# AdeeshKolluru/AdsorbDiff

Measured on AMD Instinct MI355X. Metric: sampled adsorbate sites/sec (50 denoise steps, ~200-atom slabs), higher is better.
Workload: dtype f32 (f16x3-split MFMA, fp32 accumulate; ADF_GEMM=f32 selects exact f32)

## Files before the change

adsorbdiff_amd/csrc/api.hip:

```cpp
#include <stdarg.h>
#include <stdlib.h>
#include <string.h>

#include <new>

#include "common.h"

static thread_local char g_err[512] = "";

void adf_set_error(const char* fmt, ...) {
    va_list ap;
    va_start(ap, fmt);
    vsnprintf(g_err, sizeof(g_err), fmt, ap);
    va_end(ap);
}

extern "C" const char* adf_last_error(void) { return g_err; }
extern "C" const char* adf_version(void) { return "adsorbdiff_hip 0.5.0 (gfx950)"; }

adf_tune adf_tune_from_env() {
    auto off_is_0 = [](const char* name) { const char* e = getenv(name); return (e && atoi(e) == 0) ? 0 : 1; };
    auto is_f32 = [](const char* name) { const char* e = getenv(name); return e && strcmp(e, "f32") == 0; };
    adf_tune t = {};
    t.gemm_stream = off_is_0("ADF_GEMM_STREAM");
    t.head_gate_fused = off_is_0("ADF_HEAD_GATE_FUSED");
    t.lift_emit = off_is_0("ADF_LIFT_EMIT");
    t.graph_sys_csr = off_is_0("ADF_GRAPH_SYS_CSR");
    t.train_gemm16 = is_f32("ADF_TRAIN_GEMM") ? 0 : 1;
    t.wgrad_f32 = is_f32("ADF_WGRAD") ? 1 : 0;
    const char* gt = getenv("ADF_EQV2_GEMM_TILE");
    t.eqv2_gemm_tile256 = (gt && atoi(gt) == 128) ? 0 : 1;
    t.eqv2_rotin_generic = getenv("ADF_EQV2_ROTIN_GENERIC") != nullptr;
    t.eqv2_rotout_generic = getenv("ADF_EQV2_ROTOUT_GENERIC") != nullptr;
    t.sample_split = off_is_0("ADF_SAMPLE_SPLIT");
    return t;
}
const adf_tune& adf_tune_process() {
    static const adf_tune t = adf_tune_from_env();
    return t;
}
int adf_current_num_cus() {
    int dev = 0, n = 0;
    if (hipGetDevice(&dev) != hipSuccess || hipDeviceGetAttribute(&n, hipDeviceAttributeMultiprocessorCount, dev) != hipSuccess) return 0;
    return n;
}

extern "C" int32_t adf_profile_enable(adf_painn_t h, int32_t on) {
    if (!h) { adf_set_error("null handle"); return ADF_EINVAL; }
    h->prof.enable(on != 0);
    ADF_HIP_CHECK(hipMemset(h->kcount, 0, 8 * sizeof(unsigned long long)));
    if (h->twin) return adf_profile_enable(h->twin, on);
    return ADF_OK;
}

extern "C" int32_t adf_profile_read(adf_painn_t h, float* ms, int64_t* count, int64_t* message_ksteps, void* stream) {
    if (!h || !ms || !count) { adf_set_error("null argument"); return ADF_EINVAL; }
    ADF_HIP_CHECK(hipStreamSynchronize((hipStream_t)stream));
    if (message_ksteps) {
        unsigned long long k[8];
        ADF_HIP_CHECK(hipMemcpy(k, h->kcount, sizeof(k), hipMemcpyDeviceToHost));
        ADF_HIP_CHECK(hipMemset(h->kcount, 0, sizeof(k)));
        *message_ksteps = (int64_t)k[0];
    }
    ADF_TRY(h->prof.read(ms, count, ADF_PROF_NCAT));
    if (h->twin) {
        float ms2[ADF_PROF_NCAT];
        int64_t count2[ADF_PROF_NCAT], k2 = 0;
        ADF_TRY(adf_profile_read(h->twin, ms2, count2, message_ksteps ? &k2 : nullptr, h->twin->split_stream));
        for (int c = 0; c < ADF_PROF_NCAT; ++c) { ms[c] += ms2[c]; count[c] += count2[c]; }
        if (message_ksteps) *message_ksteps += k2;
    }
    return ADF_OK;
}

extern "C" int32_t adf_painn_create(const adf_painn_hparams* hp, adf_painn_t* out) {
    if (!hp || !out) { adf_set_error("null argument"); return ADF_EINVAL; }
    if (hp->hidden_channels % ADF_SLICE_CH != 0 || hp->hidden_channels < 128 || hp->hidden_channels > 1024) {
        adf_set_error("hidden_channels=%d must be a multiple of %d in [128,1024]", hp->hidden_channels, ADF_SLICE_CH);
        return ADF_EINVAL;
    }
    if (hp->num_rbf % 2 != 0 || hp->num_rbf > 128 || hp->num_rbf < 2) {
        adf_set_error("num_rbf=%d must be even and <= 128", hp->num_rbf);
        return ADF_EINVAL;
    }
    if (hp->max_neighbors < 1 || hp->max_neighbors > ADF_MAX_K) {
        adf_set_error("max_neighbors=%d must be in [1,%d]", hp->max_neighbors, ADF_MAX_K);
        return ADF_EINVAL;
    }
    if (hp->num_layers < 1 || hp->num_layers > 16 || hp->num_heads < 0 || hp->num_heads > 2) {
        adf_set_error("num_layers must be in [1,16], num_heads in [0,2]");
        return ADF_EINVAL;
    }
    adf_painn* h = new (std::nothrow) adf_painn();
    if (!h) { adf_set_error("host allocation failed"); return ADF_EOOM; }
    h->hp = *hp;
    hipDeviceProp_t prop;
    if (hipGetDevice(&h->device) != hipSuccess || hipGetDeviceProperties(&prop, h->device) != hipSuccess) {
        adf_set_error("no usable HIP device: %s", hipGetErrorString(hipGetLastError()));
        adf_painn_destroy(h);
        return ADF_EHIP;
    }
    h->num_cus = prop.multiProcessorCount;
    h->dist_floor = 1.0e-3f;
    {
        const char* e = getenv("ADF_INCREMENTAL");
        h->inc_on = !(e && e[0] == '0');
        const char* e2 = getenv("ADF_INC_SYNC");
        h->inc_sync = e2 && e2[0] == '1';
    }
    const int H = hp->hidden_channels, R = hp->num_rbf, L = hp->num_layers;
    adf_pool& m = h->m_life;
    int32_t st = m.alloc(&h->rbf_pack, (size_t)L * (H / ADF_SLICE_CH) * R * 192);
    if (st == ADF_OK) st = m.alloc(&h->rbf_bias_pack, (size_t)L * (H / ADF_SLICE_CH) * 192);
    if (st == ADF_OK) st = m.alloc(&h->rbf_pack16, (size_t)L * (H / ADF_SLICE_CH) * R * 192 * 2 * sizeof(uint16_t));
    if (st == ADF_OK) st = m.alloc(&h->rbf_bias_pack16, (size_t)L * (H / ADF_SLICE_CH) * 192);
    if (st == ADF_OK) st = m.alloc(&h->rbf_scales, 16);
    if (st == ADF_OK) st = m.alloc(&h->flags, ADF_NFLAGS);
    if (st == ADF_OK && hipMemset(h->flags, 0, sizeof(int32_t) * ADF_NFLAGS) != hipSuccess) st = ADF_EHIP;
    {
        const size_t HH = (size_t)H * H;
        const size_t per_layer = HH + 3 * HH + 2 * HH + 2 * HH + 3 * HH;
        const size_t per_head = HH + HH / 2 + 2 * HH + HH + HH / 4 + HH / 2;
        const size_t elems = (size_t)L * per_layer + (size_t)hp->num_heads * per_head;
        h->w16_bytes = elems * 2 * sizeof(uint16_t) + 4096;
        if (st == ADF_OK) st = m.alloc(&h->w16_arena, h->w16_bytes);
        if (st == ADF_OK) st = m.alloc(&h->w16_scales, 256);
        if (st == ADF_OK) st = m.alloc(&h->w16_bias_perm, (size_t)L * 2 * 3 * H);
        if (st == ADF_OK) st = m.alloc(&h->w16_scratch, 1);
        if (st == ADF_OK) st = m.alloc(&h->wfrag_arena, h->w16_bytes);
        const char* e = getenv("ADF_GEMM");
        h->gemm_f32 = e && strcmp(e, "f32") == 0;
        const char* el = getenv("ADF_LIFT");
        h->lift_on = !(el && strcmp(el, "0") == 0);
        const char* e2 = getenv("ADF_MSG");
        h->msg_f32 = e2 ? strcmp(e2, "f32") == 0 : h->gemm_f32;
        h->msg_f32_only = hp->num_rbf % 8 != 0;
        h->msg_f32 = h->msg_f32 || h->msg_f32_only;
        const char* er = getenv("ADF_ROW_MAXIMA");
        h->rmx = (er && atoi(er) == 0) ? 0 : 1;
        h->tune = adf_tune_from_env();
    }
    if (st == ADF_OK) st = m.alloc(&h->kcount, 8);
    if (st == ADF_OK && hipMemset(h->kcount, 0, 8 * sizeof(unsigned long long)) != hipSuccess) st = ADF_EHIP;
    if (st != ADF_OK) { adf_painn_destroy(h); return st; }
    *out = h;
    return ADF_OK;
}

static void inc_free(adf_painn* h) {
    h->m_inc.release();
    h->inc_tmp_bytes = 0;
    h->inc_capN = 0; h->inc_valid = false;
}

static void free_workspaces(adf_painn* h) {
    h->m_ws.release();
    h->inc_valid = false;
    h->scan_tmp_bytes = 0;
    h->lift.cap = 0; h->mag_v3_valid = false;
    h->xpart = h->catpart = h->vpart = nullptr; h->part_stride = 0;
    h->part_x = h->part_vec = nullptr; h->dbg_msg_rows = h->dbg_cat_rows = h->dbg_comb_rows = 0; h->dbg_mag = nullptr;
    h->cache_valid = false;
    h->capN = h->capB = h->capE = 0;
}

extern "C" int32_t adf_painn_destroy(adf_painn_t h) {
    if (!h) return ADF_OK;
    if (h->twin) { adf_set_error("destroy: the handle has a live twin that reads its weight images; destroy the twin first"); return ADF_EINVAL; }
    if (h->parent) {
        h->parent->twin = nullptr;
        h->parent->split_last = false;
        if (h->split_stream) { (void)hipStreamSynchronize((hipStream_t)h->split_stream); (void)hipStreamDestroy((hipStream_t)h->split_stream); }
        for (void* e : h->split_ev)
            if (e) (void)hipEventDestroy((hipEvent_t)e);
    }
    if (h->inc_cnt_host) (void)hipHostFree(h->inc_cnt_host);
    for (int i = 0; i < 2; ++i)
        if (h->inc_ev[i]) (void)hipEventDestroy((hipEvent_t)h->inc_ev[i]);
    adf_grad_free(h);
    delete h;
    return ADF_OK;
}

static void borrow_weights(adf_painn* t, const adf_painn* p, bool bound) {
    t->emb = p->emb; t->rbf_offset = p->rbf_offset;
    memcpy(t->layer, p->layer, sizeof(t->layer));
    memcpy(t->head, p->head, sizeof(t->head));
    memcpy(t->scale, p->scale, sizeof(t->scale));
    t->rbf_pack = p->rbf_pack; t->rbf_bias_pack = p->rbf_bias_pack; t->rbf_pack16 = p->rbf_pack16;
    t->rbf_bias_pack16 = p->rbf_bias_pack16; t->rbf_scales = p->rbf_scales; t->rbf_uniform = p->rbf_uniform;
    t->w16_arena = p->w16_arena; t->w16_bytes = p->w16_bytes; t->w16_scales = p->w16_scales;
    t->w16_bias_perm = p->w16_bias_perm; t->w16_scratch = p->w16_scratch; t->wfrag_arena = p->wfrag_arena;
    t->weights_set = bound && p->weights_set;
    t->rec0_valid = false;
    t->inc_valid = false;
}
static void follow_settings(adf_painn* t, const adf_painn* p) {
    if (t->gemm_f32 != p->gemm_f32 || t->msg_f32 != p->msg_f32 || t->dist_floor != p->dist_floor || t->lift_on != p->lift_on) {
        t->cache_valid = false; t->rec0_valid = false; t->inc_valid = false;
    }
    t->gemm_f32 = p->gemm_f32; t->msg_f32 = p->msg_f32; t->msg_f32_only = p->msg_f32_only; t->dist_floor = p->dist_floor;
    t->lift_on = p->lift_on; t->tune = p->tune; t->inc_sync = p->inc_sync;
}

extern "C" int32_t adf_painn_create_twin(adf_painn_t parent, adf_painn_t* out) {
    if (!parent || !out) { adf_set_error("create_twin: null argument"); return ADF_EINVAL; }
    if (parent->parent) { adf_set_error("create_twin: the handle is a twin itself"); return ADF_EINVAL; }
    if (parent->twin) { adf_set_error("create_twin: the handle already has a twin"); return ADF_EINVAL; }
    int dev = -1;
    if (hipGetDevice(&dev) != hipSuccess || dev != parent->device) {
        adf_set_error("create_twin: the parent lives on device %d, the current device is %d", parent->device, dev);
        return ADF_EINVAL;
    }
    adf_painn* t = new (std::nothrow) adf_painn();
    if (!t) { adf_set_error("host allocation failed"); return ADF_EOOM; }
    t->hp = parent->hp; t->device = parent->device; t->num_cus = parent->num_cus;
    t->rmx = parent->rmx; t->inc_on = parent->inc_on;
    follow_settings(t, parent);
    int32_t st = t->m_life.alloc(&t->flags, ADF_NFLAGS);
    if (st == ADF_OK && hipMemset(t->flags, 0, sizeof(int32_t) * ADF_NFLAGS) != hipSuccess) st = ADF_EHIP;
    if (st == ADF_OK) st = t->m_life.alloc(&t->kcount, 8);
    if (st == ADF_OK && hipMemset(t->kcount, 0, 8 * sizeof(unsigned long long)) != hipSuccess) st = ADF_EHIP;
    if (st == ADF_OK) st = t->m_life.alloc(&t->split_state, 16);
    if (st == ADF_OK && hipStreamCreateWithFlags(reinterpret_cast<hipStream_t*>(&t->split_stream), hipStreamNonBlocking) != hipSuccess) st = ADF_EHIP;
    for (int i = 0; i < 2 && st == ADF_OK; ++i)
        if (hipEventCreateWithFlags(reinterpret_cast<hipEvent_t*>(&t->split_ev[i]), hipEventDisableTiming) != hipSuccess) st = ADF_EHIP;
    if (st != ADF_OK) {
        if (st == ADF_EHIP) adf_set_error("create_twin: %s", hipGetErrorString(hipGetLastError()));
        t->parent = parent;
        parent->twin = t;
        adf_painn_destroy(t);
        return st;
    }
    borrow_weights(t, parent, true);
    t->prof.enable(parent->prof.on);
    t->parent = parent;
    parent->twin = t;
    *out = t;
    return ADF_OK;
}

extern "C" int32_t adf_painn_set_split(adf_painn_t h, int32_t on) {
    if (!h) { adf_set_error("null handle"); return ADF_EINVAL; }
    h->tune.sample_split = on != 0;
    return ADF_OK;
}

extern "C" int32_t adf_split_stats(adf_painn_t h, int64_t* split_runs, int64_t* fallback_runs) {
    if (!h) { adf_set_error("null handle"); return ADF_EINVAL; }
    if (split_runs) *split_runs = (int64_t)h->split_runs;
    if (fallback_runs) *fallback_runs = (int64_t)h->split_fallbacks;
    return ADF_OK;
}

static void leave_split(adf_painn* h) {
    if (!h || !h->split_last) return;
    h->split_last = false;
    h->cache_valid = false; h->rec0_valid = false; h->inc_valid = false;
}

extern "C" int32_t adf_painn_set_weights(adf_painn_t h, int32_t n_weights, const void* const* w,
                                         const float* scale_factors, void* stream) {
    if (!h || !w || !scale_factors) { adf_set_error("null argument"); return ADF_EINVAL; }
    if (h->parent) { adf_set_error("set_weights: a twin reads its parent's weights; bind them there"); return ADF_EINVAL; }
    if (h->twin) borrow_weights(h->twin, h, false);
    const int L = h->hp.num_layers;
    const int expect = 2 + ADF_WEIGHTS_PER_LAYER * L + ADF_WEIGHTS_PER_HEAD * h->hp.num_heads;
    if (n_weights != expect) {
        adf_set_error("expected %d weight tensors, got %d", expect, n_weights);
        return ADF_EINVAL;
    }
    for (int i = 0; i < n_weights; ++i)
        if (!w[i]) { adf_set_error("weight %d is null", i); return ADF_EINVAL; }
    auto f = [&](int i) { return reinterpret_cast<const float*>(w[i]); };
    h->emb = f(0);
    h->rbf_offset = f(1);
    int k = 2;
    for (int l = 0; l < L; ++l) {
        adf_layer_weights& lw = h->layer[l];
        lw.ln_w = f(k++); lw.ln_b = f(k++); lw.xp0_w = f(k++); lw.xp0_b = f(k++); lw.xp2_w = f(k++); lw.xp2_b = f(k++);
        lw.rbf_w = f(k++); lw.rbf_b = f(k++); lw.vp_w = f(k++); lw.xv0_w = f(k++); lw.xv0_b = f(k++);
        lw.xv2_w = f(k++); lw.xv2_b = f(k++);
        h->scale[l] = scale_factors[l];
    }
    for (int hd = 0; hd < h->hp.num_heads; ++hd)
        for (int b = 0; b < 2; ++b) {
            adf_block_weights& bw = h->head[hd][b];
            bw.vec1_w = f(k++); bw.vec2_w = f(k++); bw.un0_w = f(k++); bw.un0_b = f(k++); bw.un2_w = f(k++);
            bw.un2_b = f(k++);
        }
    ADF_TRY(adf_pack_rbf(h, (hipStream_t)stream));
    {
        hipStream_t s = (hipStream_t)stream;
        const long long H = h->hp.hidden_channels, HH = H * H;
        unsigned char* cur = h->w16_arena;
        unsigned char* fcur = h->wfrag_arena;
        int nscale = 0;
        float* bperm = h->w16_bias_perm;
        auto split = [&](const float* w, long long rows, long long K, adf_w16* out, const float* fused_bias = nullptr,
                         bool pair_perm = false) -> int32_t {
            const long long n = rows * K;
            out->hi = cur; cur += n * 2;
            out->lo = cur; cur += n * 2;
            out->inv_scale = h->w16_scales + nscale++;
            out->bias_perm = nullptr;
            out->frag = nullptr;
            if (fused_bias) {
                out->bias_perm = bperm; bperm += 3 * H;
                ADF_TRY(adf_split_weight(w, n, out, h->w16_scratch, s, (int)H, (int)H, fused_bias));
            } else if (pair_perm) {
                ADF_TRY(adf_split_weight(w, n, out, h->w16_scratch, s, (int)H, (int)H, nullptr, 2));
            } else {
                ADF_TRY(adf_split_weight(w, n, out, h->w16_scratch, s));
            }
            if (rows % 32 == 0 && K % 16 == 0) {
                out->frag = fcur; fcur += n * 4;
                ADF_TRY(adf_pack_frag(out, (int)rows, (int)K, out->frag, s));
            }
            return ADF_OK;
        };
        for (int l = 0; l < L; ++l) {
            adf_layer_weights& lw = h->layer[l];
            ADF_TRY(split(lw.xp0_w, H, H, &lw.xp0_16));
            ADF_TRY(split(lw.xp2_w, 3 * H, H, &lw.xp2_16, lw.xp2_b));
            ADF_TRY(split(lw.vp_w, 2 * H, H, &lw.vp_16, nullptr, true));
            ADF_TRY(split(lw.xv0_w, H, 2 * H, &lw.xv0_16));
            ADF_TRY(split(lw.xv2_w, 3 * H, H, &lw.xv2_16, lw.xv2_b));
        }
        for (int hd = 0; hd < h->hp.num_heads; ++hd) {
            adf_block_weights& b0 = h->head[hd][0];
            adf_block_weights& b1 = h->head[hd][1];
            ADF_TRY(split(b0.vec1_w, H, H, &b0.vec1_16));
            ADF_TRY(split(b0.vec2_w, H / 2, H, &b0.vec2_16));
            ADF_TRY(split(b0.un0_w, H, 2 * H, &b0.un0_16));
            ADF_TRY(split(b0.un2_w, H, H, &b0.un2_16));
            ADF_TRY(split(b1.vec1_w, H / 2, H / 2, &b1.vec1_16));
            ADF_TRY(split(b1.un0_w, H / 2, H, &b1.un0_16));
        }
        if ((size_t)(cur - h->w16_arena) > h->w16_bytes || (size_t)(fcur - h->wfrag_arena) > h->w16_bytes || nscale > 256) {
            adf_set_error("internal: fp16 weight arena overflow");
            return ADF_EINVAL;
        }
    }
    h->weights_set = true;
    h->rec0_valid = false;
    h->inc_valid = false;
    adf_grad_invalidate(h);
    if (h->twin) borrow_weights(h->twin, h, true);
    return ADF_OK;
}

static int32_t ensure_capacity(adf_painn* h, int64_t N, int64_t B) {
    if (N <= h->capN && B <= h->capB) return ADF_OK;
    const int64_t capN = N > h->capN ? N : h->capN;
    const int64_t capB = B > h->capB ? B : h->capB;
    ADF_HIP_CHECK(hipDeviceSynchronize());
    free_workspaces(h);
    const int64_t H = h->hp.hidden_channels, K = h->hp.max_neighbors;
    const int64_t capE = 2 * capN * K;
    int32_t st = ADF_OK;
#define ALLOC(field, count) if (st == ADF_OK) st = h->m_ws.alloc(&h->field, (size_t)(count))
    ALLOC(nbr_cnt, capN);
    ALLOC(nbr_src, capN * K);
    ALLOC(nbr_shift, capN * K);
    ALLOC(cache_d2, capN * K);
    ALLOC(cache_cid, capN * K);
    ALLOC(cache_cnt, capN);
    ALLOC(deg, capN + 1);
    ALLOC(nptr, capN + 1);
    ALLOC(cursor, capN);
    ALLOC(img_cnt, capB);
    ALLOC(sys_slow, capB);
    ALLOC(e_src, capE);
    ALLOC(e_geom, capE);
    if (h->inc_on) {
        ALLOC(prev_nptr, capN + 1);
        ALLOC(prev_src, capE);
        ALLOC(prev_geom, capE);
    }
    if (st == ADF_OK) {
        h->scan_tmp_bytes = adf_scan_temp_bytes(capN + 1);
        st = h->m_ws.alloc(&h->scan_tmp, h->scan_tmp_bytes + 16);
    }
    ALLOC(x, capN * H);
    ALLOC(vecA, capN * 3 * H);
    ALLOC(vecB, capN * 3 * H);
    ALLOC(rec, (capN + 1) * 5 * H);
    ALLOC(y, capN * H);
    ALLOC(xh, capN * 3 * H);
    ALLOC(vv, capN * 6 * H);
    ALLOC(cat, capN * 2 * H);
    ALLOC(dot, capN * H);
    ALLOC(sys, capB * 16);
    ALLOC(lift.buf, capN * 3);
    ALLOC(mag_a, capN);
    ALLOC(mag_b, capN);
    ALLOC(mag_v3, capN * 3);
    const int64_t ps = (capN + 31) / 32 * 32, ns = H / ADF_SLICE_CH;
    if (h->rmx) ALLOC(rmx_part, (4 * ns + H / 32 + 4) * ps);
#undef ALLOC
    h->lift.cap = st == ADF_OK ? capN * 3 : 0;
    if (st != ADF_OK) { free_workspaces(h); return st; }
    if (h->rmx) {
        h->part_stride = ps;
        h->xpart = h->rmx_part; h->catpart = h->xpart + ns * ps; h->vpart = h->catpart + (H / 32) * ps;
        h->dbg_mag = h->vpart + 3 * ns * ps;
    }
    h->capN = capN; h->capB = capB; h->capE = capE;
    return ADF_OK;
}

static int32_t check_batch(const adf_painn* h, const adf_batch* b) {
    if (!h || !b) { adf_set_error("null argument"); return ADF_EINVAL; }
    if (b->num_atoms <= 0 || b->num_systems <= 0) { adf_set_error("empty batch"); return ADF_EINVAL; }
    if (!b->pos || !b->cell || !b->batch || !b->atom_offset) { adf_set_error("null batch array"); return ADF_EINVAL; }
    for (int k = 0; k < 3; ++k)
        if (b->reps[k] < 0 || b->reps[k] > 16) { adf_set_error("reps[%d]=%d out of range", k, b->reps[k]); return ADF_EINVAL; }
    return ADF_OK;
}

static int32_t read_flags(adf_painn* h, hipStream_t s) {
    int32_t f[ADF_NFLAGS];
    ADF_HIP_CHECK(hipMemcpyAsync(f, h->flags, sizeof(f), hipMemcpyDeviceToHost, s));
    ADF_HIP_CHECK(hipMemsetAsync(h->flags, 0, sizeof(f), s));
    int32_t f2[ADF_NFLAGS] = {};
    if (h->twin) {
        ADF_HIP_CHECK(hipMemcpyAsync(f2, h->twin->flags, sizeof(f2), hipMemcpyDeviceToHost, s));
        ADF_HIP_CHECK(hipMemsetAsync(h->twin->flags, 0, sizeof(f2), s));
    }
    ADF_HIP_CHECK(hipStreamSynchronize(s));
    for (int i = 0; i < ADF_NFLAGS; ++i) f[i] |= f2[i];
    if (f[4]) { adf_set_error("atomic number outside [1, %d] (rows of the embedding table)", h->hp.num_elements); return ADF_EINVAL; }
    if (f[0]) { adf_set_error("a centre atom has more than %d in-cutoff candidates", ADF_MAX_CAND); return ADF_EOVERFLOW; }
    if (f[2]) { adf_set_error("edge buffer overflow"); return ADF_EOVERFLOW; }
    if (f[3]) { adf_set_error("an atom has more than %d incoming edges", ADF_MAX_INDEG); return ADF_EOVERFLOW; }
    if (f[1]) { adf_set_error("An image has no neighbors"); return ADF_ENONEIGHBOR; }
    if (f[6]) { adf_set_error("energy gradient: an edge row has no reverse row in its partner's segment (asymmetric graph)"); return ADF_EINVAL; }
    if (f[5]) {
        adf_set_error("non-finite model output%s", h->gemm_f32 ? " (exact-f32 arithmetic: the inputs or weights are not finite)"
                      : " in f16x3 arithmetic: an activation left the fp16 range or the inputs are not finite; "
                        "adf_painn_set_arithmetic(h, 1) selects exact f32");
        return ADF_ENUMERIC;
    }
    return ADF_OK;
}

extern "C" int32_t adf_graph_set_moving(adf_painn_t h, const int32_t* moving, const int32_t* mov_idx,
                                        const int32_t* mov_off) {
    if (!h) { adf_set_error("null handle"); return ADF_EINVAL; }
    if (moving && (!mov_idx || !mov_off)) { adf_set_error("moving mask needs mov_idx and mov_off"); return ADF_EINVAL; }
    h->moving = moving; h->mov_idx = mov_idx; h->mov_off = mov_off;
    ++h->moving_serial;
    ADF_HIP_CHECK(hipMemset(h->flags, 0, sizeof(int32_t) * ADF_NFLAGS));
    h->cache_valid = false;
    h->rec0_valid = false;
    h->inc_valid = false;
    return ADF_OK;
}

extern "C" int32_t adf_graph_build(adf_painn_t h, const adf_batch* b, void* stream, int64_t* num_edges) {
    ADF_TRY(check_batch(h, b));
    leave_split(h);
    ADF_TRY(ensure_capacity(h, b->num_atoms, b->num_systems));
    hipStream_t s = (hipStream_t)stream;
    ADF_TRY(adf_graph_build_impl(h, b, s));
    if (num_edges) {
        int32_t e = 0;
        ADF_HIP_CHECK(hipMemcpyAsync(&e, h->nptr + b->num_atoms, sizeof(int32_t), hipMemcpyDeviceToHost, s));
        ADF_TRY(read_flags(h, s));
        *num_edges = e;
    }
    return ADF_OK;
}

__global__ void adf_export_edges_kernel(const int32_t* nptr, const int32_t* e_src, const float4* eg, int N,
                                        int32_t* src, int32_t* dst, float* dist, float* vec, long long cap) {
    const int n = blockIdx.x * 4 + (threadIdx.x >> 6);
    if (n >= N) return;
    for (int e = nptr[n] + (threadIdx.x & 63); e < nptr[n + 1]; e += 64) {
        if (e >= cap) continue;
        if (src) src[e] = e_src[e];
        if (dst) dst[e] = n;
        const float4 q = eg[e];
        if (dist) dist[e] = q.w;
        if (vec) { vec[3 * (size_t)e] = q.x; vec[3 * (size_t)e + 1] = q.y; vec[3 * (size_t)e + 2] = q.z; }
    }
}

__global__ void adf_export_shift_kernel(const int32_t* nbr_shift, int32_t* out, long long n, int r0, int r1, int r2) {
    const long long i = (long long)blockIdx.x * blockDim.x + threadIdx.x;
    if (i >= n) return;
    const int c = nbr_shift[i];
    const int n2 = 2 * r2 + 1, n1 = 2 * r1 + 1;
    const int ia = c / (n1 * n2), rem = c - ia * (n1 * n2);
    out[3 * i] = ia - r0;
    out[3 * i + 1] = rem / n2 - r1;
    out[3 * i + 2] = rem % n2 - r2;
}

extern "C" int32_t adf_graph_export(adf_painn_t h, int32_t* nbr_count, int32_t* nbr_src, int32_t* nbr_shift,
                                    int64_t edge_capacity, int32_t* edge_src, int32_t* edge_dst, float* edge_dist,
                                    float* edge_vec, int64_t* num_edges, void* stream) {
    if (!h || h->lastN <= 0) { adf_set_error("no graph built"); return ADF_EINVAL; }
    hipStream_t s = (hipStream_t)stream;
    const int64_t N = h->lastN, K = h->hp.max_neighbors;
    if (nbr_count) ADF_HIP_CHECK(hipMemcpyAsync(nbr_count, h->nbr_cnt, sizeof(int32_t) * N, hipMemcpyDeviceToDevice, s));
    if (nbr_src) ADF_HIP_CHECK(hipMemcpyAsync(nbr_src, h->nbr_src, sizeof(int32_t) * N * K, hipMemcpyDeviceToDevice, s));
    if (nbr_shift)
        hipLaunchKernelGGL(adf_export_shift_kernel, dim3((unsigned)((N * K + 255) / 256)), dim3(256), 0, s, h->nbr_shift,
                           nbr_shift, (long long)(N * K), h->last_reps[0], h->last_reps[1], h->last_reps[2]);
    if (edge_src || edge_dst || edge_dist || edge_vec)
        hipLaunchKernelGGL(adf_export_edges_kernel, dim3((unsigned)((N + 3) / 4)), dim3(256), 0, s, h->nptr, h->e_src,
                           h->e_geom, (int)N, edge_src, edge_dst, edge_dist, edge_vec, (long long)edge_capacity);
    ADF_HIP_CHECK(hipGetLastError());
    int32_t e = 0;
    ADF_HIP_CHECK(hipMemcpyAsync(&e, h->nptr + N, sizeof(int32_t), hipMemcpyDeviceToHost, s));
    ADF_HIP_CHECK(hipStreamSynchronize(s));
    if (num_edges) *num_edges = e;
    return ADF_OK;
}

static int32_t zero_pad_rows(adf_painn* h, int N, hipStream_t s) {
    const size_t row = (size_t)5 * h->hp.hidden_channels;
    ADF_HIP_CHECK(hipMemsetAsync(h->rec + (size_t)N * row, 0, sizeof(float) * row, s));
    return ADF_OK;
}

static int32_t make_records(adf_painn* h, int l, int n, const float* x, const float* vec, bool vec_is_zero, float* rec,
                            const int32_t* row_map, hipStream_t s) {
    const int H = h->hp.hidden_channels;
    const adf_layer_weights& w = h->layer[l];
    if (n <= 0) return ADF_OK;
    adf_prof_begin(h, ADF_PROF_NODE, s);
    const bool lift = h->lift_on && !h->gemm_f32;
    const bool em = lift && h->tune.lift_emit;
    ADF_TRY(adf_nodewise_layernorm(x, w.ln_w, w.ln_b, h->y, n, H, s, em ? h->mag_a : nullptr, h->rows_dev));
    ADF_TRY(adf_linear(h, h->y, H, w.xp0_w, &w.xp0_16, w.xp0_b, h->cat, H, n, H, H, 1, s, em ? h->mag_a : nullptr,
                       em ? h->mag_b : nullptr));
    if (h->gemm_f32) {
        if (row_map) { adf_set_error("internal: mapped records need the f16x3 path"); return ADF_EINVAL; }
        ADF_TRY(adf_launch_gemm(h->cat, H, w.xp2_w, H, w.xp2_b, h->xh, 3 * H, n, 3 * H, H, 0, s));
        ADF_TRY(adf_pack_records(h, n, h->xh, vec, vec_is_zero, s, rec));
    } else {
        adf_epi ep = {};
        ep.vec_in = vec; ep.rec = rec ? rec : h->rec; ep.H = H; ep.vec_is_zero = vec_is_zero ? 1 : 0;
        ep.row_map = row_map;
        ep.rmag = em ? h->mag_b : nullptr;
        ep.m_dev = h->rows_dev;
        ADF_TRY(adf_launch_gemm16_fused(h->cat, H, &w.xp2_16, n, H, H, 1, &ep, s, h->tune, lift ? &h->lift : nullptr));
    }
    adf_prof_end(h, s);
    return ADF_OK;
}

static int32_t message_layer(adf_painn* h, int l, int N, const float* x, const float* vec, float* x_out,
                             float* vec_out, bool vec_is_zero, hipStream_t s, const int32_t* tlist = nullptr,
                             int n_targets = 0, float* rec = nullptr, bool records_ready = false) {
    if (!records_ready) ADF_TRY(make_records(h, l, N, x, vec, vec_is_zero, rec, nullptr, s));
    adf_prof_begin(h, ADF_PROF_MESSAGE, s);
    const int items = tlist ? n_targets : N;
    const bool emit = h->rmx && h->lift_on && !h->gemm_f32 && !h->msg_f32 && items > 0 && items <= h->part_stride;
    h->part_x = h->part_vec = nullptr;
    const int32_t st = adf_message_impl(h, l, N, x, h->xh, vec, x_out, vec_out, vec_is_zero, s, tlist, n_targets, rec,
                                        tlist ? h->rows_dev : nullptr, emit ? h->xpart : nullptr, h->vpart, h->part_stride);
    if (st == ADF_OK && emit) {
        h->part_x = x_out; h->part_vec = vec_out; h->part_n = items; h->part_dev = tlist ? h->rows_dev : nullptr;
        h->dbg_msg_rows = items;
    }
    adf_prof_end(h, s);
    return st;
}

static int32_t update_layer(adf_painn* h, int l, int N, float* x, float* vec, hipStream_t s, bool from_message = true) {
    const int H = h->hp.hidden_channels;
    const adf_layer_weights& w = h->layer[l];
    adf_prof_begin(h, ADF_PROF_NODE, s);
    const bool parts = from_message && h->rmx && h->lift_on && !h->gemm_f32 && N > 0 && h->part_x == x && h->part_vec == vec &&
                       h->part_n == N && h->part_dev == h->rows_dev;
    h->part_x = h->part_vec = nullptr;
    if (h->gemm_f32) {
        ADF_TRY(adf_launch_gemm(vec, H, w.vp_w, H, nullptr, h->vv, 2 * H, 3 * N, 2 * H, H, 0, s));
        ADF_TRY(adf_nodewise_update_prep(h->vv, x, h->cat, h->dot, N, H, s));
        ADF_TRY(adf_linear(h, h->cat, 2 * H, w.xv0_w, &w.xv0_16, w.xv0_b, h->y, H, N, H, 2 * H, 1, s));
    } else {
        adf_epi ep = {};
        ep.v1 = h->vv; ep.dotw = h->dot; ep.cat = h->cat; ep.H = H; ep.m_dev = h->rows_dev;
        const adf_lift* lf = h->lift_on ? &h->lift : nullptr;
        if (parts) {
            ADF_TRY(adf_launch_rowmax_combine(h->vpart, 3 * h->part_stride, H / ADF_SLICE_CH, 3ll * N, h->lift.buf, s, h->rows_dev, 3));
            ep.rmag = h->lift.buf;
            if (h->dbg_capture) ADF_HIP_CHECK(hipMemcpyAsync(h->dbg_mag, h->lift.buf, sizeof(float) * 3 * (size_t)N, hipMemcpyDeviceToDevice, s));
        }
        if (parts || (h->dbg_capture && h->rmx && lf && N <= h->part_stride)) {
            ep.catpart = h->catpart; ep.part_stride = h->part_stride; h->dbg_cat_rows = N;
        }
        ADF_TRY(adf_launch_gemm16_fused(vec, H, &w.vp_16, N, H, H, 3, &ep, s, h->tune, lf));
        if (parts) {
            ADF_TRY(adf_launch_rowmax_combine(h->xpart, h->part_stride, H / ADF_SLICE_CH + H / 32, N, h->lift.buf, s, h->rows_dev, 1));
            if (h->dbg_capture) {
                ADF_HIP_CHECK(hipMemcpyAsync(h->dbg_mag + 3 * h->part_stride, h->lift.buf, sizeof(float) * (size_t)N, hipMemcpyDeviceToDevice, s));
                h->dbg_comb_rows = N;
            }
        }
        adf_epi e0 = {};
        e0.A2 = h->cat; e0.K1 = H; e0.m_dev = h->rows_dev;
        e0.rmag = parts ? h->lift.buf : nullptr;
        e0.out_mag = h->lift_on ? reinterpret_cast<unsigned int*>(h->mag_b) : nullptr;
        ADF_TRY(adf_launch_gemm16(x, H, &w.xv0_16, w.xv0_b, h->y, H, N, H, 2 * H, 1, &e0, s, lf, h->tune, h->num_cus));
    }
    int32_t st;
    if (h->gemm_f32) {
        ADF_TRY(adf_launch_gemm(h->y, H, w.xv2_w, H, w.xv2_b, h->xh, 3 * H, N, 3 * H, H, 0, s));
        st = adf_nodewise_update_apply(h->xh, h->dot, h->vv, x, vec, h->scale[l], N, H, s);
    } else {
        adf_epi ep = {};
        ep.x = x; ep.vec = vec; ep.dot = h->dot; ep.vv = h->vv; ep.scale = h->scale[l]; ep.H = H;
        ep.rmag = h->lift_on ? h->mag_b : nullptr;
        ep.m_dev = h->rows_dev;
        st = adf_launch_gemm16_fused(h->y, H, &w.xv2_16, N, H, H, 2, &ep, s, h->tune);
    }
// ... 701 lines not shown
```

adsorbdiff_amd/csrc/common.h:

```cpp
#pragma once
#include "base.h"
#include "arith.h"
#include "lanes.h"

#define ADF_GROUP_NODES 32
#define ADF_SLICE_CH 64
#define ADF_MAX_CAND 1024
#define ADF_MAX_K 128
#define ADF_NFLAGS 8
#define ADF_MAX_INDEG 1024
#define ADF_MAX_LAYERS 16

struct adf_w16 {
    void* hi;
    void* lo;
    float* inv_scale;
    float* bias_perm;
    void* frag;
};
struct adf_epi {
    const float* vec_in;
    float* rec;
    float* x;
    float* vec;
    const float* dot;
    const float* vv;
    float* v1;
    float* dotw;
    float* cat;
    float scale;
    int H;
    int vec_is_zero;
    const float* A2;
    int K1;
    const int32_t* row_map;
    const float* rmag;
    unsigned int* out_mag;
    const int32_t* m_dev;
    int accumulate;
    const float* gate;
    int gate_ld;
    float* catpart;
    long long part_stride;
};
struct adf_lift {
    float* buf;
    long long cap;
};
struct adf_layer_weights {
    const float *ln_w, *ln_b, *xp0_w, *xp0_b, *xp2_w, *xp2_b, *rbf_w, *rbf_b;
    const float *vp_w, *xv0_w, *xv0_b, *xv2_w, *xv2_b;
    adf_w16 xp0_16, xp2_16, vp_16, xv0_16, xv2_16;
};
struct adf_block_weights {
    const float *vec1_w, *vec2_w, *un0_w, *un0_b, *un2_w, *un2_b;
    adf_w16 vec1_16, vec2_16, un0_16, un2_16;
};

struct adf_painn {
    adf_painn_hparams hp;
    int device;
    bool weights_set;
    const float* emb;
    const float* rbf_offset;
    adf_layer_weights layer[16];
    adf_block_weights head[2][2];
    float scale[16];
    float* rbf_pack;
    float* rbf_bias_pack;
    void* rbf_pack16;
    float* rbf_bias_pack16;
    float* rbf_scales;
    unsigned char* w16_arena;
    size_t w16_bytes;
    float* w16_scales;
    float* w16_bias_perm;
    unsigned int* w16_scratch;
    unsigned char* wfrag_arena;
    bool gemm_f32;
    bool msg_f32;
    bool msg_f32_only;
    adf_tune tune;
    bool lift_on;
    adf_lift lift;
    float *mag_a, *mag_b;
    float* mag_v3;
    bool mag_v3_valid;
    int rmx;
    float* rmx_part;
    float *xpart, *catpart, *vpart;
    int64_t part_stride;
    const float *part_x, *part_vec;
    int part_n;
    const int32_t* part_dev;
    int dbg_msg_rows, dbg_cat_rows;
    bool dbg_capture;
    float* dbg_mag;
    int dbg_comb_rows;

    int64_t capN, capB, capE;
    int32_t* nbr_cnt;
    int32_t* nbr_src;
    int32_t* nbr_shift;
    int32_t* deg;
    int32_t* nptr;
    int32_t* cursor;
    int32_t* img_cnt;
    int32_t* sys_slow;
    void* scan_tmp;
    size_t scan_tmp_bytes;
    const int32_t* moving;
    const int32_t* mov_idx;
    const int32_t* mov_off;
    float* cache_d2;
    int32_t* cache_cid;
    int32_t* cache_cnt;
    bool cache_valid;
    int32_t* e_src;
    float4* e_geom;
    int32_t* flags;
    float *x, *vecA, *vecB, *y, *xh, *vv, *cat, *dot;
    float* rec;
    bool rbf_uniform;
    float* rec0;
    int64_t rec0_cap, rec0_N;
    bool rec0_valid;
    bool inc_on;
    bool inc_valid;
    int64_t inc_capN, inc_N;
    int inc_layers;
    float* incX[ADF_MAX_LAYERS + 1];
    float* incV[ADF_MAX_LAYERS + 1];
    float* incR[ADF_MAX_LAYERS];
    int32_t *prev_nptr, *prev_src;
    float4* prev_geom;
    unsigned char *inc_c0, *inc_chg;
    unsigned char *inc_pend, *inc_need, *inc_tf;
    int32_t* inc_list;
    int32_t* inc_cnt;
    int32_t* inc_cnt_host;
    void* inc_ev[2];
    bool inc_ev_live[2];
    int inc_slot;
    bool inc_sync;
    int32_t inc_seen[2 * ADF_MAX_LAYERS + 1];
    bool inc_seen_valid;
    unsigned char inc_pend_whole[2][ADF_MAX_LAYERS];
    int32_t inc_pend_N[2];
    int32_t inc_pend_Nseen;
    const int32_t* rows_dev;
    void* inc_tmp; size_t inc_tmp_bytes;
    unsigned long long inc_rows, inc_rows_full, inc_edges, inc_launches;
    unsigned long long build_serial, inc_serial;
    float *sub_x, *sub_vec, *sub_f;
    int64_t capS;
    float* sys;
    int32_t* ps_state = nullptr; int32_t ps_B = 0;
    const float *oe0_w, *oe0_b, *oe2_w, *oe2_b;
    adf_w16 oe0_16;
    unsigned char* oe0_buf;
    bool energy_set;
    const float* x_last;
    float dist_floor;
    void* grad;
    int64_t lastN, lastB;
    int32_t last_reps[3];
    int num_cus;
    adf_prof prof;
    unsigned long long* kcount;
    adf_painn* twin;
    adf_painn* parent;
    bool split_last;
    int32_t split_cut; int64_t split_N;
    unsigned long long split_runs, split_fallbacks;
    unsigned long long moving_serial, inc_set_serial;
    unsigned long long seen_moving_serial, seen_inc_serial;
    void* split_stream;
    void* split_ev[2];
    int32_t* split_state;
    int32_t* split_hist; int64_t split_hist_cap;
    adf_pool m_life;
    adf_pool m_ws;
    adf_pool m_inc;
    adf_pool m_sub;
    adf_pool m_rec0;
    void* obs_scratch = nullptr;
    int64_t obs_bytes = 0;
    adf_pool m_obs;
};

enum { ADF_PROF_GRAPH = 0, ADF_PROF_MESSAGE = 1, ADF_PROF_NODE = 2, ADF_PROF_HEADS = 3, ADF_PROF_STEPPER = 4 };
static inline void adf_prof_begin(adf_painn* h, int cat, hipStream_t s) { h->prof.begin(cat, s); }
static inline void adf_prof_end(adf_painn* h, hipStream_t s) { h->prof.end(s); }

int32_t adf_launch_gemm(const float* A, int lda, const float* W, int ldw, const float* bias, float* C, int ldc,
                        int M, int N, int K, int act_ssilu, hipStream_t s);
adf_tune adf_tune_from_env();
const adf_tune& adf_tune_process();
int adf_current_num_cus();
int32_t adf_launch_gemm16(const float* A, int lda, const adf_w16* W, const float* bias, float* C, int ldc, int M,
                          int N, int K, int act_ssilu, const adf_epi* ep, hipStream_t s, const adf_lift* lf,
                          const adf_tune& tune, int num_cus);
int32_t adf_launch_rowmag(const float* A, int lda, int K1, const float* A2, int K2, long long M, float* mag, hipStream_t s,
                          const int32_t* m_dev = nullptr, int m_mul = 1);
int32_t adf_launch_rowmax_combine(const float* part, long long stride, int nparts, long long M, float* mag, hipStream_t s,
                                  const int32_t* m_dev = nullptr, int m_mul = 1);
int32_t adf_split_weight(const float* w, long long n, adf_w16* out, unsigned int* scratch_bits, hipStream_t s,
                         int perm_H = 0, int K = 0, const float* bias = nullptr, int parts = 3);
int32_t adf_launch_gemm16_vecnorm(const float* A, int lda, const adf_w16* W, float* nrm, int M, int N, int K,
                                  hipStream_t s, const adf_tune& tune, const adf_lift* lf = nullptr,
                                  const float* premag = nullptr);
int32_t adf_launch_gemm16_fused(const float* A, int lda, const adf_w16* W, int M, int H, int K, int epi,
                                const adf_epi* ep, hipStream_t s, const adf_tune& tune, const adf_lift* lf = nullptr);
static inline int32_t adf_linear(const adf_painn* h, const float* A, int lda, const float* W, const adf_w16* W16,
                                 const float* bias, float* C, int ldc, int M, int N, int K, int act, hipStream_t s,
                                 const float* premag = nullptr, float* out_mag = nullptr) {
    if (h->gemm_f32) return adf_launch_gemm(A, lda, W, K, bias, C, ldc, M, N, K, act, s);
    adf_epi ep = {};
    ep.m_dev = h->rows_dev;
    if (h->lift_on) { ep.rmag = premag; ep.out_mag = reinterpret_cast<unsigned int*>(out_mag); }
    return adf_launch_gemm16(A, lda, W16, bias, C, ldc, M, N, K, act, &ep, s, h->lift_on ? &h->lift : nullptr, h->tune,
                             h->num_cus);
}
int32_t adf_pack_frag(const adf_w16* w, int N, int K, void* out, hipStream_t s);
int32_t adf_graph_build_impl(adf_painn* h, const adf_batch* b, hipStream_t s);
int32_t adf_energy_sum(const float* y, int H2, const float* w, const float* bias, const int32_t* atom_offset, float* energy,
                       int num_systems, hipStream_t s);
void adf_grad_invalidate(adf_painn* h);
void adf_grad_free(adf_painn* h);
bool adf_message_geo_supported(const adf_painn* h);
int32_t adf_message_geo(adf_painn* h, int layer, const float* xh, const float* vec, bool vec_is_zero, float4* part,
                        long long ecap, bool accumulate, hipStream_t s);
size_t adf_inc_temp_bytes(int64_t n);
int32_t adf_inc_compare(adf_painn* h, int N, hipStream_t s);
int32_t adf_inc_need_from_list(adf_painn* h, int N, int L, const int32_t* out_idx, int n_out, hipStream_t s);
int32_t adf_inc_plan_layer(adf_painn* h, int l, int N, bool first, bool have_need, hipStream_t s);
int32_t adf_inc_scatter_rows(const float* src, const int32_t* idx, int n, int width, float* dst, hipStream_t s,
                             const int32_t* n_dev = nullptr);
int32_t adf_inc_gather_rows(const float* src, const int32_t* idx, int n, int width, float* dst, hipStream_t s);
size_t adf_scan_temp_bytes(int64_t n);
int32_t adf_message_impl(adf_painn* h, int layer, int N, const float* x, const float* xh, const float* vec,
                         float* x_out, float* vec_out, bool vec_is_zero, hipStream_t s,
                         const int32_t* tlist = nullptr, int n_targets = 0, const float* rec = nullptr,
                         const int32_t* n_targets_dev = nullptr,
                         float* xpart = nullptr, float* vpart = nullptr, long long part_stride = 0);
int32_t adf_pack_rbf(adf_painn* h, hipStream_t s);
int32_t adf_pack_rbf_layer(adf_painn* h, int l, hipStream_t s);
int32_t adf_pack_records(adf_painn* h, int N, const float* xh, const float* vec, bool vec_is_zero, hipStream_t s,
                         float* rec = nullptr);
int32_t adf_nodewise_embed(adf_painn* h, const int32_t* Z, int N, float* x, hipStream_t s);
int32_t adf_nodewise_layernorm(const float* x, const float* w, const float* b, float* y, int N, int H, hipStream_t s,
                               float* out_mag = nullptr, const int32_t* n_dev = nullptr);
int32_t adf_nodewise_update_prep(const float* vv, const float* x, float* cat, float* dot, int N, int H, hipStream_t s);
int32_t adf_nodewise_update_apply(const float* h3, const float* dot, const float* vv, float* x, float* vec,
                                  float scale, int N, int H, hipStream_t s);
int32_t adf_head_forward(adf_painn* h, int head, int N, const float* x, const float* vec, float* out, hipStream_t s);
int32_t adf_stepper_init(const adf_batch* b, float* pos, const int32_t* tags, const float* noise,
                         hipStream_t s);
int32_t adf_stepper_step(float* sys, const adf_batch* b, float* pos, const int32_t* tags, const int32_t* fixed,
                         const float* f1, const float* f2, const adf_step_coef* coef, const adf_step_coef* coefs_dev,
                         int num_steps, const float* z_tr, const float* z_rot, int32_t early_stop_count,
                         int32_t* state, float* dcom, float* drot, hipStream_t s, int32_t* sys_state = nullptr,
                         int32_t* hist_t = nullptr);
int32_t adf_stepper_tr_step(float* sys, const adf_batch* b, float* pos, const int32_t* tags, const float* f1,
                            const adf_tr_coef* coef, const adf_tr_coef* coefs_dev, int num_steps, const float* z,
                            int32_t early_stop_count, int32_t* state, float* dcom, hipStream_t s,
                            int32_t* sys_state = nullptr);

struct adf_model {
    void* h;
    int32_t (*check)(void* h, const adf_batch* b);
    int32_t (*grow)(void* h, const adf_batch* b, float** sys);
    int32_t (*forward)(void* h, const adf_batch* b, const int32_t* out_idx, int32_t n_out, float* f1, float* f2,
                       hipStream_t s);
    void (*prof)(void* h, bool begin, hipStream_t s);
    int32_t* sys_state;
    int32_t sys_B;
};
int32_t adf_model_set_per_system_stop(int32_t** slot, int32_t* slot_B, int32_t* sys_state, int32_t B);
int32_t adf_frames_push_impl(adf_frames* f, const float* src, hipStream_t s);
int32_t adf_model_init_placement(const adf_model& m, const adf_batch* b, float* pos, const int32_t* tags,
                                 const float* noise, hipStream_t s);
int32_t adf_model_sde_step(const adf_model& m, const adf_batch* b, float* pos, const int32_t* tags, const int32_t* fixed,
                           const float* f1, const float* f2, const adf_step_coef* coef, const adf_step_coef* coefs_dev,
                           int32_t num_steps, const float* z_tr, const float* z_rot, int32_t early_stop_count,
                           int32_t* state, float* dcom, float* drot, hipStream_t s, int32_t* hist_t = nullptr);
int32_t adf_model_tr_step(const adf_model& m, const adf_batch* b, float* pos, const int32_t* tags, const float* f1,
                          const adf_tr_coef* coef, const adf_tr_coef* coefs_dev, int32_t num_steps, const float* z,
                          int32_t early_stop_count, int32_t* state, float* dcom, hipStream_t s);
int32_t adf_model_sample(const adf_model& m, const adf_batch* b, float* pos, const int32_t* tags, const int32_t* fixed,
                         const adf_step_coef* coefs_dev, int32_t num_steps, const float* z_tr_all, const float* z_rot_all,
                         int32_t early_stop_count, int32_t poll_every, int32_t* state, const int32_t* out_idx,
                         int32_t n_out, float* f1, float* f2, adf_frames* sink, int32_t frame_every, hipStream_t s);
int32_t adf_model_tr_sample(const adf_model& m, const adf_batch* b, float* pos, const int32_t* tags,
                            const adf_tr_coef* coefs_dev, int32_t num_steps, const float* z_all, int32_t early_stop_count,
                            int32_t poll_every, int32_t* state, const int32_t* out_idx, int32_t n_out, float* f1,
                            adf_frames* sink, int32_t frame_every, hipStream_t s);

struct adf_split_side {
    const adf_batch* b;
    float* pos;
    const int32_t* tags;
    const int32_t* fixed;
    const int32_t* out_idx;
    int32_t n_out;
    float* f1;
    float* f2;
    int32_t* state;
    int32_t* hist;
    int32_t sys0;
    hipStream_t s;
};
int32_t adf_model_sample_split(const adf_model& mA, const adf_model& mB, adf_split_side A, adf_split_side B,
                               const adf_step_coef* coefs_dev, int32_t num_steps, const float* z_tr_all,
                               const float* z_rot_all, int32_t total_systems, int32_t early_stop_count, int32_t poll_every,
                               int32_t* state_init, hipEvent_t fork, hipEvent_t join);
```

adsorbdiff_amd/csrc/energy_grad.hip:

```cpp
#include <stdlib.h>
#include <string.h>

#include "message.h"

struct EgW {
    const float* f32;
    adf_w16 w16;
};
enum { EG_XP0 = 0, EG_XP2, EG_VP, EG_XV0, EG_XV2, EG_NW };

struct adf_grad {
    unsigned char* warena;
    float* wscales;
    bool wvalid;
    EgW fw[ADF_MAX_LAYERS][EG_NW];
    EgW bw[ADF_MAX_LAYERS][EG_NW];
    EgW oe_bw;
    float* rbf_wt[ADF_MAX_LAYERS];
    float* act;
    size_t act_floats;
    float4* part;
    int32_t* rev;
    long long ecap;
    int part_slices;
    adf_pool m_w;
    adf_pool m_ws;
};

static adf_grad* eg_state(adf_painn* h) {
    if (!h->grad) {
        adf_grad* g = new (std::nothrow) adf_grad();
        if (!g) return nullptr;
        h->grad = g;
    }
    return reinterpret_cast<adf_grad*>(h->grad);
}

void adf_grad_invalidate(adf_painn* h) {
    if (h && h->grad) reinterpret_cast<adf_grad*>(h->grad)->wvalid = false;
}

void adf_grad_free(adf_painn* h) {
    if (!h) return;
    delete reinterpret_cast<adf_grad*>(h->grad);
    h->grad = nullptr;
}

__global__ void eg_transpose_kernel(const float* __restrict__ src, float* __restrict__ dst, int R, int C) {
    __shared__ float t[32][33];
    const int bx = blockIdx.x * 32, by = blockIdx.y * 32;
    for (int r = threadIdx.y; r < 32; r += 8) {
        const int rr = by + r, cc = bx + threadIdx.x;
        t[r][threadIdx.x] = (rr < R && cc < C) ? src[(size_t)rr * C + cc] : 0.f;
    }
    __syncthreads();
    for (int r = threadIdx.y; r < 32; r += 8) {
        const int cc = bx + r, rr = by + threadIdx.x;
        if (cc < C && rr < R) dst[(size_t)cc * R + rr] = t[threadIdx.x][r];
    }
}

static inline unsigned eg_grid(long long total) {
    long long b = (total + 255) / 256;
    if (b > 256 * 16) b = 256 * 16;
    if (b < 1) b = 1;
    return (unsigned)b;
}

__global__ void eg_seed_kernel(const float* __restrict__ he0, const float* __restrict__ w2, float* __restrict__ dhe,
                               long long N, int H2) {
    for (long long t = (long long)blockIdx.x * blockDim.x + threadIdx.x; t < N * H2; t += (long long)gridDim.x * blockDim.x) {
        const int c = (int)(t % H2);
        dhe[t] = adf_dssilu_times(he0[t], w2[c]);
    }
}

__global__ void eg_add_kernel(const float* __restrict__ src, float* __restrict__ dst, long long n) {
    for (long long i = (long long)blockIdx.x * blockDim.x + threadIdx.x; i < n; i += (long long)gridDim.x * blockDim.x)
        dst[i] += src[i];
}

__global__ __launch_bounds__(256) void eg_msg_bwd_plain_kernel(
    const int32_t* __restrict__ nptr, const int32_t* __restrict__ e_src, const float4* __restrict__ e_geom,
    const float* __restrict__ xh, const float* __restrict__ vec, const float* __restrict__ wt, const float* __restrict__ bias,
    const float* __restrict__ mu, int R, float inv_cutoff, float coeff, float env_a, float env_b, float env_c, int env_pi,
    const float* __restrict__ gx1, const float* __restrict__ gv1, float* __restrict__ dxh, float* __restrict__ dvec,
    float* __restrict__ dx, float4* __restrict__ part, int H, int vec_is_zero, int accumulate) {
    __shared__ float rbv[128], rbd[128], red[4][4];
    const int j = blockIdx.x, tid = threadIdx.x, lane = tid & 63, wave = tid >> 6;
    const int e0 = nptr[j], e1 = nptr[j + 1];
    const float is3 = 0.57735026918962576f, ish = 1.0f / sqrtf((float)H), is2 = 0.70710678118654752f;
    const int H3 = 3 * H;
    for (int cb = 0; cb < H; cb += 256) {
        const int c = cb + tid;
        const bool on = c < H;
        float xa = 0.f, xb = 0.f, xc = 0.f, w0 = 0.f, w1 = 0.f, w2 = 0.f, ba = 0.f, bb = 0.f, bc = 0.f;
        if (on) {
            const float* xr = xh + (size_t)j * H3;
            xa = xr[c]; xb = xr[H + c]; xc = xr[2 * H + c];
            ba = bias[c]; bb = bias[H + c]; bc = bias[2 * H + c];
            if (!vec_is_zero) { const float* vr = vec + (size_t)j * H3; w0 = vr[c]; w1 = vr[H + c]; w2 = vr[2 * H + c]; }
        }
        float dxa = 0.f, dxb = 0.f, dxc = 0.f, dv0 = 0.f, dv1 = 0.f, dv2 = 0.f;
        for (int e = e0; e < e1; ++e) {
            const int i = e_src[e];
            const float4 g = e_geom[e];
            __syncthreads();
            if (tid < R) {
                const float xs = g.w * inv_cutoff;
                float xq = 1.0f;
                for (int k = 1; k < env_pi; ++k) xq *= xs;
                const float xp = xq * xs, pe = (float)env_pi;
                float env = 1.0f + env_a * xp + env_b * (xp * xs) + env_c * (xp * xs * xs);
                float envd = env_a * pe * xq + env_b * (pe + 1.0f) * xp + env_c * (pe + 2.0f) * (xp * xs);
                if (!(xs < 1.0f)) { env = 0.f; envd = 0.f; }
                const float dm = xs - mu[tid];
                const float ga = expf(coeff * dm * dm);
                rbv[tid] = env * ga;
                rbd[tid] = (envd + env * 2.0f * coeff * dm) * ga * inv_cutoff;
            }
            __syncthreads();
            float al = 0.f, b0 = 0.f, b1 = 0.f, b2 = 0.f;
            if (on) {
                float ra = ba, rb = bb, rc = bc, pa = 0.f, pb = 0.f, pc = 0.f;
                for (int k = 0; k < R; ++k) {
                    const float* wr = wt + (size_t)k * H3;
                    const float wa = wr[c], wb = wr[H + c], wc = wr[2 * H + c];
                    const float v = rbv[k], d = rbd[k];
                    ra = fmaf(wa, v, ra); rb = fmaf(wb, v, rb); rc = fmaf(wc, v, rc);
                    pa = fmaf(wa, d, pa); pb = fmaf(wb, d, pb); pc = fmaf(wc, d, pc);
                }
                const float gx = gx1[(size_t)i * H + c] * is2;
                const size_t vo = (size_t)i * H3 + c;
                const float g0 = gv1[vo] * ish, g1 = gv1[vo + H] * ish, g2 = gv1[vo + 2 * H] * ish;
                const float S = (g0 * w0 + g1 * w1 + g2 * w2) * is3;
                const float T = -(g0 * g.x + g1 * g.y + g2 * g.z);
                dxa += gx * ra; dxb += S * rb; dxc += T * rc;
                const float f = xb * rb * is3;
                dv0 += g0 * f; dv1 += g1 * f; dv2 += g2 * f;
                al = gx * xa * pa + S * xb * pb + T * xc * pc;
                const float fc = xc * rc;
                b0 = g0 * fc; b1 = g1 * fc; b2 = g2 * fc;
            }
            al = adf_wave_sum(al); b0 = adf_wave_sum(b0); b1 = adf_wave_sum(b1); b2 = adf_wave_sum(b2);
            if (lane == 0) { red[wave][0] = al; red[wave][1] = b0; red[wave][2] = b1; red[wave][3] = b2; }
            __syncthreads();
            if (tid < 4) {
                const float sum = (red[0][tid] + red[1][tid]) + (red[2][tid] + red[3][tid]);
                float* o = reinterpret_cast<float*>(part + e) + tid;
                *o = (cb == 0 && !accumulate) ? sum : *o + sum;
            }
        }
        if (on) {
            float* dh = dxh + (size_t)j * H3;
            dh[c] = dxa; dh[H + c] = dxb; dh[2 * H + c] = dxc;
            dx[(size_t)j * H + c] = gx1[(size_t)j * H + c] * is2;
            if (!vec_is_zero) {
                const size_t vo = (size_t)j * H3 + c;
                dvec[vo] = gv1[vo] + dv0; dvec[vo + H] = gv1[vo + H] + dv1; dvec[vo + 2 * H] = gv1[vo + 2 * H] + dv2;
            }
        }
    }
}

__global__ __launch_bounds__(256) void eg_reverse_index_kernel(const int32_t* __restrict__ nptr, const int32_t* __restrict__ e_src,
                                                                const float4* __restrict__ e_geom, int N, int32_t* __restrict__ rev,
                                                                int32_t* __restrict__ flags) {
    const int n = blockIdx.x * 4 + (threadIdx.x >> 6);
    if (n >= N) return;
    for (int e = nptr[n] + (threadIdx.x & 63); e < nptr[n + 1]; e += 64) {
        const int i = e_src[e];
        const float4 g = e_geom[e];
        int found = -1;
        for (int f = nptr[i]; f < nptr[i + 1]; ++f) {
            if (e_src[f] != n) continue;
            const float4 o = e_geom[f];
            if (o.w == g.w && o.x == -g.x && o.y == -g.y && o.z == -g.z) { found = f; break; }
        }
        rev[e] = found;
        if (found < 0) flags[6] = 1;
    }
}

__device__ __forceinline__ void eg_row_gradient(const float4* __restrict__ part, long long ecap, int nslices,
                                                const float4 g, int e, float& gx, float& gy, float& gz) {
    float al = 0.f, bx = 0.f, by = 0.f, bz = 0.f;
    for (int sl = 0; sl < nslices; ++sl) {
        const float4 v = part[(size_t)sl * ecap + e];
        al = __fadd_rn(al, v.x); bx = __fadd_rn(bx, v.y); by = __fadd_rn(by, v.z); bz = __fadd_rn(bz, v.w);
    }
    const float bu = fmaf(bz, g.z, fmaf(by, g.y, __fmul_rn(bx, g.x)));
    const float inv = __fdiv_rn(1.0f, g.w);
    gx = __fsub_rn(__fmul_rn(al, g.x), __fmul_rn(fmaf(-bu, g.x, bx), inv));
    gy = __fsub_rn(__fmul_rn(al, g.y), __fmul_rn(fmaf(-bu, g.y, by), inv));
    gz = __fsub_rn(__fmul_rn(al, g.z), __fmul_rn(fmaf(-bu, g.z, bz), inv));
}

__global__ __launch_bounds__(256) void eg_position_kernel(const int32_t* __restrict__ nptr, const float4* __restrict__ e_geom,
                                                           const int32_t* __restrict__ rev, const float4* __restrict__ part,
                                                           long long ecap, int nslices, int N,
                                                           float* __restrict__ forces) {
    const int n = blockIdx.x * 4 + (threadIdx.x >> 6), lane = threadIdx.x & 63;
    if (n >= N) return;
    float fx = 0.f, fy = 0.f, fz = 0.f;
    for (int e = nptr[n] + lane; e < nptr[n + 1]; e += 64) {
        float ax, ay, az, bx = 0.f, by = 0.f, bz = 0.f;
        eg_row_gradient(part, ecap, nslices, e_geom[e], e, ax, ay, az);
        const int f = rev[e];
        if (f >= 0) eg_row_gradient(part, ecap, nslices, e_geom[f], f, bx, by, bz);
        fx = __fadd_rn(fx, __fsub_rn(ax, bx)); fy = __fadd_rn(fy, __fsub_rn(ay, by)); fz = __fadd_rn(fz, __fsub_rn(az, bz));
    }
#pragma unroll
    for (int o = 32; o > 0; o >>= 1) {
        fx = __fadd_rn(fx, __shfl_xor(fx, o)); fy = __fadd_rn(fy, __shfl_xor(fy, o)); fz = __fadd_rn(fz, __shfl_xor(fz, o));
    }
    if (lane == 0) { forces[3 * (size_t)n] = fx; forces[3 * (size_t)n + 1] = fy; forces[3 * (size_t)n + 2] = fz; }
}

static size_t eg_al(size_t b) { return (b + 255) & ~(size_t)255; }
static size_t eg_weight_bytes(const adf_painn* h) {
    const size_t H = h->hp.hidden_channels, L = h->hp.num_layers, R = h->hp.num_rbf;
    const size_t per_layer = eg_al(H * H * 20) + 2 * eg_al(2 * H * H * 20) + 2 * eg_al(3 * H * H * 20) + eg_al(3 * H * R * 4);
    return per_layer * L + eg_al(H / 2 * H * 12);
}

static int32_t eg_build_weights(adf_painn* h, adf_grad* g, hipStream_t s) {
    const long long H = h->hp.hidden_channels, L = h->hp.num_layers, R = h->hp.num_rbf, H2 = H / 2;
    struct Shape { long long n, k; };
    const Shape shp[EG_NW] = {{H, H}, {3 * H, H}, {2 * H, H}, {H, 2 * H}, {3 * H, H}};
    auto al = eg_al;
    const size_t bytes = eg_weight_bytes(h);
    if (!g->wscales) ADF_TRY(g->m_w.alloc(&g->wscales, (size_t)2 * EG_NW * ADF_MAX_LAYERS + 8));
    ADF_TRY(g->m_w.alloc(&g->warena, bytes));
    unsigned char* cur = g->warena;
    int nscale = 0;
    auto image = [&](const float* w, long long n, long long k, EgW* out) -> int32_t {
        const long long e = n * k;
        out->f32 = w;
        out->w16 = adf_w16{};
        out->w16.hi = cur; out->w16.lo = cur + e * 2; out->w16.frag = cur + e * 4;
        cur += e * 8;
        out->w16.inv_scale = g->wscales + nscale++;
        ADF_TRY(adf_split_weight(w, e, &out->w16, h->w16_scratch, s));
        return adf_pack_frag(&out->w16, (int)n, (int)k, out->w16.frag, s);
    };
    auto transposed = [&](const float* w, long long n, long long k, EgW* out) -> int32_t {
        float* t = reinterpret_cast<float*>(cur);
        cur += n * k * 4;
        hipLaunchKernelGGL(eg_transpose_kernel, dim3((unsigned)((k + 31) / 32), (unsigned)((n + 31) / 32)), dim3(32, 8), 0, s,
                           w, t, (int)n, (int)k);
        return image(t, k, n, out);
    };
    for (int l = 0; l < L; ++l) {
        const adf_layer_weights& lw = h->layer[l];
        const float* src[EG_NW] = {lw.xp0_w, lw.xp2_w, lw.vp_w, lw.xv0_w, lw.xv2_w};
        for (int i = 0; i < EG_NW; ++i) {
            unsigned char* start = cur;
            ADF_TRY(image(src[i], shp[i].n, shp[i].k, &g->fw[l][i]));
            ADF_TRY(transposed(src[i], shp[i].n, shp[i].k, &g->bw[l][i]));
            cur = start + al((size_t)shp[i].n * shp[i].k * 20);
        }
        g->rbf_wt[l] = reinterpret_cast<float*>(cur);
        hipLaunchKernelGGL(eg_transpose_kernel, dim3((unsigned)((R + 31) / 32), (unsigned)((3 * H + 31) / 32)), dim3(32, 8), 0, s,
                           lw.rbf_w, g->rbf_wt[l], (int)(3 * H), (int)R);
        cur += al((size_t)3 * H * R * 4);
    }
    ADF_TRY(transposed(h->oe0_w, H2, H, &g->oe_bw));
    ADF_HIP_CHECK(hipGetLastError());
    if ((size_t)(cur - g->warena) > bytes) { adf_set_error("internal: gradient weight arena overflow"); return ADF_EINVAL; }
    g->wvalid = true;
    return ADF_OK;
}

static int32_t eg_lin(adf_painn* h, const float* A, int lda, const EgW& w, const float* bias, float* C, int ldc, long long M,
                      int N, int K, hipStream_t s, int accumulate = 0, float* tmp = nullptr) {
    if (M * (long long)lda * 4 >= (1ll << 32) || M * (long long)ldc * 4 >= (1ll << 32)) {
        adf_set_error("energy gradient: %lld rows exceed the 32-bit offsets of the products, split the batch", M);
        return ADF_EOOM;
    }
    if (h->gemm_f32) {
        if (!accumulate) return adf_launch_gemm(A, lda, w.f32, K, bias, C, ldc, (int)M, N, K, 0, s);
        if (!tmp || ldc != N) { adf_set_error("internal: accumulating exact product needs contiguous scratch"); return ADF_EINVAL; }
        ADF_TRY(adf_launch_gemm(A, lda, w.f32, K, bias, tmp, N, (int)M, N, K, 0, s));
        hipLaunchKernelGGL(eg_add_kernel, dim3(eg_grid(M * N)), dim3(256), 0, s, tmp, C, M * N);
        ADF_HIP_CHECK(hipGetLastError());
        return ADF_OK;
    }
    adf_epi ep = {};
    ep.accumulate = accumulate;
    return adf_launch_gemm16(A, lda, &w.w16, bias, C, ldc, (int)M, N, K, 0, &ep, s, h->lift_on ? &h->lift : nullptr, h->tune,
                             h->num_cus);
}

struct EgLayer { float *x, *vec, *stats, *h0, *xh, *vv, *cat, *u0, *a, *dot; };
struct EgBufs {
    EgLayer layer[ADF_MAX_LAYERS];
    float *x_last, *he0;
    float *t1, *t2, *dx1, *dvec1, *dy;
    float *dxA, *dxB, *dvecA, *dvecB, *da, *ddot, *dv1, *dcat, *dvv, *dxh, *lnw, *lnscratch;
    size_t total;
};
static void eg_layout(long long N, int H, int L, float* base, EgBufs* b) {
    size_t off = 0;
    auto take = [&](long long floats) { float* p = base ? base + off : nullptr; off += ((size_t)floats + 63) & ~(size_t)63; return p; };
    const long long NH = N * H;
    for (int l = 0; l < L; ++l) {
        EgLayer& a = b->layer[l];
        a.x = take(NH); a.vec = l ? take(3 * NH) : nullptr; a.stats = take(2 * N); a.h0 = take(NH); a.xh = take(3 * NH);
        a.vv = take(6 * NH); a.cat = take(2 * NH); a.u0 = take(NH); a.a = take(3 * NH); a.dot = take(NH);
    }
    b->x_last = take(NH); b->he0 = take(NH / 2);
    b->t1 = take(NH); b->t2 = take(NH); b->dx1 = take(NH); b->dvec1 = take(3 * NH); b->dy = take(NH);
    b->dxA = take(NH); b->dxB = take(NH); b->dvecA = take(3 * NH); b->dvecB = take(3 * NH); b->da = take(3 * NH);
    b->ddot = take(NH); b->dv1 = take(3 * NH); b->dcat = take(2 * NH); b->dvv = take(6 * NH); b->dxh = take(3 * NH);
    b->lnw = take(2 * H); b->lnscratch = take((long long)512 * 2 * H + 64);
    b->total = off;
}

static long long eg_ecap(const adf_painn* h, long long N) { return 2 * N * h->hp.max_neighbors; }
static bool eg_fused(adf_painn* h) { return adf_message_geo_supported(h) && adf_op_message_bwd_fused_supported(h); }

extern "C" int32_t adf_painn_energy_gradient_workspace(adf_painn_t h, int64_t num_atoms, int64_t* bytes) {
    if (!h || !bytes || num_atoms <= 0) { adf_set_error("energy_gradient_workspace: bad argument"); return ADF_EINVAL; }
    EgBufs b;
    eg_layout(num_atoms, h->hp.hidden_channels, h->hp.num_layers, nullptr, &b);
    const long long ecap = eg_ecap(h, num_atoms);
    *bytes = (int64_t)(b.total * sizeof(float) +
                       (size_t)ecap * ((h->hp.hidden_channels / ADF_SLICE_CH) * sizeof(float4) + sizeof(int32_t)) +
                       eg_weight_bytes(h));
    return ADF_OK;
}

extern "C" int32_t adf_painn_forward_energy_gradient(adf_painn_t h, const adf_batch* b, float* energy, float* forces,
                                                     void* stream) {
    if (!h || !b || !energy || !forces) { adf_set_error("forward_energy_gradient: null argument"); return ADF_EINVAL; }
    if (!h->weights_set || !h->energy_set) {
        adf_set_error("forward_energy_gradient: weights / energy head not set (adf_painn_set_weights, adf_painn_set_energy_head)");
        return ADF_EINVAL;
    }
    if (!b->atomic_numbers) { adf_set_error("forward_energy_gradient: null atomic numbers"); return ADF_EINVAL; }
    hipStream_t s = (hipStream_t)stream;
    ADF_TRY(adf_graph_build(h, b, stream, nullptr));
    const int N = b->num_atoms, H = h->hp.hidden_channels, L = h->hp.num_layers, R = h->hp.num_rbf, H2 = H / 2;
    adf_grad* g = eg_state(h);
    if (!g) { adf_set_error("host allocation failed"); return ADF_EOOM; }
    if (!g->wvalid) ADF_TRY(eg_build_weights(h, g, s));
    const bool fused = eg_fused(h);
    const int nslices = fused ? H / ADF_SLICE_CH : 1;
    const long long ecap = eg_ecap(h, N);
    EgBufs w;
    eg_layout(N, H, L, nullptr, &w);
    if (w.total > g->act_floats || ecap > g->ecap || nslices > g->part_slices) {
        ADF_HIP_CHECK(hipDeviceSynchronize());
        g->m_ws.release();
        g->act_floats = 0; g->ecap = 0; g->part_slices = 0;
        const int sl = H / ADF_SLICE_CH;
        ADF_TRY(g->m_ws.alloc(&g->act, w.total));
        ADF_TRY(g->m_ws.alloc(&g->part, (size_t)ecap * sl));
        ADF_TRY(g->m_ws.alloc(&g->rev, (size_t)ecap));
        g->act_floats = w.total; g->ecap = ecap; g->part_slices = sl;
    }
    eg_layout(N, H, L, g->act, &w);
    const long long pstride = g->ecap;
    const size_t recrow = (size_t)(H / 32) * 160;

    ADF_TRY(adf_nodewise_embed(h, b->atomic_numbers, N, w.layer[0].x, s));
    for (int l = 0; l < L; ++l) {
        const adf_layer_weights& lw = h->layer[l];
        EgLayer& a = w.layer[l];
        const bool vz = l == 0;
        float* xn = l + 1 < L ? w.layer[l + 1].x : w.x_last;
        float* vn = l + 1 < L ? w.layer[l + 1].vec : w.dvecA;
        float *y = w.t1, *c = w.t2, *x1 = w.dx1, *vec1 = w.dvec1, *ua = w.dy;
        ADF_TRY(adf_op_layernorm_fwd(a.x, lw.ln_w, lw.ln_b, y, a.stats, N, H, stream));
        ADF_TRY(eg_lin(h, y, H, g->fw[l][EG_XP0], lw.xp0_b, a.h0, H, N, H, H, s));
        ADF_TRY(adf_op_ssilu_fwd(a.h0, c, (int64_t)N * H, stream));
        ADF_TRY(eg_lin(h, c, H, g->fw[l][EG_XP2], lw.xp2_b, a.xh, 3 * H, N, 3 * H, H, s));
        ADF_HIP_CHECK(hipMemsetAsync(h->rec + (size_t)N * recrow, 0, sizeof(float) * recrow, s));
        ADF_TRY(adf_pack_records(h, N, a.xh, a.vec, vz, s));
        {
            const bool prof = h->prof.on;
            h->prof.on = false;
            const int32_t st = adf_message_impl(h, l, N, a.x, a.xh, a.vec, x1, vec1, vz, s);
            h->prof.on = prof;
            ADF_TRY(st);
        }
        ADF_TRY(eg_lin(h, vec1, H, g->fw[l][EG_VP], nullptr, a.vv, 2 * H, 3ll * N, 2 * H, H, s));
        ADF_TRY(adf_op_copy_rows(x1, H, a.cat, 2 * H, N, H, 0, stream));
        ADF_TRY(adf_op_vdot_fwd(a.vv, a.dot, a.cat + H, 2 * H, N, H, 1e-8f, stream));
        ADF_TRY(eg_lin(h, a.cat, 2 * H, g->fw[l][EG_XV0], lw.xv0_b, a.u0, H, N, H, 2 * H, s));
        ADF_TRY(adf_op_ssilu_fwd(a.u0, ua, (int64_t)N * H, stream));
        ADF_TRY(eg_lin(h, ua, H, g->fw[l][EG_XV2], lw.xv2_b, a.a, 3 * H, N, 3 * H, H, s));
        ADF_TRY(adf_op_update_out_fwd(x1, vec1, a.a, a.dot, a.vv, h->scale[l], xn, vn, N, H, stream));
    }
    ADF_TRY(adf_linear(h, w.x_last, H, h->oe0_w, &h->oe0_16, h->oe0_b, w.he0, H2, N, H2, H, 0, s));
    ADF_TRY(adf_op_ssilu_fwd(w.he0, w.t1, (int64_t)N * H2, stream));
    ADF_TRY(adf_energy_sum(w.t1, H2, h->oe2_w, h->oe2_b, b->atom_offset, energy, b->num_systems, s));

    float *dx = w.dxA, *dx_in = w.dxB, *dvec = w.dvecA, *dvec_in = w.dvecB;
    hipLaunchKernelGGL(eg_seed_kernel, dim3(eg_grid((long long)N * H2)), dim3(256), 0, s, w.he0, h->oe2_w, w.ddot, (long long)N, H2);
    ADF_HIP_CHECK(hipGetLastError());
    ADF_TRY(eg_lin(h, w.ddot, H2, g->oe_bw, nullptr, dx, H, N, H, H2, s));
    ADF_HIP_CHECK(hipMemsetAsync(dvec, 0, sizeof(float) * 3 * (size_t)N * H, s));
    const double step = 1.0 / (R - 1), pe = (double)h->hp.envelope_exponent;
    for (int l = L - 1; l >= 0; --l) {
        const adf_layer_weights& lw = h->layer[l];
        EgLayer& a = w.layer[l];
        const bool vz = l == 0;
        ADF_TRY(adf_op_update_out_bwd(a.a, a.dot, a.vv, h->scale[l], dx, dvec, w.da, w.ddot, w.dv1, w.dx1, w.dvec1, N, H, stream));
        ADF_TRY(eg_lin(h, w.da, 3 * H, g->bw[l][EG_XV2], nullptr, w.t1, H, N, H, 3 * H, s));
        ADF_TRY(adf_op_ssilu_bwd(a.u0, w.t1, w.t2, (int64_t)N * H, stream));
        ADF_TRY(eg_lin(h, w.t2, H, g->bw[l][EG_XV0], nullptr, w.dcat, 2 * H, N, 2 * H, H, s));
        ADF_TRY(adf_op_copy_rows(w.dcat, 2 * H, w.dx1, H, N, H, 1, stream));
        ADF_TRY(adf_op_vdot_bwd(a.vv, a.cat + H, 2 * H, w.ddot, w.dcat + H, 2 * H, w.dv1, w.dvv, N, H, stream));
        ADF_TRY(eg_lin(h, w.dvv, 2 * H, g->bw[l][EG_VP], nullptr, w.dvec1, H, 3ll * N, H, 2 * H, s, 1, w.dv1));
        if (fused) {
            if (!vz) {
                ADF_TRY(adf_op_message_bwd_fused(h, l, a.xh, a.vec, w.dx1, w.dvec1, w.dxh, nullptr, ecap, dvec_in, dx_in, 0,
                                                 w.da, stream));
            } else {
                ADF_TRY(adf_pack_grad_records(h, w.dx1, w.dvec1, nullptr, s));
            }
            ADF_TRY(adf_message_geo(h, l, a.xh, a.vec, vz, g->part, pstride, l != L - 1, s));
        } else {
            hipLaunchKernelGGL(eg_msg_bwd_plain_kernel, dim3((unsigned)N), dim3(256), 0, s, h->nptr, h->e_src, h->e_geom, a.xh,
                               a.vec, g->rbf_wt[l], lw.rbf_b, h->rbf_offset, R, 1.0f / h->hp.cutoff,
                               (float)(-0.5 / (step * step)), (float)(-(pe + 1) * (pe + 2) / 2), (float)(pe * (pe + 2)),
                               (float)(-pe * (pe + 1) / 2), h->hp.envelope_exponent, w.dx1, w.dvec1, w.dxh, dvec_in, dx_in,
                               g->part, H, vz ? 1 : 0, l != L - 1 ? 1 : 0);
            ADF_HIP_CHECK(hipGetLastError());
        }
        if (vz) break;
        ADF_TRY(eg_lin(h, w.dxh, 3 * H, g->bw[l][EG_XP2], nullptr, w.t1, H, N, H, 3 * H, s));
        ADF_TRY(adf_op_ssilu_bwd(a.h0, w.t1, w.t2, (int64_t)N * H, stream));
        ADF_TRY(eg_lin(h, w.t2, H, g->bw[l][EG_XP0], nullptr, w.dy, H, N, H, H, s));
        ADF_TRY(adf_op_layernorm_bwd(a.x, lw.ln_w, a.stats, w.dy, dx_in, w.lnw, w.lnw + H, N, H, w.lnscratch, stream));
        float* t = dx; dx = dx_in; dx_in = t;
        t = dvec; dvec = dvec_in; dvec_in = t;
    }
    hipLaunchKernelGGL(eg_reverse_index_kernel, dim3((unsigned)((N + 3) / 4)), dim3(256), 0, s, h->nptr, h->e_src, h->e_geom, N,
                       g->rev, h->flags);
    hipLaunchKernelGGL(eg_position_kernel, dim3((unsigned)((N + 3) / 4)), dim3(256), 0, s, h->nptr, h->e_geom, g->rev, g->part,
                       pstride, nslices, N, forces);
    ADF_HIP_CHECK(hipGetLastError());
    return ADF_OK;
}
```

adsorbdiff_amd/csrc/gemm16.hip:

```cpp
#include <stdlib.h>

#include "common.h"

typedef float f32x16 __attribute__((ext_vector_type(16)));
typedef _Float16 half8 __attribute__((ext_vector_type(8)));
typedef _Float16 half4 __attribute__((ext_vector_type(4)));

#ifndef EPI_ABL
#define EPI_ABL 0
#endif
#ifndef G16_ABL
#define G16_ABL 0
#endif
#define HK 32
#define TLD3 96
#define TLD2 64
#define HLD 40

struct g16_tile {
    int NWN;
    int MI, NJ;
    int NT;
    int TM, TN;
    int ROWS;
};
constexpr g16_tile g16_tile_of(int epi, bool stream) {
    const int nwm = stream ? 1 : 2, nwn = stream ? 4 : 2;
    const int mi = epi >= 3 ? 3 : (epi ? 2 : (stream ? 3 : 2));
    const int nj = epi >= 3 ? 2 : (epi ? 3 : (stream ? 2 : 4));
    const int tm = 32 * mi * nwm;
    return {nwn, mi, nj, 64 * nwm * nwn, tm, 32 * nj * nwn, epi >= 3 ? tm / 3 : tm};
}

template <int ACT, int EPI, bool STREAM>
__global__ __launch_bounds__(g16_tile_of(EPI, STREAM).NT, 2) void adf_gemm_f16x3_kernel(
    const float* __restrict__ A, int lda, const _Float16* __restrict__ Whi, const _Float16* __restrict__ Wlo,
    const float* __restrict__ inv_scale, const float* __restrict__ bias, float* __restrict__ C, int ldc, int Mh, int N,
    int K, int tiles_n, adf_epi ep) {
    constexpr g16_tile geo = g16_tile_of(EPI, STREAM);
    constexpr int MI = geo.MI, NJ = geo.NJ, NWN = geo.NWN, NT = geo.NT, TM = geo.TM, TN = geo.TN;
    const int M = ep.m_dev ? min(Mh, (int)*ep.m_dev) : Mh;
    constexpr int NA = TM * 8 / NT;
    static_assert(TM * 8 % NT == 0, "A staging: whole float4s per thread");
    constexpr int LDS_STREAM = 4 * TM * HLD > NT / 64 * 6400 ? 4 * TM * HLD : NT / 64 * 6400;
    constexpr int LDS_MAIN = STREAM ? LDS_STREAM : (2 * TM + 2 * TN) * HLD;
    constexpr int LDS_REC = EPI == 1 ? NT / 64 * 2048 : 0;
    __shared__ __attribute__((aligned(16))) _Float16 lds[LDS_MAIN + LDS_REC];
    __shared__ float rinv[TM];
    _Float16* Ahi = lds;
    _Float16* Alo = Ahi + TM * HLD;
    _Float16* Bhi = Alo + TM * HLD;
    _Float16* Blo = Bhi + TN * HLD;
    const int tid = threadIdx.x;
    const int lane = tid & 63;
    const int wave = tid >> 6;
    const int wm = (wave / NWN) * (32 * MI);
    const int wn = (wave % NWN) * (32 * NJ);

    const int id = blockIdx.x;
    const int xcd = id & 7;
    const int qd = id >> 3;
    const int tile_m = (qd / tiles_n) * 8 + xcd;
    const int tile_n = qd % tiles_n;
    const int m0 = tile_m * geo.ROWS;
    const int n0 = tile_n * TN;
    if (m0 >= M) return;

    unsigned int a_goff[NA];
    int a_off[NA];
    float a_rs[NA];
    auto global_row = [&](int row) -> unsigned int {
        if constexpr (EPI >= 3) {
            const int atom = m0 + (row / 96) * 32 + (row & 31), ax = (row % 96) >> 5;
            return (unsigned int)min(atom, M - 1) * 3u + ax;
        } else {
            return (unsigned int)min(m0 + row, M - 1);
        }
    };
#pragma unroll
    for (int i = 0; i < NA; ++i) {
        const int f = tid + NT * i;
        const int row = f >> 3, kq = f & 7;
        const unsigned int grow = global_row(row);
        a_goff[i] = (grow * (unsigned int)lda + kq * 4) * 4u;
        a_off[i] = row * HLD + kq * 4;
        a_rs[i] = ep.rmag ? adf_pow2_lift(ep.rmag[grow]) : 1.0f;
    }
    if (tid < TM) rinv[tid] = ep.rmag ? 1.0f / adf_pow2_lift(ep.rmag[global_row(tid)]) : 1.0f;
    const char* const A1b = reinterpret_cast<const char*>(A);
    const char* const A2b = reinterpret_cast<const char*>(ep.A2) - (size_t)ep.K1 * 4;
    int w_src[NJ];
    int w_off[NJ];
#pragma unroll
    for (int i = 0; i < NJ; ++i) {
        const int f = tid + 256 * i;
        const int row = f >> 2, part = f & 3;
        w_src[i] = min(n0 + row, N - 1) * K + part * 8;
        w_off[i] = row * HLD + part * 8;
    }

    float4 ra[NA];
    half8 rwh[NJ], rwl[NJ];
#pragma unroll
    for (int i = 0; i < NA; ++i) ra[i] = *reinterpret_cast<const float4*>(A1b + a_goff[i]);
    if constexpr (!STREAM) {
#pragma unroll
        for (int i = 0; i < NJ; ++i) {
            rwh[i] = *reinterpret_cast<const half8*>(Whi + w_src[i]);
            rwl[i] = *reinterpret_cast<const half8*>(Wlo + w_src[i]);
        }
    }
    half8 wfa[NJ][2], wfb[NJ][2];
    const half8* const wfr = reinterpret_cast<const half8*>(Whi) + (size_t)((n0 + wn) / 32) * (K / 16) * 128 + lane;
    auto load_wf = [&](int s_, half8 (&wf)[NJ][2]) {
#pragma unroll
        for (int j = 0; j < NJ; ++j) {
            const size_t base = ((size_t)j * (K / 16) + s_) * 128;
            wf[j][0] = wfr[base];
            wf[j][1] = wfr[base + 64];
        }
    };
    if constexpr (STREAM) load_wf(0, wfa);

    f32x16 acc[MI][NJ];
#pragma unroll
    for (int i = 0; i < MI; ++i)
#pragma unroll
        for (int j = 0; j < NJ; ++j)
#pragma unroll
            for (int r = 0; r < 16; ++r) acc[i][j][r] = 0.f;

    const int nk = K / HK;
    const int fa = (wm + (lane & 31)) * HLD + (lane >> 5) * 8;
    const int fb = (wn + (lane & 31)) * HLD + (lane >> 5) * 8;
    auto stage_a = [&](int boff = 0) {
#pragma unroll
        for (int i = 0; i < NA; ++i) {
            if (G16_ABL & 2) {
                *reinterpret_cast<float2*>(Ahi + boff + a_off[i]) = make_float2(ra[i].x, ra[i].y);
                *reinterpret_cast<float2*>(Alo + boff + a_off[i]) = make_float2(ra[i].z, ra[i].w);
                continue;
            }
            const float sx = ra[i].x * a_rs[i], sy = ra[i].y * a_rs[i], sz = ra[i].z * a_rs[i], sw = ra[i].w * a_rs[i];
            half4 h, l;
            h[0] = (_Float16)sx; h[1] = (_Float16)sy; h[2] = (_Float16)sz; h[3] = (_Float16)sw;
            l[0] = (_Float16)(sx - (float)h[0]); l[1] = (_Float16)(sy - (float)h[1]);
            l[2] = (_Float16)(sz - (float)h[2]); l[3] = (_Float16)(sw - (float)h[3]);
            *reinterpret_cast<half4*>(Ahi + boff + a_off[i]) = h;
            *reinterpret_cast<half4*>(Alo + boff + a_off[i]) = l;
        }
    };
    auto request_a = [&](int kt1) {
        const int k1 = kt1 * HK;
        const char* ab = ((ep.K1 > 0 && k1 >= ep.K1) ? A2b : A1b) + (size_t)k1 * 4;
#pragma unroll
        for (int i = 0; i < NA; ++i) ra[i] = *reinterpret_cast<const float4*>(ab + ((G16_ABL & 4) ? (a_goff[i] & 127u) : a_goff[i]));
    };
    if constexpr (STREAM) {
        auto kstep = [&](int boff, int ks, const half8 (&cur)[NJ][2]) {
            if (G16_ABL & 8) { asm volatile("" :: "v"(cur[0][0]), "v"(cur[0][1]), "v"(cur[NJ - 1][0]), "v"(cur[NJ - 1][1])); return; }
#pragma unroll
            for (int i = 0; i < MI; ++i) {
                const half8 ah = *reinterpret_cast<const half8*>(Ahi + boff + fa + i * 32 * HLD + ks * 16);
                const half8 al = *reinterpret_cast<const half8*>(Alo + boff + fa + i * 32 * HLD + ks * 16);
#pragma unroll
                for (int j = 0; j < NJ; ++j) {
                    acc[i][j] = __builtin_amdgcn_mfma_f32_32x32x16_f16(al, cur[j][0], acc[i][j], 0, 0, 0);
                    acc[i][j] = __builtin_amdgcn_mfma_f32_32x32x16_f16(ah, cur[j][1], acc[i][j], 0, 0, 0);
                    acc[i][j] = __builtin_amdgcn_mfma_f32_32x32x16_f16(ah, cur[j][0], acc[i][j], 0, 0, 0);
                }
            }
        };
        {
            constexpr int BUF = 2 * TM * HLD;
            float4 rb[NA];
            auto request_b = [&](int kt1) {
                const int k1 = kt1 * HK;
                const char* ab = ((ep.K1 > 0 && k1 >= ep.K1) ? A2b : A1b) + (size_t)k1 * 4;
#pragma unroll
                for (int i = 0; i < NA; ++i) rb[i] = *reinterpret_cast<const float4*>(ab + ((G16_ABL & 4) ? (a_goff[i] & 127u) : a_goff[i]));
            };
            auto stage_from = [&](const float4 (&src)[NA], int boff) {
#pragma unroll
                for (int i = 0; i < NA; ++i) {
                    if (G16_ABL & 2) {
                        *reinterpret_cast<float2*>(Ahi + boff + a_off[i]) = make_float2(src[i].x, src[i].y);
                        *reinterpret_cast<float2*>(Alo + boff + a_off[i]) = make_float2(src[i].z, src[i].w);
                        continue;
                    }
                    const float sx = src[i].x * a_rs[i], sy = src[i].y * a_rs[i], sz = src[i].z * a_rs[i], sw = src[i].w * a_rs[i];
                    half4 h, l;
                    h[0] = (_Float16)sx; h[1] = (_Float16)sy; h[2] = (_Float16)sz; h[3] = (_Float16)sw;
                    l[0] = (_Float16)(sx - (float)h[0]); l[1] = (_Float16)(sy - (float)h[1]);
                    l[2] = (_Float16)(sz - (float)h[2]); l[3] = (_Float16)(sw - (float)h[3]);
                    *reinterpret_cast<half4*>(Ahi + boff + a_off[i]) = h;
                    *reinterpret_cast<half4*>(Alo + boff + a_off[i]) = l;
                }
            };
            half8 wfc[NJ][2], wfd[NJ][2];
            load_wf(1, wfb);
            auto tile = [&](int kt, int cur, const float4 (&nxt_regs)[NA], const half8 (&w0)[NJ][2], const half8 (&w1)[NJ][2],
                            half8 (&w2)[NJ][2], half8 (&w3)[NJ][2]) {
                load_wf(min(2 * kt + 2, 2 * nk - 1), w2);
                __builtin_amdgcn_sched_barrier(0);
                kstep(cur, 0, w0);
                __builtin_amdgcn_sched_barrier(0);
                load_wf(min(2 * kt + 3, 2 * nk - 1), w3);
                __builtin_amdgcn_sched_barrier(0);
                kstep(cur, 1, w1);
                stage_from(nxt_regs, BUF - cur);
                __builtin_amdgcn_sched_group_barrier(0x100, 2 * MI, 0);
#pragma unroll
                for (int u = 0; u < 3 * MI * NJ; ++u) {
                    __builtin_amdgcn_sched_group_barrier(0x8, 1, 0);
                    __builtin_amdgcn_sched_group_barrier(0x2, 4, 0);
                    if (u % 3 == 2) __builtin_amdgcn_sched_group_barrier(0x200, 1, 0);
                }
                __builtin_amdgcn_sched_barrier(0);
            };
            __syncthreads();
            stage_a(0);
            request_a(min(1, nk - 1));
            request_b(min(2, nk - 1));
            __syncthreads();
            for (int kt = 0; kt < nk; kt += 2) {
                tile(kt, 0, ra, wfa, wfb, wfc, wfd);
                request_a(min(kt + 3, nk - 1));
                __syncthreads();
                tile(kt + 1, BUF, rb, wfc, wfd, wfa, wfb);
                request_b(min(kt + 4, nk - 1));
                __syncthreads();
            }
        }
    } else {
    for (int kt = 0; kt < nk; ++kt) {
        __syncthreads();
        stage_a();
#pragma unroll
        for (int i = 0; i < NJ; ++i) {
            *reinterpret_cast<half8*>(Bhi + w_off[i]) = rwh[i];
            *reinterpret_cast<half8*>(Blo + w_off[i]) = rwl[i];
        }
        __syncthreads();
        if (kt + 1 < nk) {
            const int k1 = (kt + 1) * HK;
            request_a(kt + 1);
#pragma unroll
            for (int i = 0; i < NJ; ++i) {
                rwh[i] = *reinterpret_cast<const half8*>(Whi + w_src[i] + k1);
                rwl[i] = *reinterpret_cast<const half8*>(Wlo + w_src[i] + k1);
            }
        }
#pragma unroll
        for (int ks = 0; ks < 2; ++ks) {
            half8 bh[NJ], bl[NJ];
#pragma unroll
            for (int j = 0; j < NJ; ++j) {
                bh[j] = *reinterpret_cast<const half8*>(Bhi + fb + j * 32 * HLD + ks * 16);
                bl[j] = *reinterpret_cast<const half8*>(Blo + fb + j * 32 * HLD + ks * 16);
            }
#pragma unroll
            for (int i = 0; i < MI; ++i) {
                const half8 ah = *reinterpret_cast<const half8*>(Ahi + fa + i * 32 * HLD + ks * 16);
                const half8 al = *reinterpret_cast<const half8*>(Alo + fa + i * 32 * HLD + ks * 16);
#pragma unroll
                for (int j = 0; j < NJ; ++j) {
                    acc[i][j] = __builtin_amdgcn_mfma_f32_32x32x16_f16(al, bh[j], acc[i][j], 0, 0, 0);
                    acc[i][j] = __builtin_amdgcn_mfma_f32_32x32x16_f16(ah, bl[j], acc[i][j], 0, 0, 0);
                    acc[i][j] = __builtin_amdgcn_mfma_f32_32x32x16_f16(ah, bh[j], acc[i][j], 0, 0, 0);
                }
            }
        }
    }
    }

    const float isc = *inv_scale;
    if constexpr (EPI == 0) {
        if (((N | ldc) & 3) == 0 && (reinterpret_cast<uintptr_t>(C) & 15) == 0 && NJ % 2 == 0) {
            const int q = lane & 31;
            __syncthreads();
            float* T = reinterpret_cast<float*>(lds) + wave * (32 * TLD2);
#pragma unroll
            for (int jj = 0; jj < NJ / 2; ++jj) {
                const int cb = n0 + wn + 64 * jj;
                const float bv0 = (bias && cb + q < N) ? bias[cb + q] : 0.f;
                const float bv1 = (bias && cb + 32 + q < N) ? bias[cb + 32 + q] : 0.f;
#pragma unroll
                for (int i = 0; i < MI; ++i) {
#pragma unroll
                    for (int r = 0; r < 16; ++r) {
                        const int lr = (r & 3) + 8 * (r >> 2) + 4 * (lane >> 5);
                        const float sc = isc * rinv[wm + 32 * i + lr];
                        float v0 = acc[i][2 * jj][r] * sc + bv0, v1 = acc[i][2 * jj + 1][r] * sc + bv1;
                        if (ACT) { v0 = adf_ssilu(v0); v1 = adf_ssilu(v1); }
                        T[lr * TLD2 + q] = v0;
                        T[lr * TLD2 + 32 + q] = v1;
                    }
                    __builtin_amdgcn_fence(__ATOMIC_RELEASE, "wavefront");
                    __builtin_amdgcn_wave_barrier();
#pragma unroll
                    for (int it = 0; it < 8; ++it) {
                        const int item = lane + 64 * it;
                        const int lr = item >> 4, c4 = item & 15;
                        const int row = m0 + wm + 32 * i + lr, col = cb + 4 * c4;
                        float4 v = *reinterpret_cast<const float4*>(T + lr * TLD2 + 4 * c4);
                        if (row < M && col < N) {
                            if (ep.gate) {
                                const float4 g4 = *reinterpret_cast<const float4*>(ep.gate + (size_t)(row / 3) * ep.gate_ld + col);
                                v.x = g4.x * v.x; v.y = g4.y * v.y; v.z = g4.z * v.z; v.w = g4.w * v.w;
                            }
                            if (ep.accumulate) {
                                const float4 o = *reinterpret_cast<const float4*>(C + (size_t)row * ldc + col);
                                v.x += o.x; v.y += o.y; v.z += o.z; v.w += o.w;
                            }
                            *reinterpret_cast<float4*>(C + (size_t)row * ldc + col) = v;
                        }
                        if (ep.out_mag) {
                            float mg = col < N ? fmaxf(fmaxf(fabsf(v.x), fabsf(v.y)), fmaxf(fabsf(v.z), fabsf(v.w))) : 0.f;
                            mg = adf_row16_max(mg);
                            if (c4 == 0 && row < M) atomicMax(ep.out_mag + row, __float_as_uint(mg));
                        }
                    }
                    __builtin_amdgcn_wave_barrier();
                }
            }
            return;
        }
#pragma unroll
        for (int j = 0; j < NJ; ++j) {
            const int col = n0 + wn + 32 * j + (lane & 31);
            if (col >= N) continue;
            const float bv = bias ? bias[col] : 0.f;
#pragma unroll
            for (int i = 0; i < MI; ++i) {
#pragma unroll
                for (int r = 0; r < 16; ++r) {
                    const int row = m0 + wm + 32 * i + (r & 3) + 8 * (r >> 2) + 4 * (lane >> 5);
                    if (row < M) {
                        float v = acc[i][j][r] * (isc * rinv[row - m0]) + bv;
                        if (ACT) v = adf_ssilu(v);
                        if (ep.accumulate) v += C[(size_t)row * ldc + col];
                        C[(size_t)row * ldc + col] = v;
                        if (ep.out_mag) atomicMax(ep.out_mag + row, __float_as_uint(fabsf(v)));
                    }
                }
            }
        }
    } else if constexpr (EPI == 3) {
        static_assert(EPI != 3 || (NJ == 2 && MI == 3), "vec_proj epilogue: 3 components x (v1, v2)");
        const int q = lane & 31;
        const int g = (n0 + wn) / 64;
        const int H = ep.H;
        const float inv_sqrt_h = 1.0f / sqrtf((float)H);
        __syncthreads();
        float* T = reinterpret_cast<float*>(lds) + wave * 3200;
        const int a0 = m0 + (wave / NWN) * 32;
        float dv[16], nv[16];
#pragma unroll
        for (int r = 0; r < 16; ++r) {
            const int lr = (r & 3) + 8 * (r >> 2) + 4 * (lane >> 5);
            float d = 0.f, qq = 0.f;
#pragma unroll
            for (int i = 0; i < 3; ++i) {
                const float sc = isc * rinv[wm + 32 * i + lr];
                const float v1 = acc[i][0][r] * sc, v2 = acc[i][1][r] * sc;
                d += v1 * v2;
                qq += v2 * v2;
                T[lr * TLD3 + i * 32 + q] = v1;
            }
            dv[r] = d * inv_sqrt_h;
            nv[r] = sqrtf(qq + 1e-8f);
        }
        __builtin_amdgcn_fence(__ATOMIC_RELEASE, "wavefront");
        __builtin_amdgcn_wave_barrier();
#pragma unroll
        for (int it = 0; it < 4; ++it) {
            const int item = lane + 64 * it;
            const int lr = item >> 3, c4 = item & 7;
            const int n = a0 + lr;
            if (n < M) {
                float* vo = ep.v1 + (size_t)n * 3 * H + 32 * g + 4 * c4;
#pragma unroll
                for (int ax = 0; ax < 3; ++ax) {
                    const float4 tv_ = *reinterpret_cast<const float4*>(T + lr * TLD3 + ax * 32 + 4 * c4);
                    if (G16_ABL & 1) asm volatile("" :: "v"(tv_.x), "v"(tv_.w)); else
                    *reinterpret_cast<float4*>(vo + ax * H) = tv_;
                }
            }
        }
        __builtin_amdgcn_wave_barrier();
#pragma unroll
        for (int r = 0; r < 16; ++r) {
            const int lr = (r & 3) + 8 * (r >> 2) + 4 * (lane >> 5);
            T[lr * TLD3 + q] = dv[r];
            T[lr * TLD3 + 32 + q] = nv[r];
        }
        __builtin_amdgcn_fence(__ATOMIC_RELEASE, "wavefront");
        __builtin_amdgcn_wave_barrier();
#pragma unroll
        for (int it = 0; it < 4; ++it) {
            const int lr = it * 8 + (lane >> 3), c4 = lane & 7;
            const int n = a0 + lr, c = 32 * g + 4 * c4;
            const float4 dv_ = *reinterpret_cast<const float4*>(T + lr * TLD3 + 4 * c4);
            const float4 nv_ = *reinterpret_cast<const float4*>(T + lr * TLD3 + 32 + 4 * c4);
            if (n < M) {
                if (G16_ABL & 1) { asm volatile("" :: "v"(dv_.x), "v"(nv_.w)); } else {
                *reinterpret_cast<float4*>(ep.dotw + (size_t)n * H + c) = dv_;
                *reinterpret_cast<float4*>(ep.cat + (size_t)n * H + c) = nv_;
                }
            }
            if (ep.catpart) {
                const float mg = adf_lane8_max(fmaxf(fmaxf(fmaxf(0.f, fabsf(nv_.x)), fabsf(nv_.y)), fmaxf(fabsf(nv_.z), fabsf(nv_.w))));
                if (c4 == 0 && n < M) ep.catpart[(size_t)g * ep.part_stride + n] = mg;
            }
        }
    } else if constexpr (EPI == 4) {
        static_assert(EPI != 4 || (NJ == 2 && MI == 3), "norm epilogue: 3 components x 64 columns per wave");
        const int q = lane & 31;
        const int cb = n0 + wn;
        __syncthreads();
        float* T = reinterpret_cast<float*>(lds) + wave * 3200;
        const int a0 = m0 + (wave / NWN) * 32;
#pragma unroll
        for (int r = 0; r < 16; ++r) {
            const int lr = (r & 3) + 8 * (r >> 2) + 4 * (lane >> 5);
#pragma unroll
            for (int j = 0; j < 2; ++j) {
                const float a = acc[0][j][r] * (isc * rinv[wm + lr]), b = acc[1][j][r] * (isc * rinv[wm + 32 + lr]),
                            d = acc[2][j][r] * (isc * rinv[wm + 64 + lr]);
                T[lr * TLD2 + j * 32 + q] = sqrtf(a * a + b * b + d * d);
            }
        }
        __builtin_amdgcn_fence(__ATOMIC_RELEASE, "wavefront");
        __builtin_amdgcn_wave_barrier();
#pragma unroll
        for (int it = 0; it < 8; ++it) {
            const int lr = it * 4 + (lane >> 4), c4 = lane & 15;
            const int n = a0 + lr, c = cb + 4 * c4;
            if (n < M && c < N)
                *reinterpret_cast<float4*>(ep.cat + (size_t)n * N + c) = *reinterpret_cast<const float4*>(T + lr * TLD2 + 4 * c4);
        }
    } else {
        static_assert(EPI >= 3 || (NJ == 3 && MI == 2), "fused epilogues are written for the 64 x 96 wave tile");
        if (((EPI_ABL & 1) && EPI == 1) || ((EPI_ABL & 2) && EPI == 2)) {
            float sacc = 0.f;
            for (int i = 0; i < MI; ++i) for (int j = 0; j < NJ; ++j) for (int r = 0; r < 16; ++r) sacc += acc[i][j][r];
            if (ep.H < 0) ep.x[0] = sacc;
            return;
        }
        const int q = lane & 31;
        const int g = (n0 + wn) / 96;
        const int H = ep.H;
        const float b0 = bias[n0 + wn + q], b1 = bias[n0 + wn + 32 + q], b2 = bias[n0 + wn + 64 + q];
        __syncthreads();
        float* T = reinterpret_cast<float*>(lds) + wave * 3200;
#pragma unroll
        for (int i = 0; i < MI; ++i) {
#pragma unroll
            for (int r = 0; r < 16; ++r) {
                const int lr = (r & 3) + 8 * (r >> 2) + 4 * (lane >> 5);
                const float sc = isc * rinv[wm + 32 * i + lr];
                T[lr * TLD3 + q] = acc[i][0][r] * sc + b0;
                T[lr * TLD3 + 32 + q] = acc[i][1][r] * sc + b1;
                T[lr * TLD3 + 64 + q] = acc[i][2][r] * sc + b2;
            }
            __builtin_amdgcn_fence(__ATOMIC_RELEASE, "wavefront");
            __builtin_amdgcn_wave_barrier();
            const int c4 = lane & 7;
            const int c = 32 * g + 4 * c4;
            if constexpr (EPI == 1) {
                float4 v0[4], v1[4], v2[4];
                if (EPI_ABL & 4) { for (int it = 0; it < 4; ++it) { v0[it] = make_float4(1.f, 2.f, 3.f, 4.f); v1[it] = v0[it]; v2[it] = v0[it]; } }
                else if (!ep.vec_is_zero) {
#pragma unroll
                    for (int it = 0; it < 4; ++it) {
                        const int n = min(m0 + wm + 32 * i + it * 8 + (lane >> 3), M - 1);
                        const float* vr = ep.vec_in + (size_t)n * 3 * H + c;
                        v0[it] = *reinterpret_cast<const float4*>(vr);
                        v1[it] = *reinterpret_cast<const float4*>(vr + H);
                        v2[it] = *reinterpret_cast<const float4*>(vr + 2 * H);
                    }
                }
#pragma unroll
                for (int it = 0; it < 4; ++it) {
                    const int lr = it * 8 + (lane >> 3);
                    const int n = m0 + wm + 32 * i + lr;
                    const float4 p0 = *reinterpret_cast<const float4*>(T + lr * TLD3 + 4 * c4);
                    const float4 p1 = *reinterpret_cast<const float4*>(T + lr * TLD3 + 32 + 4 * c4);
                    const float4 p2 = *reinterpret_cast<const float4*>(T + lr * TLD3 + 64 + 4 * c4);
                    float4 o[4];
                    if (!ep.vec_is_zero) {
                        o[0] = make_float4(v0[it].x * p1.x, v1[it].x * p1.x, v2[it].x * p1.x, p0.x);
                        o[1] = make_float4(v0[it].y * p1.y, v1[it].y * p1.y, v2[it].y * p1.y, p0.y);
                        o[2] = make_float4(v0[it].z * p1.z, v1[it].z * p1.z, v2[it].z * p1.z, p0.z);
                        o[3] = make_float4(v0[it].w * p1.w, v1[it].w * p1.w, v2[it].w * p1.w, p0.w);
                    } else {
                        o[0] = make_float4(0.f, 0.f, 0.f, p0.x);
                        o[1] = make_float4(0.f, 0.f, 0.f, p0.y);
                        o[2] = make_float4(0.f, 0.f, 0.f, p0.z);
                        o[3] = make_float4(0.f, 0.f, 0.f, p0.w);
                    }
                    float4* X = reinterpret_cast<float4*>(lds + LDS_MAIN) + wave * 256;
#pragma unroll
                    for (int k = 0; k < 4; ++k) X[lane * 4 + k] = o[k];
                    __builtin_amdgcn_fence(__ATOMIC_RELEASE, "wavefront");
                    __builtin_amdgcn_wave_barrier();
#pragma unroll
                    for (int k = 0; k < 4; ++k) o[k] = X[(lane >> 3) * 32 + 8 * k + c4];
                    __builtin_amdgcn_wave_barrier();
                    if ((EPI_ABL & 8) && n >= 0) { if (ep.H < 0) ep.rec[0] = p2.x + o[0].x + o[1].y + o[2].z + o[3].w; }
                    else if (n < M) {
                        float* rec = ep.rec + ((size_t)(ep.row_map ? ep.row_map[n] : n) * (H / 32) + g) * 160;
#pragma unroll
                        for (int k = 0; k < 4; ++k) *reinterpret_cast<float4*>(rec + 32 * k + 4 * c4) = o[k];
                        *reinterpret_cast<float4*>(rec + 128 + 4 * c4) = p2;
                    }
                }
            } else {
                float4 d[4], xv[4], w1[4][3], tv[4][3];
#pragma unroll
                for (int it = 0; it < 4; ++it) {
                    const int n = min(m0 + wm + 32 * i + it * 8 + (lane >> 3), M - 1);
                    const size_t xo = (size_t)n * H + c;
                    d[it] = *reinterpret_cast<const float4*>(ep.dot + xo);
                    xv[it] = *reinterpret_cast<const float4*>(ep.x + xo);
                    const float* vr = ep.vec + (size_t)n * 3 * H + c;
                    const float* v1p = ep.vv + (size_t)n * 3 * H + c;
#pragma unroll
                    for (int ax = 0; ax < 3; ++ax) {
                        w1[it][ax] = *reinterpret_cast<const float4*>(v1p + ax * H);
                        tv[it][ax] = *reinterpret_cast<const float4*>(vr + ax * H);
                    }
                }
#pragma unroll
                for (int it = 0; it < 4; ++it) {
                    const int lr = it * 8 + (lane >> 3);
                    const int n = m0 + wm + 32 * i + lr;
                    const float4 p0 = *reinterpret_cast<const float4*>(T + lr * TLD3 + 4 * c4);
                    const float4 p1 = *reinterpret_cast<const float4*>(T + lr * TLD3 + 32 + 4 * c4);
                    const float4 p2 = *reinterpret_cast<const float4*>(T + lr * TLD3 + 64 + 4 * c4);
                    const float k2 = 0.70710678118654752f, sc = ep.scale;
                    float4 xo4 = xv[it];
                    xo4.x = (xo4.x + (p0.x + p1.x * d[it].x) * k2) * sc;
                    xo4.y = (xo4.y + (p0.y + p1.y * d[it].y) * k2) * sc;
                    xo4.z = (xo4.z + (p0.z + p1.z * d[it].z) * k2) * sc;
                    xo4.w = (xo4.w + (p0.w + p1.w * d[it].w) * k2) * sc;
                    if (n < M) {
                        *reinterpret_cast<float4*>(ep.x + (size_t)n * H + c) = xo4;
                        float* vr = ep.vec + (size_t)n * 3 * H + c;
#pragma unroll
                        for (int ax = 0; ax < 3; ++ax) {
                            float4 t = tv[it][ax];
                            const float4 v1 = w1[it][ax];
                            t.x += p2.x * v1.x; t.y += p2.y * v1.y; t.z += p2.z * v1.z; t.w += p2.w * v1.w;
                            *reinterpret_cast<float4*>(vr + ax * H) = t;
                        }
                    }
                }
            }
            __builtin_amdgcn_wave_barrier();
        }
    }
}

__global__ __launch_bounds__(256) void adf_rowmag_kernel(const float* __restrict__ A, int lda, int K1,
                                                         const float* __restrict__ A2, int K2, long long M,
                                                         float* __restrict__ mag, const int32_t* __restrict__ m_dev,
                                                         int m_mul) {
    const long long r = (long long)blockIdx.x * 4 + (threadIdx.x >> 6);
    const int lane = threadIdx.x & 63;
    if (r >= M || (m_dev && r >= (long long)*m_dev * m_mul)) return;
    float mx = 0.f;
    const float* a = A + (size_t)r * lda;
    for (int k = lane * 4; k < K1; k += 256) {
        const float4 v = *reinterpret_cast<const float4*>(a + k);
        mx = fmaxf(fmaxf(fmaxf(mx, fabsf(v.x)), fabsf(v.y)), fmaxf(fabsf(v.z), fabsf(v.w)));
    }
    if (A2) {
        const float* b = A2 + (size_t)r * lda;
        for (int k = lane * 4; k < K2; k += 256) {
            const float4 v = *reinterpret_cast<const float4*>(b + k);
            mx = fmaxf(fmaxf(fmaxf(mx, fabsf(v.x)), fabsf(v.y)), fmaxf(fabsf(v.z), fabsf(v.w)));
        }
    }
#pragma unroll
    for (int o = 32; o > 0; o >>= 1) mx = fmaxf(mx, __shfl_xor(mx, o));
    if (lane == 0) mag[r] = mx;
}

__global__ __launch_bounds__(256) void adf_rowmax_combine_kernel(const float* __restrict__ part, long long stride, int nparts,
                                                                 long long M, float* __restrict__ mag,
                                                                 const int32_t* __restrict__ m_dev, int m_mul) {
    const long long r = (long long)blockIdx.x * 256 + threadIdx.x;
    if (r >= M || (m_dev && r >= (long long)*m_dev * m_mul)) return;
    float mx = 0.f;
    for (int p = 0; p < nparts; ++p) mx = fmaxf(mx, part[(size_t)p * stride + r]);
    mag[r] = mx;
}

int32_t adf_launch_rowmax_combine(const float* part, long long stride, int nparts, long long M, float* mag, hipStream_t s,
                                  const int32_t* m_dev, int m_mul) {
    if (M <= 0) return ADF_OK;
    hipLaunchKernelGGL(adf_rowmax_combine_kernel, dim3((unsigned)((M + 255) / 256)), dim3(256), 0, s, part, stride, nparts, M,
                       mag, m_dev, m_mul);
    ADF_HIP_CHECK(hipGetLastError());
    return ADF_OK;
}

int32_t adf_launch_rowmag(const float* A, int lda, int K1, const float* A2, int K2, long long M, float* mag, hipStream_t s,
                          const int32_t* m_dev, int m_mul) {
    if (M <= 0) return ADF_OK;
    hipLaunchKernelGGL(adf_rowmag_kernel, dim3((unsigned)((M + 3) / 4)), dim3(256), 0, s, A, lda, K1, A2, K2, M, mag, m_dev,
                       m_mul);
    ADF_HIP_CHECK(hipGetLastError());
    return ADF_OK;
}

static int32_t lift_mags(const float* A, int lda, int K1, const float* A2, int K2, long long rows, const adf_lift* lf,
                         const float* premag, const float** out, hipStream_t s, const int32_t* m_dev = nullptr, int m_mul = 1) {
    *out = premag;
    if (!premag && lf && lf->buf) {
        if (rows > lf->cap) { adf_set_error("gemm16: lift scratch holds %lld rows, need %lld", lf->cap, rows); return ADF_EINVAL; }
        ADF_TRY(adf_launch_rowmag(A, lda, K1, A2, K2, rows, lf->buf, s, m_dev, m_mul));
        *out = lf->buf;
    }
    return ADF_OK;
}

__global__ void adf_absmax_kernel(const float* __restrict__ w, long long n, unsigned int* out_bits) {
    float m = 0.f;
    for (long long i = (long long)blockIdx.x * blockDim.x + threadIdx.x; i < n; i += (long long)gridDim.x * blockDim.x)
        m = fmaxf(m, fabsf(w[i]));
    m = adf_wave_max(m);
    if ((threadIdx.x & 63) == 0) atomicMax(out_bits, __float_as_uint(m));
}

__global__ void adf_split_kernel(const float* __restrict__ w, long long n, const unsigned int* absmax_bits,
                                 _Float16* __restrict__ hi, _Float16* __restrict__ lo, float* inv_scale, int perm_H,
                                 int K, const float* __restrict__ bias, float* __restrict__ bias_perm, int parts) {
    const float amax = __uint_as_float(*absmax_bits);
    int e = 0;
    if (amax > 0.f) (void)frexpf(amax, &e);
    const float scale = ldexpf(1.0f, 10 - e);
    if (blockIdx.x == 0 && threadIdx.x == 0) *inv_scale = 1.0f / scale;
    for (long long i = (long long)blockIdx.x * blockDim.x + threadIdx.x; i < n; i += (long long)gridDim.x * blockDim.x) {
        long long src = i;
        if (perm_H > 0) {
            const long long prow = i / K;
            const int k = (int)(i - prow * K);
            const int gw = 32 * parts;
            const int g = (int)(prow / gw), part = (int)((prow % gw) / 32), qq = (int)(prow % 32);
            const long long orow = (long long)part * perm_H + 32 * g + qq;
            src = orow * K + k;
            if (k == 0 && bias_perm) bias_perm[prow] = bias ? bias[orow] : 0.f;
        }
        const float v = w[src] * scale;
        const _Float16 h = (_Float16)v;
        hi[i] = h;
        lo[i] = (_Float16)(v - (float)h);
    }
}

int32_t adf_split_weight(const float* w, long long n, adf_w16* out, unsigned int* scratch_bits, hipStream_t s,
                         int perm_H, int K, const float* bias, int parts) {
    ADF_HIP_CHECK(hipMemsetAsync(scratch_bits, 0, sizeof(unsigned int), s));
    hipLaunchKernelGGL(adf_absmax_kernel, dim3(64), dim3(256), 0, s, w, n, scratch_bits);
    hipLaunchKernelGGL(adf_split_kernel, dim3(64), dim3(256), 0, s, w, n, scratch_bits, (_Float16*)out->hi,
                       (_Float16*)out->lo, out->inv_scale, perm_H, K, bias, out->bias_perm, parts);
    ADF_HIP_CHECK(hipGetLastError());
    return ADF_OK;
}

__global__ void adf_pack_frag_kernel(const _Float16* __restrict__ hi, const _Float16* __restrict__ lo, half8* __restrict__ out,
                                     int N, int K) {
    const int nks = K / 16;
    const long long total = (long long)(N / 32) * nks * 2 * 64;
    for (long long i = (long long)blockIdx.x * blockDim.x + threadIdx.x; i < total; i += (long long)gridDim.x * blockDim.x) {
        const int lane = (int)(i & 63), plane = (int)((i >> 6) & 1);
        const long long cs = i >> 7;
        const int s = (int)(cs % nks), cb = (int)(cs / nks);
        const _Float16* src = (plane ? lo : hi) + (size_t)(32 * cb + (lane & 31)) * K + 16 * s + 8 * (lane >> 5);
        out[i] = *reinterpret_cast<const half8*>(src);
    }
}

int32_t adf_pack_frag(const adf_w16* w, int N, int K, void* out, hipStream_t s) {
    if (N % 32 || K % 16) { adf_set_error("pack_frag: N %% 32 or K %% 16"); return ADF_EINVAL; }
    hipLaunchKernelGGL(adf_pack_frag_kernel, dim3(256), dim3(256), 0, s, (const _Float16*)w->hi, (const _Float16*)w->lo,
                       (half8*)out, N, K);
    ADF_HIP_CHECK(hipGetLastError());
    return ADF_OK;
}

static int32_t check_a_span(long long rows, int lda) {
    if (rows * (long long)lda * 4 >= (1ll << 32)) {
        adf_set_error("gemm16: A operand of %lld rows x %d exceeds the 32-bit offset range, split the batch", rows, lda);
        return ADF_EOOM;
    }
    return ADF_OK;
}

static bool can_stream(const adf_tune& tune, const adf_w16* W, int epi, int N, int K) {
    return tune.gemm_stream && W->frag && N % g16_tile_of(epi, true).TN == 0 && (K / HK) % 2 == 0;
}

static int32_t launch_f16x3(bool stream, int act, int epi, const float* A, int lda, const adf_w16* W, const float* bias, float* C,
                            int ldc, int M, int N, int K, const adf_epi& ep, hipStream_t s) {
    using kern_t = decltype(&adf_gemm_f16x3_kernel<0, 0, false>);
#define G16_FORM(STREAM_)                                                                                              \
    { adf_gemm_f16x3_kernel<0, 0, STREAM_>, adf_gemm_f16x3_kernel<1, 0, STREAM_>, adf_gemm_f16x3_kernel<0, 1, STREAM_>, \
      adf_gemm_f16x3_kernel<0, 2, STREAM_>, adf_gemm_f16x3_kernel<0, 3, STREAM_>, adf_gemm_f16x3_kernel<0, 4, STREAM_> }
    static const kern_t kernels[2][6] = {G16_FORM(false), G16_FORM(true)};
#undef G16_FORM
    const g16_tile t = g16_tile_of(epi, stream);
    const int tiles_n = (N + t.TN - 1) / t.TN;
    const int tiles_m8 = ((M + t.ROWS - 1) / t.ROWS + 7) / 8 * 8;
    hipLaunchKernelGGL(kernels[stream][epi ? epi + 1 : (act ? 1 : 0)], dim3((unsigned)(tiles_m8 * tiles_n)), dim3(t.NT), 0, s, A, lda,
                       (const _Float16*)(stream ? W->frag : W->hi), (const _Float16*)(stream ? nullptr : W->lo), W->inv_scale,
                       bias, C, ldc, M, N, K, tiles_n, ep);
    ADF_HIP_CHECK(hipGetLastError());
    return ADF_OK;
}

int32_t adf_launch_gemm16(const float* A, int lda, const adf_w16* W, const float* bias, float* C, int ldc, int M,
                          int N, int K, int act_ssilu, const adf_epi* ep_in, hipStream_t s, const adf_lift* lf,
                          const adf_tune& tune, int num_cus) {
    if (M <= 0) return ADF_OK;
    adf_epi ep = {};
    if (ep_in) ep = *ep_in;
    if (!ep.A2) ep.K1 = 0;
    if (K % HK != 0 || (lda & 3) || (ep.A2 && (ep.K1 <= 0 || ep.K1 % HK != 0 || ep.K1 >= K))) {
        adf_set_error("gemm16: K=%d (K1=%d) must be multiples of %d and lda a multiple of 4", K, ep.K1, HK);
        return ADF_EINVAL;
    }
    ADF_TRY(check_a_span(M, lda));
    if (ep.gate && (((N | ldc | ep.gate_ld) & 3) || (((uintptr_t)C | (uintptr_t)ep.gate) & 15))) {
        adf_set_error("gemm16: the gate epilogue needs N, ldc and gate_ld multiples of 4 and 16-byte aligned C and gate");
        return ADF_EINVAL;
    }
    ADF_TRY(lift_mags(A, lda, ep.A2 ? ep.K1 : K, ep.A2, ep.A2 ? K - ep.K1 : 0, M, lf, ep.rmag, &ep.rmag, s, ep.m_dev, 1));
    if (ep.out_mag) ADF_HIP_CHECK(hipMemsetAsync(ep.out_mag, 0, sizeof(float) * (size_t)M, s));
    const g16_tile ts = g16_tile_of(0, true);
    const long long wg = (long long)((M + ts.ROWS - 1) / ts.ROWS) * (N / ts.TN > 0 ? N / ts.TN : 1);
    const long long slots = 2ll * (num_cus > 0 ? num_cus : 256);
    const bool ragged4 = wg < 4 * slots && wg % slots != 0 && wg % slots < (3 * slots) / 10 && wg > slots;
    return launch_f16x3(can_stream(tune, W, 0, N, K) && !ragged4, act_ssilu, 0, A, lda, W, bias, C, ldc, M, N, K, ep, s);
}

int32_t adf_launch_gemm16_vecnorm(const float* A, int lda, const adf_w16* W, float* nrm, int M, int N, int K,
                                  hipStream_t s, const adf_tune& tune, const adf_lift* lf, const float* premag) {
    if (M <= 0) return ADF_OK;
    if (K % HK != 0 || (lda & 3) || (N & 3)) { adf_set_error("gemm16_vecnorm: bad shape"); return ADF_EINVAL; }
    ADF_TRY(check_a_span(3ll * M, lda));
    adf_epi ep = {};
    ep.cat = nrm;
    ADF_TRY(lift_mags(A, lda, K, nullptr, 0, 3ll * M, lf, premag, &ep.rmag, s));
    return launch_f16x3(can_stream(tune, W, 4, N, K), 0, 4, A, lda, W, nullptr, nullptr, 0, M, N, K, ep, s);
}

int32_t adf_launch_gemm16_fused(const float* A, int lda, const adf_w16* W, int M, int H, int K, int epi,
                                const adf_epi* ep_in, hipStream_t s, const adf_tune& tune, const adf_lift* lf) {
    adf_epi ep = *ep_in;
    if (M <= 0) return ADF_OK;
    if (K % HK != 0 || (lda & 3) || H % 64 != 0 || (epi != 3 && !W->bias_perm)) {
        adf_set_error("gemm16_fused: bad shape");
        return ADF_EINVAL;
    }
    const int rows_per = epi == 3 ? 3 : 1;
    ADF_TRY(check_a_span((long long)rows_per * M, lda));
    ADF_TRY(lift_mags(A, lda, K, nullptr, 0, (long long)rows_per * M, lf, ep_in->rmag, &ep.rmag, s, ep_in->m_dev, rows_per));
    const int N = (epi == 3 ? 2 : 3) * H;
    return launch_f16x3(can_stream(tune, W, epi, N, K), 0, epi, A, lda, W, epi == 3 ? nullptr : W->bias_perm, nullptr, 0, M, N, K, ep, s);
}
```

adsorbdiff_amd/csrc/peaks.hip:

```cpp
#include "common.h"

typedef float f32x16 __attribute__((ext_vector_type(16)));
typedef _Float16 half8 __attribute__((ext_vector_type(8)));

__global__ void adf_peak_copy_kernel(const float4* __restrict__ src, float4* __restrict__ dst, long long n4) {
    const long long i = (long long)blockIdx.x * blockDim.x + threadIdx.x;
    if (i < n4) dst[i] = src[i];
}

template <bool F16>
__global__ __launch_bounds__(256, 2) void adf_peak_mfma_kernel(float* out, int iters) {
    const int lane = threadIdx.x & 63;
    f32x16 acc[4];
#pragma unroll
    for (int b = 0; b < 4; ++b)
#pragma unroll
        for (int r = 0; r < 16; ++r) acc[b][r] = 0.f;
    half8 a, bb;
#pragma unroll
    for (int j = 0; j < 8; ++j) {
        a[j] = (_Float16)(0.37f * (float)(((lane * 7 + j * 13) % 31) - 15));
        bb[j] = (_Float16)(0.011f * (float)(((lane * 11 + j * 5) % 29) - 14));
    }
    const float af = (float)a[0], bf = (float)bb[1];
    for (int it = 0; it < iters; ++it) {
#pragma unroll
        for (int b = 0; b < 4; ++b) {
            if (F16) acc[b] = __builtin_amdgcn_mfma_f32_32x32x16_f16(a, bb, acc[b], 0, 0, 0);
            else acc[b] = __builtin_amdgcn_mfma_f32_32x32x2f32(af, bf, acc[b], 0, 0, 0);
        }
    }
    float sum = 0.f;
#pragma unroll
    for (int b = 0; b < 4; ++b)
#pragma unroll
        for (int r = 0; r < 16; ++r) sum += acc[b][r];
    if (sum == 123.456f) out[0] = sum;
}

extern "C" int32_t adf_measure_peaks(float* out_host3, void* stream) {
    hipStream_t s = (hipStream_t)stream;
    if (!out_host3) { adf_set_error("null argument"); return ADF_EINVAL; }
    int dev = 0, cus = 0;
    ADF_HIP_CHECK(hipGetDevice(&dev));
    ADF_HIP_CHECK(hipDeviceGetAttribute(&cus, hipDeviceAttributeMultiprocessorCount, dev));
    hipEvent_t e0, e1;
    ADF_HIP_CHECK(hipEventCreate(&e0));
    ADF_HIP_CHECK(hipEventCreate(&e1));
    float ms = 0.f;
    {
        const long long n4 = (1ll << 30) / 16;
        float4 *a = nullptr, *b = nullptr;
        ADF_HIP_CHECK(hipMalloc(&a, n4 * 16));
        ADF_HIP_CHECK(hipMalloc(&b, n4 * 16));
        ADF_HIP_CHECK(hipMemsetAsync(a, 1, n4 * 16, s));
        const dim3 grid((unsigned)((n4 + 255) / 256));
        hipLaunchKernelGGL(adf_peak_copy_kernel, grid, dim3(256), 0, s, a, b, n4);
        ADF_HIP_CHECK(hipEventRecord(e0, s));
        for (int i = 0; i < 5; ++i) hipLaunchKernelGGL(adf_peak_copy_kernel, grid, dim3(256), 0, s, a, b, n4);
        ADF_HIP_CHECK(hipEventRecord(e1, s));
        ADF_HIP_CHECK(hipEventSynchronize(e1));
        ADF_HIP_CHECK(hipEventElapsedTime(&ms, e0, e1));
        out_host3[0] = (float)(5.0 * 2.0 * (double)n4 * 16.0 / (ms * 1e-3) * 1e-9);
        (void)hipFree(a); (void)hipFree(b);
    }
    float* d = nullptr;
    ADF_HIP_CHECK(hipMalloc(&d, 64));
    const int iters = 4096;
    const double waves = (double)cus * 2 * 4;
    for (int f16 = 1; f16 >= 0; --f16) {
        for (int rep = 0; rep < 2; ++rep) {
            ADF_HIP_CHECK(hipEventRecord(e0, s));
            if (f16) hipLaunchKernelGGL(adf_peak_mfma_kernel<true>, dim3(cus * 2), dim3(256), 0, s, d, iters);
            else hipLaunchKernelGGL(adf_peak_mfma_kernel<false>, dim3(cus * 2), dim3(256), 0, s, d, iters);
            ADF_HIP_CHECK(hipEventRecord(e1, s));
            ADF_HIP_CHECK(hipEventSynchronize(e1));
            ADF_HIP_CHECK(hipEventElapsedTime(&ms, e0, e1));
        }
        const double flop = waves * iters * 4.0 * 2.0 * 32 * 32 * (f16 ? 16 : 2);
        out_host3[f16 ? 1 : 2] = (float)(flop / (ms * 1e-3) * 1e-12);
    }
    (void)hipFree(d);
    (void)hipEventDestroy(e0); (void)hipEventDestroy(e1);
    ADF_HIP_CHECK(hipGetLastError());
    return ADF_OK;
}
```

adsorbdiff_amd/engine.py:

```python
from __future__ import annotations

import ctypes as C
import logging
import os
from dataclasses import dataclass
from typing import List, Optional, Sequence

import torch

from . import lib as _lib


def cell_repeats(cell: torch.Tensor, radius: float, pbc: Sequence[bool] = (True, True, True)) -> List[int]:
    cell = cell.detach().to("cpu", torch.float32).reshape(-1, 3, 3)
    a1, a2, a3 = cell[:, 0], cell[:, 1], cell[:, 2]
    c23 = torch.cross(a2, a3, dim=-1)
    vol = torch.sum(a1 * c23, dim=-1, keepdim=True)
    crosses = (c23, torch.cross(a3, a1, dim=-1), torch.cross(a1, a2, dim=-1))
    reps = []
    for k in range(3):
        if pbc[k]:
            inv_min_dist = torch.norm(crosses[k] / vol, p=2, dim=-1)
            reps.append(int(torch.ceil(radius * inv_min_dist).max().item()))
        else:
# ... 277 lines not shown
        hp = _lib.Hparams(
            hidden_channels=model.hidden_channels, num_layers=model.num_layers, num_rbf=model.num_rbf,
            num_elements=model.num_elements, max_neighbors=model.max_neighbors,
            envelope_exponent=int(model.radial_basis.envelope.p),
            num_heads=getattr(model, "num_force_heads", 2 if model.so3_denoising else 1),
            cutoff=float(model.cutoff),
        )
        self.num_heads = hp.num_heads
        self.handle = C.c_void_p()
        with torch.cuda.device(self.device):
            _lib.check(self.lib.adf_painn_create(C.byref(hp), C.byref(self.handle)))
        self._last_graph_N = 0
        self._twin = None
        self._split_keepalive = None
        self._moving_gen = 0
        self._split_moving = None
        self._split_default = bool(self.get_tune()["sample_split"])
        floor = getattr(model, "distance_floor", None)
        if floor is not None:
            _lib.check(self.lib.adf_painn_set_distance_floor(self.handle, float(floor)))
        self.bind_weights()

    def _weight_list(self) -> List[torch.Tensor]:
        m = self.model
        sd = dict(m.named_parameters())
        sd.update(dict(m.named_buffers()))
        names = ["atom_emb.embeddings.weight", "radial_basis.rbf.offset"]
        for i in range(m.num_layers):
            p, u = f"message_layers.{i}.", f"update_layers.{i}."
            names += [
                p + "x_layernorm.weight", p + "x_layernorm.bias", p + "x_proj.0.weight", p + "x_proj.0.bias",
                p + "x_proj.2.weight", p + "x_proj.2.bias", p + "rbf_proj.weight", p + "rbf_proj.bias",
                u + "vec_proj.weight", u + "xvec_proj.0.weight", u + "xvec_proj.0.bias",
                u + "xvec_proj.2.weight", u + "xvec_proj.2.bias",
            ]
        heads = ["out_forces", "out_forces2"][:self.num_heads]
        for hname in heads:
            for b in range(2):
                q = f"{hname}.output_network.{b}."
                names += [q + "vec1_proj.weight", q + "vec2_proj.weight", q + "update_net.0.weight",
                          q + "update_net.0.bias", q + "update_net.2.weight", q + "update_net.2.bias"]
        out = []
        for n in names:
            t = sd[n].detach()
            _require_gpu(t, f"parameter {n}")
            if t.dtype != torch.float32 or not t.is_contiguous():
                t = t.to(torch.float32).contiguous()
            out.append(t)
        return out

    def bind_weights(self) -> None:
        ws = self._weight_list()
        self._weights_keepalive = ws
        ptrs = (C.c_void_p * len(ws))(*[w.data_ptr() for w in ws])
        scales = self.model.scale_factors()
        sf = (C.c_float * len(scales))(*scales)
        with torch.cuda.device(self.device):
            _lib.check(self.lib.adf_painn_set_weights(self.handle, len(ws), ptrs, sf, self._stream()))
        if getattr(self.model, "energy_head", False):
            oe = self.model.out_energy
            es = [t.detach().to(torch.float32).contiguous() for t in (oe[0].weight, oe[0].bias, oe[2].weight, oe[2].bias)]
            for t in es:
                _require_gpu(t, "out_energy parameter")
            self._weights_keepalive = ws + es
            eptrs = (C.c_void_p * 4)(*[t.data_ptr() for t in es])
            with torch.cuda.device(self.device):
                _lib.check(self.lib.adf_painn_set_energy_head(self.handle, 4, eptrs, self._stream()))

    def set_moving_atoms(self, prep, moving_mask) -> None:
        self._moving_gen += 1
        super().set_moving_atoms(prep, moving_mask)

    def split_view(self, prep: PreparedBatch, out_idx: Optional[torch.Tensor]):
        cached = getattr(prep, "_split_cut", None)
        if cached is None:
            off = prep.atom_offset.cpu()
            cut = split_cut((off[1:] - off[:-1]).tolist(), prep.edge_counts)
            na = int(off[cut])
            cached = prep._split_cut = (cut, na, (prep.atom_offset[cut:] - na).contiguous(), (prep.batch[na:] - cut).contiguous())
        cut, na, off_b, batch_b = cached
        v = _lib.SplitView()
        v.cut, v.atoms_a, v.atom_offset, v.batch = cut, na, off_b.data_ptr(), batch_b.data_ptr()
        keep = [off_b, batch_b]
        if out_idx is not None:
            n_a = int((out_idx < na).sum().item())
            keep.append((out_idx[n_a:] - na).contiguous())
            v.n_out_a, v.n_out_b, v.out_idx = n_a, int(out_idx.numel()) - n_a, keep[-1].data_ptr()
        if self._moving_keepalive is not None:
            if self._split_moving is None or self._split_moving[0] != (self._moving_gen, cut, na):
                _, idx, moff = self._moving_keepalive
                m0 = int(moff[cut].item())
                self._split_moving = ((self._moving_gen, cut, na), (idx[m0:] - na).contiguous(), (moff[cut:] - m0).contiguous())
            v.mov_idx, v.mov_off = self._split_moving[1].data_ptr(), self._split_moving[2].data_ptr()
        return v, keep

    def split_stats(self):
        a, b = C.c_int64(0), C.c_int64(0)
        _lib.check(self.lib.adf_split_stats(self.handle, C.byref(a), C.byref(b)))
        return int(a.value), int(b.value)

    def sample(self, prep: PreparedBatch, pos, f1, f2, coefs_dev: torch.Tensor, num_steps: int, state,
               z_tr_all=None, z_rot_all=None, early_stop_count: int = 10, poll_every: int = 0,
               out_idx: Optional[torch.Tensor] = None, sink=None, frame_every: int = 1,
               split_streams: Optional[bool] = None) -> None:
        want = self._split_default if split_streams is None else bool(split_streams)
        if not want or sink is not None or prep.num_systems < 2:
            return super().sample(prep, pos, f1, f2, coefs_dev, num_steps, state, z_tr_all, z_rot_all, early_stop_count,
                                  poll_every, out_idx, sink, frame_every)
        with torch.cuda.device(self.device):
            if self._twin is None:
                twin = C.c_void_p()
                _lib.check(self.lib.adf_painn_create_twin(self.handle, C.byref(twin)))
                self._twin = twin
            _lib.check(self.lib.adf_painn_set_split(self.handle, 1))
            view, keep = self.split_view(prep, out_idx)
            self._split_keepalive = keep
            desc = prep.desc(pos)
            _lib.check(self.lib.adf_sample_split(
                self.handle, self._twin, C.byref(desc), C.byref(view), pos.data_ptr(), prep.tags.data_ptr(), _ptr(prep.fixed),
                coefs_dev.data_ptr(), num_steps, _ptr(z_tr_all), _ptr(z_rot_all), early_stop_count, poll_every,
                state.data_ptr(), _ptr(out_idx), _numel(out_idx), f1.data_ptr(), f2.data_ptr(), self._stream()))

    def forward_prepared(self, prep: PreparedBatch, pos: torch.Tensor, f1: torch.Tensor, f2: Optional[torch.Tensor],
                         out_idx: Optional[torch.Tensor] = None) -> None:
        desc = prep.desc(pos)
        with torch.cuda.device(self.device):
            if out_idx is None:
                _lib.check(self.lib.adf_painn_forward(
                    self.handle, C.byref(desc), f1.data_ptr(), f2.data_ptr() if f2 is not None else None, self._stream()))
            else:
                assert out_idx.dtype == torch.int32 and out_idx.is_contiguous() and out_idx.device == pos.device
                _lib.check(self.lib.adf_painn_forward_subset(
                    self.handle, C.byref(desc), out_idx.data_ptr(), int(out_idx.numel()), f1.data_ptr(),
                    f2.data_ptr() if f2 is not None else None, self._stream()))

    def forward(self, data):
        prep = self.prepare(data)
        pos = data.pos.to(torch.float32).contiguous()
        f1 = torch.empty(prep.num_atoms, 3, dtype=torch.float32, device=self.device)
        f2 = torch.empty_like(f1) if self.model.so3_denoising else None
        self.forward_prepared(prep, pos, f1, f2)
        try:
            self.check_flags()
        except _lib.NumericRangeError:
            if not self.use_exact_f32():
                raise
            self.forward_prepared(prep, pos, f1, f2)
            self.check_flags()
        return f1, f2

    def forward_observe(self, data, upto: Optional[int] = None, with_heads: bool = False):
        L = int(self.model.num_layers)
        upto = L - 1 if upto is None else int(upto)
        prep = self.prepare(data)
        pos = data.pos.to(torch.float32).contiguous()
        layer_var = torch.full((L,), float("nan"), dtype=torch.float64, device=self.device)
        f1 = f2 = None
        if with_heads:
            f1 = torch.empty(prep.num_atoms, 3, dtype=torch.float32, device=self.device)
            f2 = torch.empty_like(f1) if self.num_heads == 2 else None
        self._moving_keepalive = None
        self._moving_gen += 1
        desc = prep.desc(pos)

        def run():
            with torch.cuda.device(self.device):
                _lib.check(self.lib.adf_painn_forward_observe(self.handle, C.byref(desc), upto, layer_var.data_ptr(),
                                                              _ptr(f1), _ptr(f2), self._stream()))
        run()
        try:
            self.check_flags()
        except _lib.NumericRangeError:
            if not self.use_exact_f32():
                raise
            run()
            self.check_flags()
        return (layer_var, f1, f2) if with_heads else layer_var

    def forward_energy_prepared(self, prep: PreparedBatch, pos: torch.Tensor, energy: torch.Tensor,
                                forces: Optional[torch.Tensor]) -> None:
        desc = prep.desc(pos)
        with torch.cuda.device(self.device):
            _lib.check(self.lib.adf_painn_forward_energy(
                self.handle, C.byref(desc), energy.data_ptr(), forces.data_ptr() if forces is not None else None,
                self._stream()))

    def forward_energy(self, data):
        prep = self.prepare(data)
        pos = data.pos.to(torch.float32).contiguous()
        energy = torch.empty(prep.num_systems, dtype=torch.float32, device=self.device)
        forces = torch.empty(prep.num_atoms, 3, dtype=torch.float32, device=self.device) if self.num_heads else None
        self.forward_energy_prepared(prep, pos, energy, forces)
        try:
            self.check_flags()
        except _lib.NumericRangeError:
            if not self.use_exact_f32():
                raise
            self.forward_energy_prepared(prep, pos, energy, forces)
            self.check_flags()
        return energy, forces

    def forward_energy_gradient_prepared(self, prep: PreparedBatch, pos: torch.Tensor, energy: torch.Tensor,
                                         forces: torch.Tensor) -> None:
        desc = prep.desc(pos)
        with torch.cuda.device(self.device):
            _lib.check(self.lib.adf_painn_forward_energy_gradient(
                self.handle, C.byref(desc), energy.data_ptr(), forces.data_ptr(), self._stream()))

    def forward_energy_gradient(self, data):
        prep = self.prepare(data)
        pos = data.pos.to(torch.float32).contiguous()
        energy = torch.empty(prep.num_systems, dtype=torch.float32, device=self.device)
        forces = torch.empty(prep.num_atoms, 3, dtype=torch.float32, device=self.device)
        self.forward_energy_gradient_prepared(prep, pos, energy, forces)
        try:
            self.check_flags()
        except _lib.NumericRangeError:
            if not self.use_exact_f32():
                raise
            self.forward_energy_gradient_prepared(prep, pos, energy, forces)
            self.check_flags()
        return energy, forces

    def energy_gradient_workspace_bytes(self, num_atoms: int) -> int:
        n = C.c_int64(0)
        _lib.check(self.lib.adf_painn_energy_gradient_workspace(self.handle, int(num_atoms), C.byref(n)))
        return int(n.value)

    def get_tune(self) -> dict:
        t = _lib.Tune()
        _lib.check(self.lib.adf_painn_get_tune(self.handle, C.byref(t)))
        return {name: int(getattr(t, name)) for name, _ in _lib.Tune._fields_}

    def build_graph(self, data, prep=None):
        if prep is None:
            prep = self.prepare(data)
        pos = data.pos.to(torch.float32).contiguous()
        desc = prep.desc(pos)
        n = C.c_int64(0)
        with torch.cuda.device(self.device):
            _lib.check(self.lib.adf_graph_build(self.handle, C.byref(desc), self._stream(), C.byref(n)))
        self._last_graph_N = prep.num_atoms
        return int(n.value)

    def export_graph(self):
        N, K = self._last_graph_N, self.model.max_neighbors
        if N <= 0:
            raise RuntimeError("export_graph: call build_graph first")
        dev = self.device
        cnt = torch.empty(N, dtype=torch.int32, device=dev)
        src = torch.empty(N, K, dtype=torch.int32, device=dev)
        sh = torch.empty(N, K, 3, dtype=torch.int32, device=dev)
        cap = 2 * N * K
        es = torch.empty(cap, dtype=torch.int32, device=dev)
        ed = torch.empty(cap, dtype=torch.int32, device=dev)
        dist = torch.empty(cap, dtype=torch.float32, device=dev)
        vec = torch.empty(cap, 3, dtype=torch.float32, device=dev)
        n = C.c_int64(0)
        with torch.cuda.device(dev):
            _lib.check(self.lib.adf_graph_export(
                self.handle, cnt.data_ptr(), src.data_ptr(), sh.data_ptr(), cap, es.data_ptr(), ed.data_ptr(),
                dist.data_ptr(), vec.data_ptr(), C.byref(n), self._stream()))
        E = int(n.value)
        return cnt, src, sh, es[:E], ed[:E], dist[:E], vec[:E]

    def message_layer(self, layer: int, x: torch.Tensor, vec: torch.Tensor):
        x_out, vec_out = torch.empty_like(x), torch.empty_like(vec)
        with torch.cuda.device(self.device):
            _lib.check(self.lib.adf_painn_message_layer(
                self.handle, layer, x.shape[0], x.data_ptr(), vec.data_ptr(), x_out.data_ptr(), vec_out.data_ptr(),
                self._stream()))
        return x_out, vec_out

    def update_layer(self, layer: int, x: torch.Tensor, vec: torch.Tensor):
        with torch.cuda.device(self.device):
            _lib.check(self.lib.adf_painn_update_layer(
                self.handle, layer, x.shape[0], x.data_ptr(), vec.data_ptr(), self._stream()))
        return x, vec

    def _sde_entry(self, coef, coefs_dev, num_steps):
        if coef is not None:
            return self.lib.adf_sde_step, (C.byref(coef),)
        return self.lib.adf_sde_step_scheduled, (coefs_dev.data_ptr(), num_steps)

    def counters(self) -> _lib.Counters:
        c = _lib.Counters()
        with torch.cuda.device(self.device):
            _lib.check(self.lib.adf_get_counters(self.handle, C.byref(c), self._stream()))
        return c

    PROFILE_CATEGORIES = ("graph", "message", "node_dense", "heads", "stepper")

    def profile_read(self):
        ms = (C.c_float * 5)()
        cnt = (C.c_int64 * 5)()
        ksteps = C.c_int64(0)
        with torch.cuda.device(self.device):
            _lib.check(self.lib.adf_profile_read(self.handle, ms, cnt, C.byref(ksteps), self._stream()))
        out = {k: (float(ms[i]), int(cnt[i])) for i, k in enumerate(self.PROFILE_CATEGORIES)}
        out["message_ksteps"] = int(ksteps.value)
        return out

    def measure_peaks(self):
        out = (C.c_float * 3)()
        with torch.cuda.device(self.device):
            _lib.check(self.lib.adf_measure_peaks(out, self._stream()))
        return {"hbm_copy_gbps": float(out[0]), "mfma_f16_tflops": float(out[1]), "mfma_f32_tflops": float(out[2])}
```

adsorbdiff_amd/lib.py:

```python
from __future__ import annotations

import ctypes as C
import re
from pathlib import Path

ADF_OK, ADF_EINVAL, ADF_EOOM, ADF_ENONEIGHBOR, ADF_EHIP, ADF_EOVERFLOW, ADF_ENUMERIC = 0, 1, 2, 3, 4, 5, 6


class NumericRangeError(ArithmeticError):
    """Non-finite model output (ADF_ENUMERIC).  Not a RuntimeError on purpose: ``ml_diffuse`` must not answer it by
    splitting the batch; the engine answers it by re-running in exact f32."""


class Hparams(C.Structure):
    _fields_ = [
        ("hidden_channels", C.c_int32), ("num_layers", C.c_int32), ("num_rbf", C.c_int32),
        ("num_elements", C.c_int32), ("max_neighbors", C.c_int32), ("envelope_exponent", C.c_int32),
        ("num_heads", C.c_int32), ("cutoff", C.c_float),
    ]


class EqV2Hparams(C.Structure):
    _fields_ = [
        ("lmax", C.c_int32), ("mmax", C.c_int32), ("num_layers", C.c_int32), ("sphere_channels", C.c_int32),
        ("attn_hidden_channels", C.c_int32), ("num_heads", C.c_int32), ("attn_alpha_channels", C.c_int32),
        ("attn_value_channels", C.c_int32), ("ffn_hidden_channels", C.c_int32), ("grid_resolution", C.c_int32),
        ("edge_channels", C.c_int32), ("num_distance_basis", C.c_int32), ("max_num_elements", C.c_int32),
        ("max_neighbors", C.c_int32), ("max_radius", C.c_float), ("avg_degree", C.c_float),
    ]


class EqV2Counters(C.Structure):
    _fields_ = [("num_edges", C.c_int64), ("num_atoms", C.c_int64), ("dense_flops", C.c_int64), ("conv_flops", C.c_int64),
                ("inc_rows", C.c_int64), ("inc_rows_full", C.c_int64), ("forwards_total", C.c_int64),
                ("conv_flops_total", C.c_int64)]


class Tune(C.Structure):
    _fields_ = [(name, C.c_int32) for name in (
        "gemm_stream", "head_gate_fused", "lift_emit", "graph_sys_csr", "train_gemm16", "wgrad_f32",
        "eqv2_gemm_tile256", "eqv2_rotin_generic", "eqv2_rotout_generic", "sample_split")]


class SplitView(C.Structure):
    _fields_ = [("cut", C.c_int32), ("atoms_a", C.c_int32), ("n_out_a", C.c_int32), ("n_out_b", C.c_int32),
                ("atom_offset", C.c_void_p), ("batch", C.c_void_p), ("out_idx", C.c_void_p), ("mov_idx", C.c_void_p),
                ("mov_off", C.c_void_p)]


class BatchDesc(C.Structure):
    _fields_ = [
        ("num_systems", C.c_int32), ("num_atoms", C.c_int32), ("pos", C.c_void_p), ("cell", C.c_void_p),
        ("atomic_numbers", C.c_void_p), ("batch", C.c_void_p), ("atom_offset", C.c_void_p), ("reps", C.c_int32 * 3),
    ]


class ActiveField(C.Structure):
    _fields_ = [("src", C.c_void_p), ("dst", C.c_void_p), ("row_bytes", C.c_int32), ("per_system", C.c_int32)]


class StepCoef(C.Structure):
    _fields_ = [
        ("coef_tr", C.c_float), ("rot_pre", C.c_float), ("rot_dt", C.c_float), ("rot_g2", C.c_float),
        ("noise_tr", C.c_float), ("noise_rot", C.c_float),
    ]


class TrCoef(C.Structure):
    _fields_ = [("coef", C.c_float), ("noise", C.c_float)]


class Counters(C.Structure):
    _fields_ = [
        ("num_edges", C.c_int64), ("num_atoms", C.c_int64), ("message_bytes_per_layer", C.c_int64),
        ("dense_flops", C.c_int64),
        ("inc_rows", C.c_int64), ("inc_rows_full", C.c_int64), ("inc_msg_launches", C.c_int64),
        ("inc_msg_edges", C.c_int64),
    ]


HEADER = Path(__file__).resolve().parent.parent / "include" / "adsorbdiff_hip.h"

_SCALARS = {"int32_t": C.c_int32, "int64_t": C.c_int64, "float": C.c_float, "double": C.c_double}
_RETURNS = {"int32_t": C.c_int32, "int64_t": C.c_int64, "const char*": C.c_char_p}
_BYREF = {"adf_batch": BatchDesc, "adf_painn_hparams": Hparams, "adf_eqv2_hparams": EqV2Hparams, "adf_tune": Tune,
          "adf_counters": Counters, "adf_eqv2_counters": EqV2Counters, "adf_active_field": ActiveField}


def parse_header(text: str) -> dict:
    text = re.sub(r"/\*.*?\*/|//[^\n]*", " ", text, flags=re.S)
    text = re.sub(r"^[ \t]*#.*$", " ", text, flags=re.M)
    structs = set(re.findall(r"typedef\s+struct\s*\w*\s*\{[^}]*\}\s*(\w+)\s*;", text))
    text = re.sub(r"(typedef\s+struct|enum)\s*\w*\s*\{[^}]*\}\s*\w*\s*;", " ", text)
    handles = set(re.findall(r"typedef\s+struct\s+\w+\s*\*\s*(adf_\w+_t)\s*;", text))
    text = re.sub(r"typedef\s+struct\s+\w+\s*\*\s*adf_\w+_t\s*;|extern\s+\"C\"\s*\{|\}", " ", text)
    pointees = set(_SCALARS) | structs | handles | {"void", "char", "uint8_t"}

    def argtype(fn: str, param: str):
        tokens = [t for t in re.findall(r"\w+|\*|\S", param) if t != "const"]
        base, stars, name = tokens[:1], tokens[1:-1], tokens[-1:]
        if len(tokens) < 2 or any(t != "*" for t in stars) or not re.fullmatch(r"[A-Za-z_]\w*", name[0]) or name[0] in pointees:
            raise ValueError(f"{fn}: parameter {param.strip()!r} is not `type name`")
        base = base[0]
        if stars:
            if base not in pointees:
                raise ValueError(f"{fn}: parameter {param.strip()!r} points to the unknown type {base!r}")
            return C.POINTER(_BYREF[base]) if base in _BYREF and len(stars) == 1 else C.c_void_p
        if base in handles:
            return C.c_void_p
        if base not in _SCALARS:
            raise ValueError(f"{fn}: parameter {param.strip()!r} has the unknown type {base!r}")
        return _SCALARS[base]

    out = {}
    for stmt in filter(None, (s.strip() for s in text.split(";"))):
        m = re.fullmatch(r"(.*?)\b(adf_[a-z_0-9]+)\s*\((.*)\)", stmt, flags=re.S)
        if m is None:
            raise ValueError(f"not a prototype, an enum, a struct or a handle typedef: {' '.join(stmt.split())!r}")
        ret, fn, params = re.sub(r"\s*\*\s*", "*", " ".join(m.group(1).split())), m.group(2), m.group(3).strip()
        if ret not in _RETURNS:
            raise ValueError(f"{fn}: unknown return type {ret!r}")
        if fn in out:
            raise ValueError(f"{fn}: declared twice")
        out[fn] = (_RETURNS[ret], [] if params == "void" else [argtype(fn, p) for p in params.split(",")])
    return out


SIGNATURES = parse_header(HEADER.read_text())
EXPORTS = tuple(SIGNATURES)
SPLIT_HEADER = HEADER.with_name("adsorbdiff_split.h")
SPLIT_SIGNATURES = {name: sig for name, sig in parse_header(HEADER.read_text() + "\n" + SPLIT_HEADER.read_text()).items()
                    if name not in SIGNATURES}
SCALE_FIT_HEADER = HEADER.with_name("adsorbdiff_scale_fit.h")
SCALE_FIT_SIGNATURES = {name: sig for name, sig in parse_header(HEADER.read_text() + "\n" + SCALE_FIT_HEADER.read_text()).items()
                        if name not in SIGNATURES}
SLABS_HEADER = HEADER.with_name("adsorbdiff_slabs.h")
SLABS_SIGNATURES = {name: sig for name, sig in parse_header(HEADER.read_text() + "\n" + SLABS_HEADER.read_text()).items()
                    if name not in SIGNATURES}

_LIB = None


def lib_path() -> Path:
    import os

    override = os.environ.get("ADF_LIB_PATH")
    if override:
        return Path(override)
    return Path(__file__).resolve().parent / "libadsorbdiff_hip.so"


def load():
    global _LIB
    if _LIB is not None:
        return _LIB
    path = lib_path()
    if not path.exists():
        raise RuntimeError(
            f"{path} not found: build it with `python -m adsorbdiff_amd.build` "
            "(the HIP path has no CPU fallback)"
        )
    lib = C.CDLL(str(path))
    for name, (restype, argtypes) in {**SIGNATURES, **SPLIT_SIGNATURES, **SCALE_FIT_SIGNATURES, **SLABS_SIGNATURES}.items():
        fn = getattr(lib, name)
        fn.restype, fn.argtypes = restype, argtypes
    _LIB = lib
    return lib


def check(status: int) -> None:
    if status == ADF_OK:
        return
    msg = load().adf_last_error().decode("utf-8", "replace")
    if status == ADF_ENONEIGHBOR:
        raise ValueError(msg)
    if status == ADF_EOVERFLOW:
        raise ValueError(f"adsorbdiff_hip: capacity exceeded: {msg}")
    if status == ADF_EOOM:
        raise RuntimeError(f"HIP out of memory: {msg}")
    if status == ADF_ENUMERIC:
        raise NumericRangeError(msg)
    if status == ADF_EINVAL:
        raise ValueError(f"adsorbdiff_hip: invalid argument: {msg}")
    raise RuntimeError(f"adsorbdiff_hip error {status}: {msg}")
```

include/adsorbdiff_hip.h:

```cpp
#ifndef ADSORBDIFF_HIP_H
#define ADSORBDIFF_HIP_H

#include <stdint.h>

#ifdef __cplusplus
extern "C" {
#endif

#define ADF_OK 0
#define ADF_EINVAL 1
#define ADF_EOOM 2
#define ADF_ENONEIGHBOR 3
#define ADF_EHIP 4
#define ADF_EOVERFLOW 5
#define ADF_ENUMERIC 6

typedef struct adf_painn* adf_painn_t;

typedef struct {
    int32_t hidden_channels;
    int32_t num_layers;
    int32_t num_rbf;
    int32_t num_elements;
    int32_t max_neighbors;
    int32_t envelope_exponent;
    int32_t num_heads;
    float cutoff;
} adf_painn_hparams;

#define ADF_WEIGHTS_PER_LAYER 13
#define ADF_WEIGHTS_PER_HEAD 12

int32_t adf_painn_create(const adf_painn_hparams* hp, adf_painn_t* out);
int32_t adf_painn_destroy(adf_painn_t h);

int32_t adf_painn_set_weights(adf_painn_t h, int32_t n_weights, const void* const* weights,
                              const float* scale_factors, void* stream);

typedef struct {
    int32_t num_systems;
    int32_t num_atoms;
    const float* pos;
    const float* cell;
    const int32_t* atomic_numbers;
    const int32_t* batch;
    const int32_t* atom_offset;
    int32_t reps[3];
} adf_batch;

int32_t adf_graph_build(adf_painn_t h, const adf_batch* b, void* stream, int64_t* num_edges);

int32_t adf_graph_set_moving(adf_painn_t h, const int32_t* moving, const int32_t* mov_idx, const int32_t* mov_off);

int32_t adf_painn_set_arithmetic(adf_painn_t h, int32_t exact_f32);

int32_t adf_painn_set_incremental(adf_painn_t h, int32_t on);

typedef struct adf_tune {
    int32_t gemm_stream;
    int32_t head_gate_fused;
    int32_t lift_emit;
    int32_t graph_sys_csr;
    int32_t train_gemm16;
    int32_t wgrad_f32;
    int32_t eqv2_gemm_tile256;
    int32_t eqv2_rotin_generic;
    int32_t eqv2_rotout_generic;
    int32_t sample_split;
} adf_tune;
int32_t adf_painn_get_tune(adf_painn_t h, adf_tune* out);

int32_t adf_check_flags(adf_painn_t h, void* stream);

int32_t adf_graph_export(adf_painn_t h, int32_t* nbr_count, int32_t* nbr_src, int32_t* nbr_shift,
                         int64_t edge_capacity, int32_t* edge_src, int32_t* edge_dst, float* edge_dist,
                         float* edge_vec, int64_t* num_edges, void* stream);

int32_t adf_painn_forward(adf_painn_t h, const adf_batch* b, float* f1, float* f2, void* stream);

int32_t adf_painn_forward_subset(adf_painn_t h, const adf_batch* b, const int32_t* out_idx, int32_t n_out, float* f1,
                                 float* f2, void* stream);

int32_t adf_painn_message_layer(adf_painn_t h, int32_t layer, int32_t num_atoms, const float* x,
                                const float* vec, float* x_out, float* vec_out, void* stream);
int32_t adf_painn_update_layer(adf_painn_t h, int32_t layer, int32_t num_atoms, float* x, float* vec,
                               void* stream);
int32_t adf_painn_debug_row_maxima(adf_painn_t h, int32_t which, float* out, int64_t capacity, int32_t* rows,
                                   void* stream);

int32_t adf_linear_forward(const float* A, const float* W, const float* bias, float* C, int32_t M, int32_t N,
                           int32_t K, int32_t act_ssilu, int32_t mode, void* stream);

typedef struct {
    float coef_tr;
    float rot_pre;
    float rot_dt;
    float rot_g2;
    float noise_tr;
    float noise_rot;
} adf_step_coef;

int32_t adf_sde_init_placement(adf_painn_t h, const adf_batch* b, float* pos, const int32_t* tags,
                               const float* noise, void* stream);

int32_t adf_sde_step(adf_painn_t h, const adf_batch* b, float* pos, const int32_t* tags,
                     const int32_t* fixed, const float* f1, const float* f2, const adf_step_coef* coef,
                     const float* z_tr, const float* z_rot, int32_t early_stop_count, int32_t* state,
                     float* dcom, float* drot, void* stream);

int32_t adf_sde_step_scheduled(adf_painn_t h, const adf_batch* b, float* pos, const int32_t* tags,
                               const int32_t* fixed, const float* f1, const float* f2,
                               const adf_step_coef* coefs_dev, int32_t num_steps, const float* z_tr,
                               const float* z_rot, int32_t early_stop_count, int32_t* state, float* dcom,
                               float* drot, void* stream);

int32_t adf_sample(adf_painn_t h, const adf_batch* b, float* pos, const int32_t* tags, const int32_t* fixed,
                   const adf_step_coef* coefs_dev, int32_t num_steps, const float* z_tr_all, const float* z_rot_all,
                   int32_t early_stop_count, int32_t poll_every, int32_t* state, const int32_t* out_idx,
                   int32_t n_out, float* f1, float* f2, void* stream);

typedef struct {
    float coef;
    float noise;
} adf_tr_coef;

int32_t adf_tr_step(adf_painn_t h, const adf_batch* b, float* pos, const int32_t* tags, const float* f1,
                    const adf_tr_coef* coef, const adf_tr_coef* coefs_dev, int32_t num_steps, const float* z,
                    int32_t early_stop_count, int32_t* state, float* dcom, void* stream);
int32_t adf_tr_sample(adf_painn_t h, const adf_batch* b, float* pos, const int32_t* tags, const adf_tr_coef* coefs_dev,
                      int32_t num_steps, const float* z_all, int32_t early_stop_count, int32_t poll_every,
                      int32_t* state, const int32_t* out_idx, int32_t n_out, float* f1, void* stream);

typedef struct {
    int64_t num_edges;
    int64_t num_atoms;
    int64_t message_bytes_per_layer;
    int64_t dense_flops;
    int64_t inc_rows, inc_rows_full, inc_msg_launches, inc_msg_edges;
} adf_counters;
int32_t adf_get_counters(adf_painn_t h, adf_counters* out, void* stream);

int32_t adf_painn_set_per_system_stop(adf_painn_t h, int32_t* sys_state, int32_t B);

#define ADF_PROF_NCAT 5
int32_t adf_profile_enable(adf_painn_t h, int32_t on);
int32_t adf_profile_read(adf_painn_t h, float* ms, int64_t* count, int64_t* message_ksteps, void* stream);

int32_t adf_measure_peaks(float* out_host3, void* stream);

typedef struct adf_frames* adf_frames_t;
int32_t adf_frames_create(int32_t device, int64_t frame_floats, int32_t slots, adf_frames_t* out);
int32_t adf_frames_destroy(adf_frames_t f);
int32_t adf_frames_push(adf_frames_t f, const float* src, void* stream);
int32_t adf_frames_wait(adf_frames_t f, int64_t index, int32_t timeout_ms, const float** host_ptr);
int32_t adf_frames_release(adf_frames_t f, int64_t index);
int64_t adf_frames_pushed(adf_frames_t f);
int32_t adf_frames_abort(adf_frames_t f);
int32_t adf_sample_traj(adf_painn_t h, const adf_batch* b, float* pos, const int32_t* tags, const int32_t* fixed,
                        const adf_step_coef* coefs_dev, int32_t num_steps, const float* z_tr_all, const float* z_rot_all,
                        int32_t early_stop_count, int32_t poll_every, int32_t* state, const int32_t* out_idx,
                        int32_t n_out, float* f1, float* f2, adf_frames_t sink, int32_t frame_every, void* stream);
int32_t adf_tr_sample_traj(adf_painn_t h, const adf_batch* b, float* pos, const int32_t* tags,
                           const adf_tr_coef* coefs_dev, int32_t num_steps, const float* z_all, int32_t early_stop_count,
                           int32_t poll_every, int32_t* state, const int32_t* out_idx, int32_t n_out, float* f1,
                           adf_frames_t sink, int32_t frame_every, void* stream);

int32_t adf_lift_adsorbates(float* pos, const int32_t* tags, const int32_t* atom_offset, int32_t B, float min_gap,
                            float* lifted, void* stream);

int32_t adf_flag_anomalies(const adf_batch* b, const float* pos_final, const float* pos_slab_ref, const int32_t* tags,
                           const float* radii, int32_t num_radii, float skin, float surface_mult, float desorption_mult,
                           int32_t* flags, void* stream);

int32_t adf_select_best_sites(const float* energy, const int32_t* flags, const int32_t* group_offset, int32_t num_groups,
                              int32_t* best, float* best_energy, int32_t* n_valid, void* stream);

int32_t adf_site_pair_distances(const float* pos, const float* cell, const int32_t* tags, const int32_t* atomic_numbers,
                                const int32_t* atom_offset, const int32_t* group_offset, const int64_t* pair_offset,
                                int32_t num_atoms, int32_t num_sites, int32_t num_groups, int64_t out_len,
                                int32_t include_slab, int32_t permutation_invariant, float* out, void* stream);
int32_t adf_unique_sites(const float* dist, const int32_t* group_offset, const int64_t* pair_offset, int32_t num_sites,
                         int32_t num_groups, int64_t dist_len, const float* energy, const int32_t* flags, float tol,
                         float energy_tol, int32_t* rep, int32_t* n_unique, void* stream);
int32_t adf_select_top_sites(const float* energy, const int32_t* flags, const int32_t* rep, const int32_t* group_offset,
                             int32_t num_groups, int32_t k, int32_t* top, float* top_energy, void* stream);

int64_t adf_slab_symmetry_scratch(int32_t num_atoms, int32_t num_slabs);
int32_t adf_slab_symmetry_search(const float* pos, const float* cell, const int32_t* atomic_numbers,
                                 const int32_t* atom_offset, int32_t num_atoms, int32_t num_slabs, double symprec,
                                 int32_t proper_only, void* scratch, int32_t* n_ops, int32_t* n_ops_host, void* stream);
int32_t adf_slab_symmetry_emit(const int32_t* atom_offset, int32_t num_atoms, int32_t num_slabs, double symprec,
                               const void* scratch, const int32_t* op_offset, const int64_t* perm_offset, int32_t num_ops,
                               int64_t perm_len, double* rot, double* trans, int32_t* W, int32_t* perm, void* stream);
int32_t adf_site_pair_distances_sym(const float* pos, const float* cell, const int32_t* tags, const int32_t* atomic_numbers,
                                    const int32_t* atom_offset, const int32_t* group_offset, const int64_t* pair_offset,
                                    int32_t num_atoms, int32_t num_sites, int32_t num_groups, int64_t out_len,
                                    int32_t include_slab, int32_t permutation_invariant, const int32_t* op_offset,
                                    const double* rot, const double* trans, const int32_t* perm, const int64_t* perm_offset,
                                    int32_t num_ops, int64_t perm_len, float* out, int32_t* best_op, void* stream);

int32_t adf_place_draws(int64_t seed, const int64_t* keys, const int32_t* index, int32_t n, double* out, void* stream);
int32_t adf_place_adsorbates(const adf_batch* slabs, const int32_t* slab_of, const float* site, const double* draws,
                             const int32_t* ads_offset, const float* ads_pos, const int32_t* ads_Z, const float* radii,
                             int32_t num_radii, const float* masses, int32_t num_masses, float interstitial_gap,
                             int32_t mode, const int32_t* binding_idx, const int32_t* pbc, int32_t P,
                             const int32_t* out_row, int64_t out_rows, float* out_pos, double* scaled_normal,
                             int32_t* n_combos, double* rot_meta, void* stream);
int32_t adf_place_site_candidates(const float* tri, const int32_t* tri_offset, const int32_t* per_tri,
                                  const int32_t* cand_offset, const int32_t* cand_slab, const float* cell,
                                  const double* draws, int32_t B, int32_t num_candidates, float* cand, int32_t* keep,
                                  void* stream);
int32_t adf_interstitial_distances(const adf_batch* b, const int32_t* tags, const float* radii, int32_t num_radii,
                                   const float* masses, int32_t num_masses, const int32_t* pbc, float* out, void* stream);

int32_t adf_surface_site_candidates(const float* pos, const int32_t* tags, const int32_t* atom_offset, const float* cell,
                                    const float* tri, const int32_t* tri_offset, int32_t num_atoms, int32_t num_triangles,
                                    int32_t num_slabs, int32_t capacity, int32_t* seg_offset, float* cand, int32_t* valid,
                                    void* stream);
int32_t adf_reduce_sites(const float* cand, const int32_t* valid, const int32_t* seg_offset, const int32_t* seg_slab,
                         const float* cell, int32_t num_candidates, int32_t num_segments, int32_t num_slabs,
                         const int32_t* op_offset, const double* rot, const double* trans, int32_t num_ops, double tol,
                         int32_t* first, int32_t* rep, int32_t* multiplicity, int32_t* counts, void* stream);

int32_t adf_surface_triangles(const float* pos, const int32_t* tags, const int32_t* atom_offset, const float* cell,
                              int32_t num_atoms, int32_t num_slabs, double circle_tol, int32_t capacity,
                              int32_t* tri_offset, float* tri, int32_t* tri_index, void* stream);

int32_t adf_voronoi_coordination(const float* pos, const float* cell, const int32_t* pbc, const int32_t* atom_offset,
                                 int32_t num_atoms, int32_t num_systems, const int32_t* select, double cutoff,
                                 double weight_tol, double far, double* cn, double* omega_max, int32_t* nn, int32_t* flags,
                                 void* stream);
int32_t adf_bulk_coordination_min(const double* cn, const int32_t* flags, const int32_t* atomic_numbers,
                                  const int32_t* atom_offset, int32_t num_atoms, int32_t num_systems, double* table,
                                  void* stream);
int32_t adf_tag_surface_atoms(const float* pos, const float* cell, const int32_t* pbc, const int32_t* atomic_numbers,
                              const int32_t* atom_offset, int32_t num_atoms, int32_t num_systems, const double* masses,
                              const double* bulk_cn_min, double height, double cutoff, double weight_tol, double far,
                              double cn_tol, int32_t* tags, double* cn, int32_t* flags, void* stream);

#define ADF_COMM_ID_BYTES 128
typedef struct adf_comm* adf_comm_t;
int32_t adf_comm_unique_id(uint8_t* out128);
int32_t adf_comm_create(const uint8_t* id128, int32_t rank, int32_t world, adf_comm_t* out);
int32_t adf_comm_destroy(adf_comm_t comm);
int32_t adf_allgather_sites(adf_comm_t comm, const void* local, int64_t bytes_per_rank, void* out, void* stream);

int32_t adf_op_linear_fwd(const float* A, int32_t lda, const float* W, const float* bias, float* C, int32_t ldc, int64_t M,
                          int32_t N, int32_t K, void* stream);
int64_t adf_op_linear_bwd_scratch(int64_t M, int32_t N, int32_t K);
int32_t adf_op_linear_bwd(const float* A, int32_t lda, const float* W, const float* dC, int32_t ldc, float* dA, int32_t ldda,
                          int32_t acc_dA, float* dW, float* db, int32_t acc_dW, int64_t M, int32_t N, int32_t K,
                          float* scratch, void* stream);
int32_t adf_op_ssilu_fwd(const float* h, float* y, int64_t n, void* stream);
int32_t adf_op_ssilu_bwd(const float* h, const float* dy, float* dh, int64_t n, void* stream);
int32_t adf_op_layernorm_fwd(const float* x, const float* w, const float* b, float* y, float* stats, int32_t N, int32_t H,
                             void* stream);
int32_t adf_op_layernorm_bwd(const float* x, const float* w, const float* stats, const float* dy, float* dx, float* dw,
                             float* db, int32_t N, int32_t H, float* scratch, void* stream);
int32_t adf_op_embed_fwd(adf_painn_t h, const int32_t* Z, int32_t N, float* x, void* stream);
int32_t adf_op_embed_bwd(const float* dx, const int32_t* Z, float* demb, int32_t N, int32_t H, void* stream);
int32_t adf_op_rbf(adf_painn_t h, float* rbf, void* stream);
int32_t adf_op_message_fwd(adf_painn_t h, const float* xh, const float* vec, const float* rbfh, const float* x, float* x1,
                           float* vec1, int32_t vec_is_zero, void* stream);
int32_t adf_op_message_fwd_fused(adf_painn_t h, int32_t layer, const float* xh, const float* vec, const float* x, float* x1,
                                 float* vec1, int32_t vec_is_zero, void* stream);
int32_t adf_op_message_bwd(adf_painn_t h, const float* xh, const float* vec, const float* rbfh, const float* gx1,
                           const float* gv1, float* dxh, float* drbfh, float* dvec, float* dx, int32_t vec_is_zero,
                           void* stream);
int32_t adf_op_message_bwd_fused_supported(adf_painn_t h);
int32_t adf_op_message_bwd_perm(adf_painn_t h, int32_t* perm_host, int32_t n);
int32_t adf_op_message_bwd_fused(adf_painn_t h, int32_t layer, const float* xh, const float* vec, const float* gx1,
                                 const float* gv1, float* dxh, float* drbfh_lane_order, int64_t num_edges, float* dvec,
                                 float* dx, int32_t vec_is_zero, float* dbias_rows, void* stream);
int32_t adf_op_edge_owner(adf_painn_t h, int32_t* edge_owner, int64_t num_edges, void* stream);
int64_t adf_op_rbf_image_bytes(int64_t num_edges);
int32_t adf_op_rbf_image(adf_painn_t h, const float* rbf, int64_t num_edges, void* image, void* stream);
int64_t adf_op_rbf_wgrad_fused_scratch(adf_painn_t h);
int32_t adf_op_rbf_wgrad_fused(adf_painn_t h, const float* xh, const float* vec, const void* rbf_image, const int32_t* edge_owner,
                               int64_t num_edges, float* dW, float* scratch, int32_t vec_is_zero, void* stream);
int32_t adf_op_vdot_fwd(const float* vv, float* dot, float* nrm, int32_t ldn, int64_t N, int32_t C, float eps, void* stream);
int32_t adf_op_vdot_bwd(const float* vv, const float* nrm, int32_t ldn, const float* ddot, const float* dnrm, int32_t lddn,
                        const float* dv1, float* dvv, int64_t N, int32_t C, void* stream);
int32_t adf_op_update_out_fwd(const float* x1, const float* vec1, const float* a, const float* dot, const float* vv, float s,
                              float* x2, float* vec2, int64_t N, int32_t H, void* stream);
int32_t adf_op_update_out_bwd(const float* a, const float* dot, const float* vv, float s, const float* dx2,
                              const float* dvec2, float* da, float* ddot, float* dv1, float* dx1, float* dvec1, int64_t N,
                              int32_t H, void* stream);
int32_t adf_op_vnorm_fwd(const float* t1, float* nrm, int32_t ldn, int64_t N, int32_t C, void* stream);
int32_t adf_op_vnorm_bwd(const float* t1, const float* nrm, int32_t ldn, const float* dnrm, int32_t lddn, float* dt1,
                         int64_t N, int32_t C, void* stream);
int32_t adf_op_gate_fwd(const float* o, const float* t2, float* xs, int32_t ldx, float* vout, int64_t N, int32_t C,
                        void* stream);
int32_t adf_op_gate_bwd(const float* o, const float* t2, const float* dxs, int32_t lddx, const float* dvout, float* d_o,
                        float* dt2, int64_t N, int32_t C, void* stream);
int32_t adf_op_copy_rows(const float* src, int32_t lds_, float* dst, int32_t ldd, int64_t M, int32_t C, int32_t accumulate,
                         void* stream);
int32_t adf_op_score_loss(const float* f1, const float* f2, const int32_t* tags, const int32_t* atom_offset,
                          const float* tr_sigma, const float* rot_sigma, const float* tr_score, const float* rot_score,
                          const float* rot_norm, float* loss, float* df1, float* df2, int32_t B, float* scratch, void* stream);
int32_t adf_op_score_loss_tr(const float* f1, const int32_t* tags, const int32_t* atom_offset, const float* tr_sigma,
                             const float* tr_score, float* loss, float* df1, int32_t B, float* scratch, void* stream);

int32_t adf_noise_draws(int64_t seed, int32_t step, const int64_t* keys, int32_t B, double* out, void* stream);
int32_t adf_sampler_draws(int64_t seed, const int64_t* keys, const int32_t* site, int32_t B, int32_t T, float* place,
                          float* z_a, float* z_b, void* stream);
int32_t adf_noise_tr_so3(const float* pos, const float* cell, const int32_t* tags, const int32_t* atom_offset, int32_t B,
                         int32_t N, const double* draws, float ads_std_low, float ads_std_high, float rot_std_low,
                         float rot_std_high, const double* omegas, const double* cdf, const double* score,
                         const double* exp_score_norm, int32_t n_eps, int32_t n_omega, float* pos_out, float* tr_sigma,
                         float* rot_sigma, float* tr_score, float* rot_score, float* noise_vec, float* rot_norm,
                         void* stream);
int32_t adf_noise_com(const float* pos, const float* cell, const int32_t* tags, const int32_t* atom_offset, int32_t B,
                      int32_t N, const double* draws, float ads_std_low, float ads_std_high, float* pos_out,
                      float* tr_sigma, float* tr_score, float* noise_vec, void* stream);
int32_t adf_igso3_score_norm(const float* rot_sigma, const double* table, int32_t n_eps, int32_t B, float* out, void* stream);
int32_t adf_op_s2ef_loss(const float* E_pred, const float* F_pred, const float* E_tgt, const float* F_tgt,
                         const int32_t* fixed, const int32_t* atom_offset, int32_t B, int32_t free_only, float mean_E,
                         float std_E, float mean_F, float std_F, float c_E, float c_F, const int64_t* counts, float* loss,
                         float* dE, float* dF, float* metrics, float* scratch, void* stream);
int64_t adf_op_s2ef_loss_scratch(int32_t B);
int32_t adf_op_energy_sum(const float* y, int32_t H2, const float* w, const float* bias, const int32_t* atom_offset,
                          float* energy, int32_t B, void* stream);
int32_t adf_op_energy_head_bwd(const float* he0, const float* w2, const float* dE, const int32_t* atom_sys, float* dhe0,
                               float* dW2, float* db2, int32_t accumulate, int64_t N, int32_t H2, float* scratch,
                               void* stream);
int64_t adf_op_energy_head_bwd_scratch(int64_t N, int32_t H2);
int32_t adf_op_sqnorm_accumulate(const float* g, int64_t n, float* out, void* stream);
int32_t adf_op_adamw_step(float* p, const float* g, float* m, float* v, float* ema, int64_t n, const float* sqnorm,
                          float max_norm, float lr, float beta1, float beta2, float eps, float weight_decay, int32_t step,
                          float ema_decay, void* stream);

int64_t adf_op_optimizer_chunk(void);
int32_t adf_op_grad_sqnorm_multi(const void* tensors, const void* chunks, int32_t nchunks, float* partials, void* state,
                                 float max_norm, double beta1, double beta2, float ema_decay, int64_t ema_updates0,
                                 void* stream);
int32_t adf_op_adamw_multi(const void* tensors, const void* chunks, int32_t nchunks, const void* state, float lr, float beta1,
                           float beta2, float eps, float weight_decay, void* stream);
int32_t adf_op_embed_bwd_ordered(const float* dx, const int32_t* Z, float* demb, int32_t N, int32_t H, int32_t rows,
                                 float* scratch, void* stream);
int64_t adf_op_embed_bwd_ordered_scratch(int64_t N, int32_t H, int32_t rows);

enum {
    ADF_EVAL_ENERGY_MAE = 0,
    ADF_EVAL_FORCESX_MAE = 1,
    ADF_EVAL_FORCESY_MAE = 2,
    ADF_EVAL_FORCESZ_MAE = 3,
    ADF_EVAL_FORCES_MAE = 4,
    ADF_EVAL_FORCES_COSINE_SIMILARITY = 5,
    ADF_EVAL_FORCES_MAGNITUDE_ERROR = 6,
    ADF_EVAL_ENERGY_FORCES_WITHIN_THRESHOLD = 7,
    ADF_EVAL_POSITIONS_AVERAGE_DISTANCE_WITHIN_THRESHOLD = 8,
    ADF_EVAL_POSITIONS_MAE = 9,
    ADF_EVAL_POSITIONS_MSE = 10,
    ADF_EVAL_ENERGY_MSE = 11,
    ADF_EVAL_ENERGY_WITHIN_THRESHOLD = 12,
    ADF_EVAL_LOSS = 13,
    ADF_EVAL_SLOTS = 14
};
int64_t adf_eval_scratch(int32_t B);
int32_t adf_eval_s2ef(const float* E_pred, const float* F_pred, const float* E_tgt, const float* F_tgt,
                      const int32_t* fixed, const int32_t* atom_offset, int32_t B, int32_t N, int32_t free_only,
                      float mean_E, float std_E, float mean_F, float std_F, double* total, int64_t* numel, double* scratch,
                      void* stream);
int32_t adf_eval_is2rs(const float* pos_pred, const float* pos_tgt, const float* cell, const int32_t* fixed,
                       const int32_t* atom_offset, int32_t B, int32_t N, const double* thresholds, int32_t T,
                       double* total, int64_t* numel, double* scratch, void* stream);
int32_t adf_eval_is2re(const float* E_pred, const float* E_tgt, int32_t B, double* total, int64_t* numel, void* stream);
int32_t adf_eval_add(const float* value, int32_t slot, double* total, int64_t* numel, void* stream);

typedef struct adf_eqv2* adf_eqv2_t;
typedef struct {
// ... 144 lines not shown
```

Baseline: 263.0.

## Add 16x16x32 MFMA path for f16x3 GEMM with swizzled LDS layout

Adds a second instruction shape to the split-f16 GEMM kernel, using 16x16x32 MFMA instead of 32x32 tiles. It brings a new weight fragment packing order, an XOR-swizzled LDS layout to avoid bank conflicts, and a re-mapped epilogue. By default it is enabled only for fused-bias epilogue weights (mask value 2); other GEMMs keep the 32x32 shape. This aims at better MFMA throughput and latency on gfx950 for these shapes, at the cost of more instructions, more register pressure and a new fragment mapping that must stay correct. A peak-measurement kernel for the new instruction is also added.

New measurement: 264.7, median of 6. No clear change (+0.6%).

```diff
diff --git a/adsorbdiff_amd/csrc/api.hip b/adsorbdiff_amd/csrc/api.hip
--- a/adsorbdiff_amd/csrc/api.hip
+++ b/adsorbdiff_amd/csrc/api.hip
@@ -33,6 +33,8 @@
     t.eqv2_rotin_generic = getenv("ADF_EQV2_ROTIN_GENERIC") != nullptr;
     t.eqv2_rotout_generic = getenv("ADF_EQV2_ROTOUT_GENERIC") != nullptr;
     t.sample_split = off_is_0("ADF_SAMPLE_SPLIT");
+    const char* m16 = getenv("ADF_GEMM_MFMA16");
+    t.gemm_mfma16 = m16 ? atoi(m16) & 3 : 0;
     return t;
 }
 const adf_tune& adf_tune_process() {
@@ -139,6 +141,7 @@
         const char* er = getenv("ADF_ROW_MAXIMA");
         h->rmx = (er && atoi(er) == 0) ? 0 : 1;
         h->tune = adf_tune_from_env();
+        if (!getenv("ADF_GEMM_MFMA16")) h->tune.gemm_mfma16 = ADF_GEMM_MFMA16_DEFAULT;
     }
     if (st == ADF_OK) st = m.alloc(&h->kcount, 8);
     if (st == ADF_OK && hipMemset(h->kcount, 0, 8 * sizeof(unsigned long long)) != hipSuccess) st = ADF_EHIP;
@@ -313,9 +316,11 @@
             } else {
                 ADF_TRY(adf_split_weight(w, n, out, h->w16_scratch, s));
             }
+            out->frag16 = 0;
             if (rows % 32 == 0 && K % 16 == 0) {
+                out->frag16 = (h->tune.gemm_mfma16 >> (fused_bias ? 1 : 0)) & 1 && K % 32 == 0;
                 out->frag = fcur; fcur += n * 4;
-                ADF_TRY(adf_pack_frag(out, (int)rows, (int)K, out->frag, s));
+                ADF_TRY(adf_pack_frag(out, (int)rows, (int)K, out->frag, s, out->frag16));
             }
             return ADF_OK;
         };
diff --git a/adsorbdiff_amd/csrc/common.h b/adsorbdiff_amd/csrc/common.h
--- a/adsorbdiff_amd/csrc/common.h
+++ b/adsorbdiff_amd/csrc/common.h
@@ -17,6 +17,7 @@
     float* inv_scale;
     float* bias_perm;
     void* frag;
+    int frag16 = 0;
 };
 struct adf_epi {
     const float* vec_in;
@@ -195,6 +196,7 @@
 
 int32_t adf_launch_gemm(const float* A, int lda, const float* W, int ldw, const float* bias, float* C, int ldc,
                         int M, int N, int K, int act_ssilu, hipStream_t s);
+#define ADF_GEMM_MFMA16_DEFAULT 2
 adf_tune adf_tune_from_env();
 const adf_tune& adf_tune_process();
 int adf_current_num_cus();
@@ -222,7 +224,7 @@
     return adf_launch_gemm16(A, lda, W16, bias, C, ldc, M, N, K, act, &ep, s, h->lift_on ? &h->lift : nullptr, h->tune,
                              h->num_cus);
 }
-int32_t adf_pack_frag(const adf_w16* w, int N, int K, void* out, hipStream_t s);
+int32_t adf_pack_frag(const adf_w16* w, int N, int K, void* out, hipStream_t s, int shape16 = 0);
 int32_t adf_graph_build_impl(adf_painn* h, const adf_batch* b, hipStream_t s);
 int32_t adf_energy_sum(const float* y, int H2, const float* w, const float* bias, const int32_t* atom_offset, float* energy,
                        int num_systems, hipStream_t s);
diff --git a/adsorbdiff_amd/csrc/energy_grad.hip b/adsorbdiff_amd/csrc/energy_grad.hip
--- a/adsorbdiff_amd/csrc/energy_grad.hip
+++ b/adsorbdiff_amd/csrc/energy_grad.hip
@@ -242,7 +242,8 @@
         cur += e * 8;
         out->w16.inv_scale = g->wscales + nscale++;
         ADF_TRY(adf_split_weight(w, e, &out->w16, h->w16_scratch, s));
-        return adf_pack_frag(&out->w16, (int)n, (int)k, out->w16.frag, s);
+        out->w16.frag16 = h->tune.gemm_mfma16 & 1;
+        return adf_pack_frag(&out->w16, (int)n, (int)k, out->w16.frag, s, out->w16.frag16);
     };
     auto transposed = [&](const float* w, long long n, long long k, EgW* out) -> int32_t {
         float* t = reinterpret_cast<float*>(cur);
diff --git a/adsorbdiff_amd/csrc/frag_map.h b/adsorbdiff_amd/csrc/frag_map.h
--- /dev/null
+++ b/adsorbdiff_amd/csrc/frag_map.h
@@ -0,0 +1,22 @@
+#pragma once
+
+#if defined(__HIPCC__)
+#define ADF_FRAG_HD __host__ __device__
+#else
+#define ADF_FRAG_HD
+#endif
+
+ADF_FRAG_HD constexpr int g16_swz(int row) { return ((row >> 2) ^ (row >> 3)) & 1; }
+
+ADF_FRAG_HD inline long long adf_frag_total(int N, int K) { return (long long)N * K / 4; }
+
+ADF_FRAG_HD inline long long adf_frag_src(long long i, int K, int shape16, int* plane) {
+    const int lane = (int)(i & 63);
+    *plane = (int)((i >> 6) & 1);
+    const long long cs = i >> 7;
+    const int steps = shape16 ? K / 32 : K / 16;
+    const int s = (int)(cs % steps);
+    const long long cb = cs / steps;
+    if (shape16) return (16 * cb + (lane & 15)) * K + 32 * s + 8 * (lane >> 4);
+    return (32 * cb + (lane & 31)) * K + 16 * s + 8 * (lane >> 5);
+}
diff --git a/adsorbdiff_amd/csrc/gemm16.hip b/adsorbdiff_amd/csrc/gemm16.hip
--- a/adsorbdiff_amd/csrc/gemm16.hip
+++ b/adsorbdiff_amd/csrc/gemm16.hip
@@ -1,8 +1,10 @@
 #include <stdlib.h>
 
 #include "common.h"
+#include "frag_map.h"
 
 typedef float f32x16 __attribute__((ext_vector_type(16)));
+typedef float f32x4 __attribute__((ext_vector_type(4)));
 typedef _Float16 half8 __attribute__((ext_vector_type(8)));
 typedef _Float16 half4 __attribute__((ext_vector_type(4)));
 
@@ -32,13 +34,18 @@
     return {nwn, mi, nj, 64 * nwm * nwn, tm, 32 * nj * nwn, epi >= 3 ? tm / 3 : tm};
 }
 
-template <int ACT, int EPI, bool STREAM>
+#define G16_SJ(r) (SHAPE == 16 ? ((r) >> 2) & 1 : 0)
+#define G16_ROW(r) (SHAPE == 16 ? 16 * ((r) >> 3) + 4 * (lane >> 4) + ((r) & 3) : ((r) & 3) + 8 * ((r) >> 2) + 4 * (lane >> 5))
+#define G16_COL(r) (SHAPE == 16 ? 16 * G16_SJ(r) + (lane & 15) : lane & 31)
+
+template <int ACT, int EPI, bool STREAM, int SHAPE>
 __global__ __launch_bounds__(g16_tile_of(EPI, STREAM).NT, 2) void adf_gemm_f16x3_kernel(
     const float* __restrict__ A, int lda, const _Float16* __restrict__ Whi, const _Float16* __restrict__ Wlo,
     const float* __restrict__ inv_scale, const float* __restrict__ bias, float* __restrict__ C, int ldc, int Mh, int N,
     int K, int tiles_n, adf_epi ep) {
     constexpr g16_tile geo = g16_tile_of(EPI, STREAM);
     constexpr int MI = geo.MI, NJ = geo.NJ, NWN = geo.NWN, NT = geo.NT, TM = geo.TM, TN = geo.TN;
+    static_assert(SHAPE == 32 || SHAPE == 16, "MFMA shape");
     const int M = ep.m_dev ? min(Mh, (int)*ep.m_dev) : Mh;
     constexpr int NA = TM * 8 / NT;
     static_assert(TM * 8 % NT == 0, "A staging: whole float4s per thread");
@@ -83,7 +90,7 @@
         const int row = f >> 3, kq = f & 7;
         const unsigned int grow = global_row(row);
         a_goff[i] = (grow * (unsigned int)lda + kq * 4) * 4u;
-        a_off[i] = row * HLD + kq * 4;
+        a_off[i] = SHAPE == 16 ? row * HLD + (((kq >> 1) ^ g16_swz(row)) * 8 + (kq & 1) * 4) : row * HLD + kq * 4;
         a_rs[i] = ep.rmag ? adf_pow2_lift(ep.rmag[grow]) : 1.0f;
     }
     if (tid < TM) rinv[tid] = ep.rmag ? 1.0f / adf_pow2_lift(ep.rmag[global_row(tid)]) : 1.0f;
@@ -96,7 +103,7 @@
         const int f = tid + 256 * i;
         const int row = f >> 2, part = f & 3;
         w_src[i] = min(n0 + row, N - 1) * K + part * 8;
-        w_off[i] = row * HLD + part * 8;
+        w_off[i] = SHAPE == 16 ? row * HLD + (part ^ g16_swz(row)) * 8 : row * HLD + part * 8;
     }
 
     float4 ra[NA];
@@ -120,19 +127,43 @@
             wf[j][1] = wfr[base + 64];
         }
     };
-    if constexpr (STREAM) load_wf(0, wfa);
+    half8 wga[2 * NJ][2], wgb[2 * NJ][2];
+    const half8* const wgr = reinterpret_cast<const half8*>(Whi) + (size_t)((n0 + wn) / 16) * (K / 32) * 128 + lane;
+    auto load_wf16 = [&](int kt_, half8 (&wf)[2 * NJ][2]) {
+#pragma unroll
+        for (int j = 0; j < 2 * NJ; ++j) {
+            const size_t base = ((size_t)j * (K / 32) + kt_) * 128;
+            wf[j][0] = wgr[base];
+            wf[j][1] = wgr[base + 64];
+        }
+    };
+    if constexpr (STREAM) {
+        if constexpr (SHAPE == 16) load_wf16(0, wga);
+        else load_wf(0, wfa);
+    }
 
     f32x16 acc[MI][NJ];
+    f32x4 acc16[MI][NJ][4];
 #pragma unroll
     for (int i = 0; i < MI; ++i)
 #pragma unroll
         for (int j = 0; j < NJ; ++j)
 #pragma unroll
-            for (int r = 0; r < 16; ++r) acc[i][j][r] = 0.f;
+            for (int r = 0; r < 16; ++r) {
+                if constexpr (SHAPE == 16) acc16[i][j][r >> 2][r & 3] = 0.f;
+                else acc[i][j][r] = 0.f;
+            }
+#define accr(i, j, r) (SHAPE == 16 ? acc16[i][j][(r) >> 2][(r) & 3] : acc[i][j][r])
+    auto mma16 = [&](int b, int jb, const half8& ah, const half8& al, const half8& bh, const half8& bl) {
+        f32x4& c = acc16[b >> 1][jb >> 1][(b & 1) * 2 + (jb & 1)];
+        c = __builtin_amdgcn_mfma_f32_16x16x32_f16(al, bh, c, 0, 0, 0);
+        c = __builtin_amdgcn_mfma_f32_16x16x32_f16(ah, bl, c, 0, 0, 0);
+        c = __builtin_amdgcn_mfma_f32_16x16x32_f16(ah, bh, c, 0, 0, 0);
+    };
 
     const int nk = K / HK;
-    const int fa = (wm + (lane & 31)) * HLD + (lane >> 5) * 8;
-    const int fb = (wn + (lane & 31)) * HLD + (lane >> 5) * 8;
+    const int fa = SHAPE == 16 ? (wm + (lane & 15)) * HLD + ((lane >> 4) ^ g16_swz(lane & 15)) * 8 : (wm + (lane & 31)) * HLD + (lane >> 5) * 8;
+    const int fb = SHAPE == 16 ? (wn + (lane & 15)) * HLD + ((lane >> 4) ^ g16_swz(lane & 15)) * 8 : (wn + (lane & 31)) * HLD + (lane >> 5) * 8;
     auto stage_a = [&](int boff = 0) {
 #pragma unroll
         for (int i = 0; i < NA; ++i) {
@@ -197,6 +228,47 @@
                     *reinterpret_cast<half4*>(Alo + boff + a_off[i]) = l;
                 }
             };
+            if constexpr (SHAPE == 16) {
+            auto khalf = [&](int boff, int hb, const half8 (&cur)[2 * NJ][2]) {
+#pragma unroll
+                for (int bi = 0; bi < MI; ++bi) {
+                    const int b = hb * MI + bi;
+                    const half8 ah = *reinterpret_cast<const half8*>(Ahi + boff + fa + b * 16 * HLD);
+                    const half8 al = *reinterpret_cast<const half8*>(Alo + boff + fa + b * 16 * HLD);
+#pragma unroll
+                    for (int jb = 0; jb < 2 * NJ; ++jb) mma16(b, jb, ah, al, cur[jb][0], cur[jb][1]);
+                }
+            };
+            auto tile16 = [&](int kt, int cur, const float4 (&nxt_regs)[NA], const half8 (&w0)[2 * NJ][2], half8 (&w1)[2 * NJ][2]) {
+                load_wf16(min(kt + 1, nk - 1), w1);
+                __builtin_amdgcn_sched_barrier(0);
+                khalf(cur, 0, w0);
+                __builtin_amdgcn_sched_barrier(0);
+                khalf(cur, 1, w0);
+                stage_from(nxt_regs, BUF - cur);
+                __builtin_amdgcn_sched_group_barrier(0x100, 2 * MI, 0);
+#pragma unroll
+                for (int u = 0; u < 3 * MI * NJ; ++u) {
+                    __builtin_amdgcn_sched_group_barrier(0x8, 2, 0);
+                    __builtin_amdgcn_sched_group_barrier(0x2, 4, 0);
+                    if (u % 3 == 2) __builtin_amdgcn_sched_group_barrier(0x200, 1, 0);
+                }
+                __builtin_amdgcn_sched_barrier(0);
+            };
+            __syncthreads();
+            stage_a(0);
+            request_a(min(1, nk - 1));
+            request_b(min(2, nk - 1));
+            __syncthreads();
+            for (int kt = 0; kt < nk; kt += 2) {
+                tile16(kt, 0, ra, wga, wgb);
+                request_a(min(kt + 3, nk - 1));
+                __syncthreads();
+                tile16(kt + 1, BUF, rb, wgb, wga);
+                request_b(min(kt + 4, nk - 1));
+                __syncthreads();
+            }
+            } else {
             half8 wfc[NJ][2], wfd[NJ][2];
             load_wf(1, wfb);
             auto tile = [&](int kt, int cur, const float4 (&nxt_regs)[NA], const half8 (&w0)[NJ][2], const half8 (&w1)[NJ][2],
@@ -231,6 +303,7 @@
                 request_b(min(kt + 4, nk - 1));
                 __syncthreads();
             }
+            }
         }
     } else {
     for (int kt = 0; kt < nk; ++kt) {
@@ -251,6 +324,26 @@
                 rwl[i] = *reinterpret_cast<const half8*>(Wlo + w_src[i] + k1);
             }
         }
+        if constexpr (SHAPE == 16) {
+            constexpr int NP = NJ > 3 ? 2 : 1, JB = 2 * NJ / NP;
+#pragma unroll
+            for (int p = 0; p < NP; ++p) {
+                half8 bh[JB], bl[JB];
+#pragma unroll
+                for (int jb = 0; jb < JB; ++jb) {
+                    bh[jb] = *reinterpret_cast<const half8*>(Bhi + fb + (p * JB + jb) * 16 * HLD);
+                    bl[jb] = *reinterpret_cast<const half8*>(Blo + fb + (p * JB + jb) * 16 * HLD);
+                }
+#pragma unroll
+                for (int b = 0; b < 2 * MI; ++b) {
+                    const half8 ah = *reinterpret_cast<const half8*>(Ahi + fa + b * 16 * HLD);
+                    const half8 al = *reinterpret_cast<const half8*>(Alo + fa + b * 16 * HLD);
+#pragma unroll
+                    for (int jb = 0; jb < JB; ++jb) mma16(b, p * JB + jb, ah, al, bh[jb], bl[jb]);
+                }
+                if (NP > 1) __builtin_amdgcn_sched_barrier(0);
+            }
+        } else {
 #pragma unroll
         for (int ks = 0; ks < 2; ++ks) {
             half8 bh[NJ], bl[NJ];
@@ -271,27 +364,34 @@
                 }
             }
         }
+        }
     }
     }
 
     const float isc = *inv_scale;
     if constexpr (EPI == 0) {
         if (((N | ldc) & 3) == 0 && (reinterpret_cast<uintptr_t>(C) & 15) == 0 && NJ % 2 == 0) {
-            const int q = lane & 31;
             __syncthreads();
             float* T = reinterpret_cast<float*>(lds) + wave * (32 * TLD2);
 #pragma unroll
             for (int jj = 0; jj < NJ / 2; ++jj) {
                 const int cb = n0 + wn + 64 * jj;
-                const float bv0 = (bias && cb + q < N) ? bias[cb + q] : 0.f;
-                const float bv1 = (bias && cb + 32 + q < N) ? bias[cb + 32 + q] : 0.f;
+                const int q0 = G16_COL(0);
+                const float bv0 = (bias && cb + q0 < N) ? bias[cb + q0] : 0.f;
+                const float bv1 = (bias && cb + 32 + q0 < N) ? bias[cb + 32 + q0] : 0.f;
+                float bw0 = 0.f, bw1 = 0.f;
+                if constexpr (SHAPE == 16) {
+                    const int q1 = G16_COL(4);
+                    bw0 = (bias && cb + q1 < N) ? bias[cb + q1] : 0.f;
+                    bw1 = (bias && cb + 32 + q1 < N) ? bias[cb + 32 + q1] : 0.f;
+                }
 #pragma unroll
                 for (int i = 0; i < MI; ++i) {
 #pragma unroll
                     for (int r = 0; r < 16; ++r) {
-                        const int lr = (r & 3) + 8 * (r >> 2) + 4 * (lane >> 5);
+                        const int lr = G16_ROW(r), q = G16_COL(r);
                         const float sc = isc * rinv[wm + 32 * i + lr];
-                        float v0 = acc[i][2 * jj][r] * sc + bv0, v1 = acc[i][2 * jj + 1][r] * sc + bv1;
+                        float v0 = accr(i, 2 * jj, r) * sc + (G16_SJ(r) ? bw0 : bv0), v1 = accr(i, 2 * jj + 1, r) * sc + (G16_SJ(r) ? bw1 : bv1);
                         if (ACT) { v0 = adf_ssilu(v0); v1 = adf_ssilu(v1); }
                         T[lr * TLD2 + q] = v0;
                         T[lr * TLD2 + 32 + q] = v1;
@@ -326,6 +426,31 @@
             }
             return;
         }
+        if constexpr (SHAPE == 16) {
+#pragma unroll
+            for (int j2 = 0; j2 < NJ * 2; ++j2) {
+                const int j = j2 >> 1, c = j2 & 1;
+                const int col = n0 + wn + 32 * j + G16_COL(4 * c);
+                if (col >= N) continue;
+                const float bv = bias ? bias[col] : 0.f;
+#pragma unroll
+                for (int i = 0; i < MI; ++i) {
+#pragma unroll
+                    for (int r = 0; r < 16; ++r) {
+                        if (G16_SJ(r) != c) continue;
+                        const int row = m0 + wm + 32 * i + G16_ROW(r);
+                        if (row < M) {
+                            float v = accr(i, j, r) * (isc * rinv[row - m0]) + bv;
+                            if (ACT) v = adf_ssilu(v);
+                            if (ep.accumulate) v += C[(size_t)row * ldc + col];
+                            C[(size_t)row * ldc + col] = v;
+                            if (ep.out_mag) atomicMax(ep.out_mag + row, __float_as_uint(fabsf(v)));
+                        }
+                    }
+                }
+            }
+            return;
+        }
 #pragma unroll
         for (int j = 0; j < NJ; ++j) {
             const int col = n0 + wn + 32 * j + (lane & 31);
@@ -348,7 +473,6 @@
         }
     } else if constexpr (EPI == 3) {
         static_assert(EPI != 3 || (NJ == 2 && MI == 3), "vec_proj epilogue: 3 components x (v1, v2)");
-        const int q = lane & 31;
         const int g = (n0 + wn) / 64;
         const int H = ep.H;
         const float inv_sqrt_h = 1.0f / sqrtf((float)H);
@@ -358,12 +482,12 @@
         float dv[16], nv[16];
 #pragma unroll
         for (int r = 0; r < 16; ++r) {
-            const int lr = (r & 3) + 8 * (r >> 2) + 4 * (lane >> 5);
+            const int lr = G16_ROW(r), q = G16_COL(r);
             float d = 0.f, qq = 0.f;
 #pragma unroll
             for (int i = 0; i < 3; ++i) {
                 const float sc = isc * rinv[wm + 32 * i + lr];
-                const float v1 = acc[i][0][r] * sc, v2 = acc[i][1][r] * sc;
+                const float v1 = accr(i, 0, r) * sc, v2 = accr(i, 1, r) * sc;
                 d += v1 * v2;
                 qq += v2 * v2;
                 T[lr * TLD3 + i * 32 + q] = v1;
@@ -391,7 +515,7 @@
         __builtin_amdgcn_wave_barrier();
 #pragma unroll
         for (int r = 0; r < 16; ++r) {
-            const int lr = (r & 3) + 8 * (r >> 2) + 4 * (lane >> 5);
+            const int lr = G16_ROW(r), q = G16_COL(r);
             T[lr * TLD3 + q] = dv[r];
             T[lr * TLD3 + 32 + q] = nv[r];
         }
@@ -416,18 +540,17 @@
         }
     } else if constexpr (EPI == 4) {
         static_assert(EPI != 4 || (NJ == 2 && MI == 3), "norm epilogue: 3 components x 64 columns per wave");
-        const int q = lane & 31;
         const int cb = n0 + wn;
         __syncthreads();
         float* T = reinterpret_cast<float*>(lds) + wave * 3200;
         const int a0 = m0 + (wave / NWN) * 32;
 #pragma unroll
         for (int r = 0; r < 16; ++r) {
-            const int lr = (r & 3) + 8 * (r >> 2) + 4 * (lane >> 5);
+            const int lr = G16_ROW(r), q = G16_COL(r);
 #pragma unroll
             for (int j = 0; j < 2; ++j) {
-                const float a = acc[0][j][r] * (isc * rinv[wm + lr]), b = acc[1][j][r] * (isc * rinv[wm + 32 + lr]),
-                            d = acc[2][j][r] * (isc * rinv[wm + 64 + lr]);
+                const float a = accr(0, j, r) * (isc * rinv[wm + lr]), b = accr(1, j, r) * (isc * rinv[wm + 32 + lr]),
+                            d = accr(2, j, r) * (isc * rinv[wm + 64 + lr]);
                 T[lr * TLD2 + j * 32 + q] = sqrtf(a * a + b * b + d * d);
             }
         }
@@ -444,25 +567,29 @@
         static_assert(EPI >= 3 || (NJ == 3 && MI == 2), "fused epilogues are written for the 64 x 96 wave tile");
         if (((EPI_ABL & 1) && EPI == 1) || ((EPI_ABL & 2) && EPI == 2)) {
             float sacc = 0.f;
-            for (int i = 0; i < MI; ++i) for (int j = 0; j < NJ; ++j) for (int r = 0; r < 16; ++r) sacc += acc[i][j][r];
+            for (int i = 0; i < MI; ++i) for (int j = 0; j < NJ; ++j) for (int r = 0; r < 16; ++r) sacc += accr(i, j, r);
             if (ep.H < 0) ep.x[0] = sacc;
             return;
         }
-        const int q = lane & 31;
         const int g = (n0 + wn) / 96;
         const int H = ep.H;
-        const float b0 = bias[n0 + wn + q], b1 = bias[n0 + wn + 32 + q], b2 = bias[n0 + wn + 64 + q];
+        float b0[SHAPE == 16 ? 2 : 1], b1[SHAPE == 16 ? 2 : 1], b2[SHAPE == 16 ? 2 : 1];
+#pragma unroll
+        for (int c = 0; c < (SHAPE == 16 ? 2 : 1); ++c) {
+            const int q = G16_COL(4 * c);
+            b0[c] = bias[n0 + wn + q]; b1[c] = bias[n0 + wn + 32 + q]; b2[c] = bias[n0 + wn + 64 + q];
+        }
         __syncthreads();
         float* T = reinterpret_cast<float*>(lds) + wave * 3200;
 #pragma unroll
         for (int i = 0; i < MI; ++i) {
 #pragma unroll
             for (int r = 0; r < 16; ++r) {
-                const int lr = (r & 3) + 8 * (r >> 2) + 4 * (lane >> 5);
+                const int lr = G16_ROW(r), q = G16_COL(r);
                 const float sc = isc * rinv[wm + 32 * i + lr];
-                T[lr * TLD3 + q] = acc[i][0][r] * sc + b0;
-                T[lr * TLD3 + 32 + q] = acc[i][1][r] * sc + b1;
-                T[lr * TLD3 + 64 + q] = acc[i][2][r] * sc + b2;
+                T[lr * TLD3 + q] = accr(i, 0, r) * sc + b0[G16_SJ(r)];
+                T[lr * TLD3 + 32 + q] = accr(i, 1, r) * sc + b1[G16_SJ(r)];
+                T[lr * TLD3 + 64 + q] = accr(i, 2, r) * sc + b2[G16_SJ(r)];
             }
             __builtin_amdgcn_fence(__ATOMIC_RELEASE, "wavefront");
             __builtin_amdgcn_wave_barrier();
@@ -563,6 +690,11 @@
     }
 }
 
+#undef accr
+#undef G16_ROW
+#undef G16_COL
+#undef G16_SJ
+
 __global__ __launch_bounds__(256) void adf_rowmag_kernel(const float* __restrict__ A, int lda, int K1,
                                                          const float* __restrict__ A2, int K2, long long M,
                                                          float* __restrict__ mag, const int32_t* __restrict__ m_dev,
@@ -672,22 +804,19 @@
 }
 
 __global__ void adf_pack_frag_kernel(const _Float16* __restrict__ hi, const _Float16* __restrict__ lo, half8* __restrict__ out,
-                                     int N, int K) {
-    const int nks = K / 16;
-    const long long total = (long long)(N / 32) * nks * 2 * 64;
+                                     int N, int K, int shape16) {
+    const long long total = adf_frag_total(N, K);
     for (long long i = (long long)blockIdx.x * blockDim.x + threadIdx.x; i < total; i += (long long)gridDim.x * blockDim.x) {
-        const int lane = (int)(i & 63), plane = (int)((i >> 6) & 1);
-        const long long cs = i >> 7;
-        const int s = (int)(cs % nks), cb = (int)(cs / nks);
-        const _Float16* src = (plane ? lo : hi) + (size_t)(32 * cb + (lane & 31)) * K + 16 * s + 8 * (lane >> 5);
-        out[i] = *reinterpret_cast<const half8*>(src);
-    }
-}
-
-int32_t adf_pack_frag(const adf_w16* w, int N, int K, void* out, hipStream_t s) {
-    if (N % 32 || K % 16) { adf_set_error("pack_frag: N %% 32 or K %% 16"); return ADF_EINVAL; }
+        int plane;
+        const long long e = adf_frag_src(i, K, shape16, &plane);
+        out[i] = *reinterpret_cast<const half8*>((plane ? lo : hi) + e);
+    }
+}
+
+int32_t adf_pack_frag(const adf_w16* w, int N, int K, void* out, hipStream_t s, int shape16) {
+    if (N % 32 || K % 16 || (shape16 && K % 32)) { adf_set_error("pack_frag: N %% 32 or K %% 16 (16x16x32 image: K %% 32)"); return ADF_EINVAL; }
     hipLaunchKernelGGL(adf_pack_frag_kernel, dim3(256), dim3(256), 0, s, (const _Float16*)w->hi, (const _Float16*)w->lo,
-                       (half8*)out, N, K);
+                       (half8*)out, N, K, shape16);
     ADF_HIP_CHECK(hipGetLastError());
     return ADF_OK;
 }
@@ -700,22 +829,26 @@
     return ADF_OK;
 }
 
+static bool g16_shape16(const adf_tune& tune, int epi) { return (tune.gemm_mfma16 >> ((epi == 1 || epi == 2) ? 1 : 0)) & 1; }
+
 static bool can_stream(const adf_tune& tune, const adf_w16* W, int epi, int N, int K) {
-    return tune.gemm_stream && W->frag && N % g16_tile_of(epi, true).TN == 0 && (K / HK) % 2 == 0;
-}
-
-static int32_t launch_f16x3(bool stream, int act, int epi, const float* A, int lda, const adf_w16* W, const float* bias, float* C,
+    return tune.gemm_stream && W->frag && (W->frag16 != 0) == g16_shape16(tune, epi) && N % g16_tile_of(epi, true).TN == 0 &&
+           (K / HK) % 2 == 0;
+}
+
+static int32_t launch_f16x3(bool stream, bool shape16, int act, int epi, const float* A, int lda, const adf_w16* W, const float* bias, float* C,
                             int ldc, int M, int N, int K, const adf_epi& ep, hipStream_t s) {
-    using kern_t = decltype(&adf_gemm_f16x3_kernel<0, 0, false>);
-#define G16_FORM(STREAM_)                                                                                              \
-    { adf_gemm_f16x3_kernel<0, 0, STREAM_>, adf_gemm_f16x3_kernel<1, 0, STREAM_>, adf_gemm_f16x3_kernel<0, 1, STREAM_>, \
-      adf_gemm_f16x3_kernel<0, 2, STREAM_>, adf_gemm_f16x3_kernel<0, 3, STREAM_>, adf_gemm_f16x3_kernel<0, 4, STREAM_> }
-    static const kern_t kernels[2][6] = {G16_FORM(false), G16_FORM(true)};
+    using kern_t = decltype(&adf_gemm_f16x3_kernel<0, 0, false, 32>);
+#define G16_FORM(STREAM_, SHAPE_)                                                                        \
+    { adf_gemm_f16x3_kernel<0, 0, STREAM_, SHAPE_>, adf_gemm_f16x3_kernel<1, 0, STREAM_, SHAPE_>,        \
+      adf_gemm_f16x3_kernel<0, 1, STREAM_, SHAPE_>, adf_gemm_f16x3_kernel<0, 2, STREAM_, SHAPE_>,        \
+      adf_gemm_f16x3_kernel<0, 3, STREAM_, SHAPE_>, adf_gemm_f16x3_kernel<0, 4, STREAM_, SHAPE_> }
+    static const kern_t kernels[2][2][6] = {{G16_FORM(false, 32), G16_FORM(true, 32)}, {G16_FORM(false, 16), G16_FORM(true, 16)}};
 #undef G16_FORM
     const g16_tile t = g16_tile_of(epi, stream);
     const int tiles_n = (N + t.TN - 1) / t.TN;
     const int tiles_m8 = ((M + t.ROWS - 1) / t.ROWS + 7) / 8 * 8;
-    hipLaunchKernelGGL(kernels[stream][epi ? epi + 1 : (act ? 1 : 0)], dim3((unsigned)(tiles_m8 * tiles_n)), dim3(t.NT), 0, s, A, lda,
+    hipLaunchKernelGGL(kernels[shape16][stream][epi ? epi + 1 : (act ? 1 : 0)], dim3((unsigned)(tiles_m8 * tiles_n)), dim3(t.NT), 0, s, A, lda,
                        (const _Float16*)(stream ? W->frag : W->hi), (const _Float16*)(stream ? nullptr : W->lo), W->inv_scale,
                        bias, C, ldc, M, N, K, tiles_n, ep);
     ADF_HIP_CHECK(hipGetLastError());
@@ -744,7 +877,7 @@
     const long long wg = (long long)((M + ts.ROWS - 1) / ts.ROWS) * (N / ts.TN > 0 ? N / ts.TN : 1);
     const long long slots = 2ll * (num_cus > 0 ? num_cus : 256);
     const bool ragged4 = wg < 4 * slots && wg % slots != 0 && wg % slots < (3 * slots) / 10 && wg > slots;
-    return launch_f16x3(can_stream(tune, W, 0, N, K) && !ragged4, act_ssilu, 0, A, lda, W, bias, C, ldc, M, N, K, ep, s);
+    return launch_f16x3(can_stream(tune, W, 0, N, K) && !ragged4, g16_shape16(tune, 0), act_ssilu, 0, A, lda, W, bias, C, ldc, M, N, K, ep, s);
 }
 
 int32_t adf_launch_gemm16_vecnorm(const float* A, int lda, const adf_w16* W, float* nrm, int M, int N, int K,
@@ -755,7 +888,7 @@
     adf_epi ep = {};
     ep.cat = nrm;
     ADF_TRY(lift_mags(A, lda, K, nullptr, 0, 3ll * M, lf, premag, &ep.rmag, s));
-    return launch_f16x3(can_stream(tune, W, 4, N, K), 0, 4, A, lda, W, nullptr, nullptr, 0, M, N, K, ep, s);
+    return launch_f16x3(can_stream(tune, W, 4, N, K), g16_shape16(tune, 4), 0, 4, A, lda, W, nullptr, nullptr, 0, M, N, K, ep, s);
 }
 
 int32_t adf_launch_gemm16_fused(const float* A, int lda, const adf_w16* W, int M, int H, int K, int epi,
@@ -770,5 +903,5 @@
     ADF_TRY(check_a_span((long long)rows_per * M, lda));
     ADF_TRY(lift_mags(A, lda, K, nullptr, 0, (long long)rows_per * M, lf, ep_in->rmag, &ep.rmag, s, ep_in->m_dev, rows_per));
     const int N = (epi == 3 ? 2 : 3) * H;
-    return launch_f16x3(can_stream(tune, W, epi, N, K), 0, epi, A, lda, W, epi == 3 ? nullptr : W->bias_perm, nullptr, 0, M, N, K, ep, s);
-}
+    return launch_f16x3(can_stream(tune, W, epi, N, K), g16_shape16(tune, epi), 0, epi, A, lda, W, epi == 3 ? nullptr : W->bias_perm, nullptr, 0, M, N, K, ep, s);
+}
diff --git a/adsorbdiff_amd/csrc/peaks.hip b/adsorbdiff_amd/csrc/peaks.hip
--- a/adsorbdiff_amd/csrc/peaks.hip
+++ b/adsorbdiff_amd/csrc/peaks.hip
@@ -1,6 +1,8 @@
 #include "common.h"
+#include "../../include/adsorbdiff_peaks.h"
 
 typedef float f32x16 __attribute__((ext_vector_type(16)));
+typedef float f32x4 __attribute__((ext_vector_type(4)));
 typedef _Float16 half8 __attribute__((ext_vector_type(8)));
 
 __global__ void adf_peak_copy_kernel(const float4* __restrict__ src, float4* __restrict__ dst, long long n4) {
@@ -38,7 +40,32 @@
     if (sum == 123.456f) out[0] = sum;
 }
 
-extern "C" int32_t adf_measure_peaks(float* out_host3, void* stream) {
+__global__ __launch_bounds__(256, 2) void adf_peak_mfma16_kernel(float* out, int iters) {
+    const int lane = threadIdx.x & 63;
+    f32x4 acc[16];
+#pragma unroll
+    for (int b = 0; b < 16; ++b)
+#pragma unroll
+        for (int r = 0; r < 4; ++r) acc[b][r] = 0.f;
+    half8 a, bb;
+#pragma unroll
+    for (int j = 0; j < 8; ++j) {
+        a[j] = (_Float16)(0.37f * (float)(((lane * 7 + j * 13) % 31) - 15));
+        bb[j] = (_Float16)(0.011f * (float)(((lane * 11 + j * 5) % 29) - 14));
+    }
+    for (int it = 0; it < iters; ++it) {
+#pragma unroll
+        for (int b = 0; b < 16; ++b) acc[b] = __builtin_amdgcn_mfma_f32_16x16x32_f16(a, bb, acc[b], 0, 0, 0);
+    }
+    float sum = 0.f;
+#pragma unroll
+    for (int b = 0; b < 16; ++b)
+#pragma unroll
+        for (int r = 0; r < 4; ++r) sum += acc[b][r];
+    if (sum == 123.456f) out[0] = sum;
+}
+
+static int32_t measure_peaks(float* out_host3, int n, void* stream) {
     hipStream_t s = (hipStream_t)stream;
     if (!out_host3) { adf_set_error("null argument"); return ADF_EINVAL; }
     int dev = 0, cus = 0;
@@ -80,8 +107,22 @@
         const double flop = waves * iters * 4.0 * 2.0 * 32 * 32 * (f16 ? 16 : 2);
         out_host3[f16 ? 1 : 2] = (float)(flop / (ms * 1e-3) * 1e-12);
     }
+    if (n == 4) {
+        for (int rep = 0; rep < 2; ++rep) {
+            ADF_HIP_CHECK(hipEventRecord(e0, s));
+            hipLaunchKernelGGL(adf_peak_mfma16_kernel, dim3(cus * 2), dim3(256), 0, s, d, iters / 2);
+            ADF_HIP_CHECK(hipEventRecord(e1, s));
+            ADF_HIP_CHECK(hipEventSynchronize(e1));
+            ADF_HIP_CHECK(hipEventElapsedTime(&ms, e0, e1));
+        }
+        out_host3[3] = (float)(waves * (iters / 2) * 16.0 * 2.0 * 16 * 16 * 32 / (ms * 1e-3) * 1e-12);
+    }
     (void)hipFree(d);
     (void)hipEventDestroy(e0); (void)hipEventDestroy(e1);
     ADF_HIP_CHECK(hipGetLastError());
     return ADF_OK;
 }
+
+extern "C" int32_t adf_measure_peaks(float* out_host3, void* stream) { return measure_peaks(out_host3, 3, stream); }
+
+extern "C" int32_t adf_measure_peaks4(float* out_host4, void* stream) { return measure_peaks(out_host4, 4, stream); }
diff --git a/adsorbdiff_amd/engine.py b/adsorbdiff_amd/engine.py
--- a/adsorbdiff_amd/engine.py
+++ b/adsorbdiff_amd/engine.py
@@ -603,7 +603,8 @@
         return out
 
     def measure_peaks(self):
-        out = (C.c_float * 3)()
-        with torch.cuda.device(self.device):
-            _lib.check(self.lib.adf_measure_peaks(out, self._stream()))
-        return {"hbm_copy_gbps": float(out[0]), "mfma_f16_tflops": float(out[1]), "mfma_f32_tflops": float(out[2])}
+        out = (C.c_float * 4)()
+        with torch.cuda.device(self.device):
+            _lib.check(self.lib.adf_measure_peaks4(out, self._stream()))
+        return {"hbm_copy_gbps": float(out[0]), "mfma_f16_tflops": float(out[1]), "mfma_f32_tflops": float(out[2]),
+                "mfma_f16_16x16x32_tflops": float(out[3])}
diff --git a/adsorbdiff_amd/lib.py b/adsorbdiff_amd/lib.py
--- a/adsorbdiff_amd/lib.py
+++ b/adsorbdiff_amd/lib.py
@@ -39,7 +39,7 @@
 class Tune(C.Structure):
     _fields_ = [(name, C.c_int32) for name in (
         "gemm_stream", "head_gate_fused", "lift_emit", "graph_sys_csr", "train_gemm16", "wgrad_f32",
-        "eqv2_gemm_tile256", "eqv2_rotin_generic", "eqv2_rotout_generic", "sample_split")]
+        "eqv2_gemm_tile256", "eqv2_rotin_generic", "eqv2_rotout_generic", "sample_split", "gemm_mfma16")]
 
 
 class SplitView(C.Structure):
@@ -137,6 +137,9 @@
 SLABS_HEADER = HEADER.with_name("adsorbdiff_slabs.h")
 SLABS_SIGNATURES = {name: sig for name, sig in parse_header(HEADER.read_text() + "\n" + SLABS_HEADER.read_text()).items()
                     if name not in SIGNATURES}
+PEAKS_HEADER = HEADER.with_name("adsorbdiff_peaks.h")
+PEAKS_SIGNATURES = {name: sig for name, sig in parse_header(HEADER.read_text() + "\n" + PEAKS_HEADER.read_text()).items()
+                    if name not in SIGNATURES}
 
 _LIB = None
 
@@ -161,7 +164,8 @@
             "(the HIP path has no CPU fallback)"
         )
     lib = C.CDLL(str(path))
-    for name, (restype, argtypes) in {**SIGNATURES, **SPLIT_SIGNATURES, **SCALE_FIT_SIGNATURES, **SLABS_SIGNATURES}.items():
+    for name, (restype, argtypes) in {**SIGNATURES, **SPLIT_SIGNATURES, **SCALE_FIT_SIGNATURES, **SLABS_SIGNATURES,
+                                      **PEAKS_SIGNATURES}.items():
         fn = getattr(lib, name)
         fn.restype, fn.argtypes = restype, argtypes
     _LIB = lib
diff --git a/include/adsorbdiff_hip.h b/include/adsorbdiff_hip.h
--- a/include/adsorbdiff_hip.h
+++ b/include/adsorbdiff_hip.h
@@ -67,6 +67,7 @@
     int32_t eqv2_rotin_generic;
     int32_t eqv2_rotout_generic;
     int32_t sample_split;
+    int32_t gemm_mfma16;
 } adf_tune;
 int32_t adf_painn_get_tune(adf_painn_t h, adf_tune* out);
 
diff --git a/include/adsorbdiff_peaks.h b/include/adsorbdiff_peaks.h
--- /dev/null
+++ b/include/adsorbdiff_peaks.h
@@ -0,0 +1,15 @@
+#ifndef ADSORBDIFF_PEAKS_H
+#define ADSORBDIFF_PEAKS_H
+
+#include "adsorbdiff_hip.h"
+
+#ifdef __cplusplus
+extern "C" {
+#endif
+
+int32_t adf_measure_peaks4(float* out_host4, void* stream);
+
+#ifdef __cplusplus
+}
+#endif
+#endif
```
